# ketanfatania/QMRI-PnP-Recon-POC

Hardware: AMD Instinct MI355X
Metric: ADMM iters/sec (224x224x10 TSMI, spiral mask) (higher is better)
Workload: dtype f32; 1 GPU; cut3 224x224x10 single slice per GPU, spiral mask S=771 T=200, PnP-ADMM + 10-channel UNetRes (DRUNet) denoiser; solver=lsqr, admm_iters=20, dc_dtype=f64, parallelism=slice-parallel x1 (no collective)

## Files before the change

### include/qmri.h

```cpp
#ifndef QMRI_H
#define QMRI_H

#include <stddef.h>
#include <stdint.h>

#ifdef __cplusplus
extern "C" {
#endif

#define QMRI_ABI_VERSION 1

typedef enum {
    QMRI_OK = 0,
    QMRI_ERR_INVALID_ARG = -1,
    QMRI_ERR_STATE = -2,
    QMRI_ERR_HIP = -3,
    QMRI_ERR_UNSUPPORTED = -4,
    QMRI_ERR_NOMEM = -5
} qmri_status;

typedef struct qmri_ctx qmri_ctx;

int qmri_abi_version(void);
int qmri_create(int device, qmri_ctx** out);
// ... 192 lines not shown
int qmri_coil_maps(qmri_ctx* ctx, int nslices, int ncoil, int N, int M, const void* calib, const qmri_csm_params* p, void* maps_out, void* img_out,
                   double* lambda_out, qmri_csm_info* info);
int qmri_coil_maps_dev(qmri_ctx* ctx, int nslices, int ncoil, int N, int M, const void* d_calib, const qmri_csm_params* p, void* d_maps_out,
                       void* d_img_out, double* d_lambda_out, qmri_csm_info* info);

typedef struct {
    int32_t s;
    int32_t s_max;
    double  energy;
    double  tol;
    int32_t maxit;
} qmri_dsvd_params;
typedef struct {
    int32_t s;
    int32_t iters;
    int32_t converged;
    int32_t energy_reached;
    double  max_resid;
    double  energy_kept;
} qmri_dsvd_info;
int qmri_dict_compress(qmri_ctx* ctx, int K, int T, const void* F, int f_is_f64, const qmri_dsvd_params* p, int* s_out, double* V_out, float* D_out,
                       float* normD_out, double* eig_out, qmri_dsvd_info* info);
int qmri_dict_compress_dev(qmri_ctx* ctx, int K, int T, const void* d_F, int f_is_f64, const qmri_dsvd_params* p, int* s_out, double* d_V_out,
                           float* d_D_out, float* d_normD_out, double* eig_out, qmri_dsvd_info* info);

typedef struct {
    int32_t nstates;
    int32_t inversion;
    double  ti;
    double  inv_eff;
    int32_t out_is_f64;
} qmri_epg_params;
int qmri_dict_simulate(qmri_ctx* ctx, int K, int T, const double* alpha, const double* tr, const double* te, const double* t1, const double* t2,
                       const double* b1, const qmri_epg_params* p, void* F_out);
int qmri_dict_simulate_dev(qmri_ctx* ctx, int K, int T, const double* alpha, const double* tr, const double* te, const double* d_t1, const double* d_t2,
                           const double* d_b1, const qmri_epg_params* p, void* d_F_out);

typedef struct {
    int32_t iters;
    double  beta;
    int32_t phase_sign;
    int32_t reserved[4];
} qmri_fieldmap_params;
typedef struct {
    double  cost0, cost;
    double  f_min, f_max;
    int32_t iters;
    int32_t reserved;
    double  unwrap_limit_hz;
} qmri_fieldmap_info;
int qmri_field_map_estimate(qmri_ctx* ctx, int nslices, int nechoes, int ncoil, int N, int M, const void* Y, const double* t_s, const double* f_init,
                            const qmri_fieldmap_params* p, double* f_out, double* trust_out, qmri_fieldmap_info* info);
int qmri_field_map_estimate_dev(qmri_ctx* ctx, int nslices, int nechoes, int ncoil, int N, int M, const void* d_Y, const double* t_s,
                                const double* d_f_init, const qmri_fieldmap_params* p, double* d_f_out, double* d_trust_out, qmri_fieldmap_info* info);

typedef struct {
    double  tau;
    int32_t block;
    int32_t shift;
    int32_t reserved[5];
} qmri_llr_params;
int qmri_llr_prox(qmri_ctx* ctx, int N, int M, int s, int nslices, const void* x, int x_is_complex, const qmri_llr_params* p, int o1, int o2,
                  void* out, double* sigma_max_out);
int qmri_llr_prox_dev(qmri_ctx* ctx, int N, int M, int s, int nslices, const void* d_x, int x_is_complex, const qmri_llr_params* p, int o1, int o2,
                      void* d_out, double* sigma_max_out);
int qmri_set_llr(qmri_ctx* ctx, const qmri_llr_params* p);

typedef struct {
    double ms_xupdate, ms_denoiser, ms_elementwise, ms_diag, ms_match;
    double ms_conv3x3;
    int64_t n_conv3x3;
    int64_t lsqr_iters;
    int64_t admm_iters;
    double ms_tv_iter;
    int64_t n_tv_iter;
    double flop_conv3x3;
    double ms_conv2x2;
    int64_t n_conv2x2;
    double flop_conv2x2;
    double ms_lsqr_kernels;
    int64_t n_lsqr_launches;
    double ms_net_forward;
    int64_t n_net_forward;
} qmri_profile;
int qmri_profile_enable(qmri_ctx* ctx, int level);
int qmri_profile_get(qmri_ctx* ctx, qmri_profile* out, int reset);

typedef struct {
    int denoiser_scheme;
    int denoiser_fallbacks;
    int resident_armed;
    int resident_timeouts;
    int lsqr_one_launch;
    int lsqr_timeouts;
    int repeated_calls;
    int reserved;
    double last_call_wall_ms;
    double last_call_stage_ms[4];
    double set_denoiser_ms[3];
} qmri_health;
int qmri_get_health(const qmri_ctx* ctx, qmri_health* out);

int qmri_debug_lsqr_stamps(qmri_ctx* ctx, unsigned long long* out);
int qmri_debug_conv_stamps(qmri_ctx* ctx, unsigned long long* out, int reserved);
int qmri_debug_lsqr_persist(qmri_ctx* ctx, int on);
int qmri_debug_dict_filter(qmri_ctx* ctx, int on, float margin_scale);
int qmri_debug_conv_resident(qmri_ctx* ctx, int on, int* timeouts_out);
int qmri_debug_dsvd_gram(qmri_ctx* ctx, int K, int T, const void* F, int f_is_f64, int on_device, double* G_out);
int qmri_debug_epg_shift(qmri_ctx* ctx, int S, int nshift, const double* in, double* out);
int qmri_debug_knob(const char* name, int value);

#ifdef __cplusplus
}
#endif
#endif
```

### qmri_pnp_recon_poc_amd/_lib.py

```python
from __future__ import annotations

import ctypes as C
import os
import subprocess

_PKG = os.path.dirname(os.path.abspath(__file__))
LIB_PATH = os.path.join(_PKG, "libqmri.so")
CSRC = os.path.join(_PKG, "csrc")

SYMBOLS = [
    "qmri_abi_version", "qmri_create", "qmri_destroy", "qmri_last_error", "qmri_set_stream", "qmri_synchronize",
    "qmri_build_spiral", "qmri_build_epi", "qmri_build_spiral_traj", "qmri_set_operator", "qmri_set_operator_nufft", "qmri_nufft_prepare_normal", "qmri_normal", "qmri_normal_dev",
    "qmri_nufft_dcf", "qmri_set_sample_weights", "qmri_adjoint_w", "qmri_adjoint_w_dev", "qmri_adjoint_w_mc", "qmri_set_field_map", "qmri_nufft_prepare_normal_fm", "qmri_operator_m", "qmri_forward", "qmri_adjoint",
    "qmri_forward_f32", "qmri_adjoint_f32", "qmri_forward_dev", "qmri_adjoint_dev", "qmri_set_coils", "qmri_forward_mc", "qmri_adjoint_mc", "qmri_xupdate_mc", "qmri_pnp_admm_mc", "qmri_xupdate_mc_batch", "qmri_pnp_admm_mc_batch", "qmri_pnp_admm_mc_dev", "qmri_xupdate", "qmri_net_nparams", "qmri_set_denoiser", "qmri_denoise",
    "qmri_net_forward_dev", "qmri_denoiser_scheme", "qmri_pnp_admm", "qmri_pnp_admm_dev", "qmri_pnp_admm_batch", "qmri_set_dictionary", "qmri_dict_match",
    "qmri_dict_match_dev", "qmri_dict_match_xfit", "qmri_dict_match_xfit_dev", "qmri_set_dictionary_groups", "qmri_dict_group_assign", "qmri_dict_match_grouped",
    "qmri_dict_match_grouped_dev", "qmri_recon_batch", "qmri_recon_batch_mc",
    "qmri_coil_compress", "qmri_coil_compress_dev", "qmri_coil_eig", "qmri_recon_batch_mc_cc", "qmri_coil_maps", "qmri_coil_maps_dev", "qmri_dict_compress", "qmri_dict_compress_dev", "qmri_dict_simulate", "qmri_dict_simulate_dev", "qmri_field_map_estimate", "qmri_field_map_estimate_dev", "qmri_llr_prox", "qmri_llr_prox_dev", "qmri_set_llr", "qmri_profile_enable", "qmri_profile_get", "qmri_get_health",
    "qmri_debug_lsqr_stamps", "qmri_debug_conv_stamps", "qmri_debug_lsqr_persist", "qmri_debug_dict_filter", "qmri_debug_conv_resident", "qmri_debug_dsvd_gram", "qmri_debug_epg_shift", "qmri_debug_knob",
    "qmri_onnx_read_unetres",
    "qmri_lrtv", "qmri_prox_tv", "qmri_norm_tv", "qmri_synthesize_tsmi", "qmri_synthesize_tsmi_complex",
]


# ... 19 lines not shown
    _fields_ = [("nv", C.c_int32), ("energy", C.c_double), ("shared", C.c_int32)]


class CsmParams(C.Structure):
    _fields_ = [("kind", C.c_int), ("cN", C.c_int), ("cM", C.c_int), ("patch", C.c_int), ("window", C.c_int), ("phase_ref", C.c_int), ("thresh", C.c_double)]


class CsmInfo(C.Structure):
    _fields_ = [("max_iters", C.c_int32), ("not_converged", C.c_int32)]


class DsvdParams(C.Structure):
    _fields_ = [("s", C.c_int32), ("s_max", C.c_int32), ("energy", C.c_double), ("tol", C.c_double), ("maxit", C.c_int32)]


class DsvdInfo(C.Structure):
    _fields_ = [("s", C.c_int32), ("iters", C.c_int32), ("converged", C.c_int32), ("energy_reached", C.c_int32),
                ("max_resid", C.c_double), ("energy_kept", C.c_double)]


class EpgParams(C.Structure):
    _fields_ = [("nstates", C.c_int32), ("inversion", C.c_int32), ("ti", C.c_double), ("inv_eff", C.c_double), ("out_is_f64", C.c_int32)]


class NufftParams(C.Structure):
    _fields_ = [("width", C.c_int32), ("reserved", C.c_int32 * 7)]


class DcfParams(C.Structure):
    _fields_ = [("niter", C.c_int32), ("tol", C.c_double), ("reserved", C.c_int32 * 6)]


class DcfInfo(C.Structure):
    _fields_ = [("iters", C.c_int32), ("dev", C.c_double), ("clamped", C.c_int32), ("split_tiles", C.c_int32), ("reserved", C.c_int32 * 4)]


class OffresParams(C.Structure):
    _fields_ = [("nseg", C.c_int32), ("nbins", C.c_int32), ("tol", C.c_double), ("reserved", C.c_int32 * 4)]


class OffresInfo(C.Structure):
    _fields_ = [("nseg", C.c_int32), ("tol_reached", C.c_int32), ("fit_max", C.c_double), ("fit_rms", C.c_double), ("f_min", C.c_double),
                ("f_max", C.c_double), ("t_min", C.c_double), ("t_max", C.c_double), ("reserved", C.c_int32 * 4)]


class OffresNormalParams(C.Structure):
    _fields_ = [("nseg", C.c_int32), ("tol", C.c_double), ("reserved", C.c_int32 * 4)]


class OffresNormalInfo(C.Structure):
    _fields_ = [("nseg", C.c_int32), ("tol_reached", C.c_int32), ("fit_max", C.c_double), ("fit_rms", C.c_double), ("khat_bytes", C.c_uint64),
                ("reserved", C.c_int32 * 4)]


class FieldmapParams(C.Structure):
    _fields_ = [("iters", C.c_int32), ("beta", C.c_double), ("phase_sign", C.c_int32), ("reserved", C.c_int32 * 4)]


class FieldmapInfo(C.Structure):
    _fields_ = [("cost0", C.c_double), ("cost", C.c_double), ("f_min", C.c_double), ("f_max", C.c_double), ("iters", C.c_int32), ("reserved", C.c_int32),
                ("unwrap_limit_hz", C.c_double)]


class LlrParams(C.Structure):
    _fields_ = [("tau", C.c_double), ("block", C.c_int32), ("shift", C.c_int32), ("reserved", C.c_int32 * 5)]


class LrtvParams(C.Structure):
    _fields_ = [("K", C.c_double), ("iters", C.c_int32), ("step", C.c_double), ("tol", C.c_double), ("backtrack", C.c_int32),
                ("prox_tol", C.c_double), ("prox_maxit", C.c_int32)]


class LrtvInfo(C.Structure):
    _fields_ = [("iters", C.c_int32), ("halvings", C.c_int32), ("step", C.c_double), ("obj", C.c_double),
                ("prox_calls", C.c_int32), ("prox_iters_total", C.c_int32)]


class Profile(C.Structure):
    _fields_ = [("ms_xupdate", C.c_double), ("ms_denoiser", C.c_double), ("ms_elementwise", C.c_double),
                ("ms_diag", C.c_double), ("ms_match", C.c_double), ("ms_conv3x3", C.c_double),
                ("n_conv3x3", C.c_int64), ("lsqr_iters", C.c_int64), ("admm_iters", C.c_int64),
                ("ms_tv_iter", C.c_double), ("n_tv_iter", C.c_int64),
                ("flop_conv3x3", C.c_double), ("ms_conv2x2", C.c_double), ("n_conv2x2", C.c_int64), ("flop_conv2x2", C.c_double),
                ("ms_lsqr_kernels", C.c_double), ("n_lsqr_launches", C.c_int64), ("ms_net_forward", C.c_double), ("n_net_forward", C.c_int64)]


class Health(C.Structure):
    _fields_ = [("denoiser_scheme", C.c_int32), ("denoiser_fallbacks", C.c_int32), ("resident_armed", C.c_int32), ("resident_timeouts", C.c_int32),
                ("lsqr_one_launch", C.c_int32), ("lsqr_timeouts", C.c_int32), ("repeated_calls", C.c_int32), ("reserved", C.c_int32),
                ("last_call_wall_ms", C.c_double), ("last_call_stage_ms", C.c_double * 4), ("set_denoiser_ms", C.c_double * 3)]


def build(force: bool = False) -> str:
    srcs = [os.path.join(CSRC, f) for f in os.listdir(CSRC) if f.endswith((".hip", ".cpp", ".h")) or f == "Makefile"]
    srcs.append(os.path.join(os.path.dirname(_PKG), "include", "qmri.h"))
    stale = force or not os.path.exists(LIB_PATH)
    if not stale:
        t = os.path.getmtime(LIB_PATH)
        stale = any(os.path.getmtime(s) > t for s in srcs)
    if stale:
        subprocess.run(["make", "-C", CSRC, "-s", "-j4"], check=True)
    return LIB_PATH


_lib = None


def lib() -> C.CDLL:
    global _lib
    if _lib is not None:
        return _lib
    path = os.environ.get("QMRI_LIBQMRI") or LIB_PATH
    if path == LIB_PATH and not os.path.exists(LIB_PATH):
        build()
    L = C.CDLL(path)
    missing = [s for s in SYMBOLS if not hasattr(L, s)]
    if missing:
        raise ImportError(f"libqmri.so lacks symbols declared in include/qmri.h: {missing}")
    vp, ip, dp, fp, i = C.c_void_p, C.POINTER(C.c_int32), C.POINTER(C.c_double), C.POINTER(C.c_float), C.c_int
    L.qmri_abi_version.restype = i
    L.qmri_create.argtypes = [i, C.POINTER(vp)]
    L.qmri_destroy.argtypes = [vp]
    L.qmri_last_error.restype = C.c_char_p
    L.qmri_last_error.argtypes = [vp]
    L.qmri_set_stream.argtypes = [vp, vp]
    L.qmri_synchronize.argtypes = [vp]
    L.qmri_build_spiral.argtypes = [vp, i, i, i, ip, ip, i, C.POINTER(i)]
    L.qmri_build_epi.argtypes = [vp, i, i, C.c_double, i, ip, ip, i, C.POINTER(i)]
    L.qmri_set_operator.argtypes = [vp, i, i, i, i, dp, ip, ip, i]
    L.qmri_build_spiral_traj.argtypes = [vp, i, i, i, ip, dp, i, C.POINTER(i)]
    L.qmri_set_operator_nufft.argtypes = [vp, i, i, i, i, dp, ip, dp, i, C.POINTER(NufftParams)]
    L.qmri_nufft_prepare_normal.argtypes = [vp]
    L.qmri_normal.argtypes = [vp, vp, i, vp]
    L.qmri_normal_dev.argtypes = [vp, vp, vp, i]
    L.qmri_nufft_dcf.argtypes = [vp, C.POINTER(DcfParams), dp, C.POINTER(DcfInfo)]
    L.qmri_set_sample_weights.argtypes = [vp, dp]
    L.qmri_adjoint_w.argtypes = [vp, vp, vp]
    L.qmri_adjoint_w_dev.argtypes = [vp, vp, vp, i]
    L.qmri_adjoint_w_mc.argtypes = [vp, vp, vp]
    L.qmri_set_field_map.argtypes = [vp, dp, dp, C.POINTER(OffresParams), C.POINTER(OffresInfo)]
    L.qmri_nufft_prepare_normal_fm.argtypes = [vp, C.POINTER(OffresNormalParams), C.POINTER(OffresNormalInfo)]
    L.qmri_operator_m.argtypes = [vp, C.POINTER(i)]
    L.qmri_forward.argtypes = [vp, vp, i, vp]
    L.qmri_adjoint.argtypes = [vp, vp, vp]
    L.qmri_forward_f32.argtypes = [vp, fp, i, fp]
    L.qmri_adjoint_f32.argtypes = [vp, fp, fp]
    L.qmri_forward_dev.argtypes = [vp, vp, vp, i]
    L.qmri_adjoint_dev.argtypes = [vp, vp, vp, i]
    L.qmri_set_coils.argtypes = [vp, i, vp]
    L.qmri_forward_mc.argtypes = [vp, vp, i, vp]
    L.qmri_adjoint_mc.argtypes = [vp, vp, vp]
    L.qmri_xupdate_mc.argtypes = [vp, vp, vp, C.c_double, C.c_double, i, vp, vp, ip, ip]
    L.qmri_pnp_admm_mc.argtypes = [vp, vp, C.POINTER(AdmmParams), vp, vp, ip]
    L.qmri_xupdate_mc_batch.argtypes = [vp, i, i, vp, vp, vp, C.c_double, C.c_double, i, vp, vp, ip, ip]
    L.qmri_pnp_admm_mc_batch.argtypes = [vp, i, i, i, vp, vp, C.POINTER(AdmmParams), vp, vp, ip]
    L.qmri_pnp_admm_mc_dev.argtypes = [vp, i, i, vp, vp, C.POINTER(AdmmParams), vp, vp, ip]
    L.qmri_xupdate.argtypes = [vp, vp, vp, C.c_double, C.c_double, i, i, vp, ip, ip]
    L.qmri_net_nparams.restype = C.c_size_t
    L.qmri_net_nparams.argtypes = [C.POINTER(NetDesc)]
    L.qmri_set_denoiser.argtypes = [vp, C.POINTER(NetDesc), fp, C.c_size_t, i, i, i]
    L.qmri_denoise.argtypes = [vp, dp, i, i, i, i, dp]
    L.qmri_onnx_read_unetres.argtypes = [C.c_char_p, C.POINTER(NetDesc), fp, C.c_size_t, C.POINTER(C.c_size_t)]
    L.qmri_net_forward_dev.argtypes = [vp, vp, i, vp]
    L.qmri_denoiser_scheme.argtypes = [vp, C.POINTER(i), C.POINTER(i)]
    L.qmri_get_health.argtypes = [vp, C.POINTER(Health)]
    L.qmri_pnp_admm.argtypes = [vp, vp, C.POINTER(AdmmParams), vp, vp, vp, dp, ip]
    L.qmri_pnp_admm_dev.argtypes = [vp, i, vp, C.POINTER(AdmmParams), vp, vp, vp, dp, ip]
# ... 42 lines not shown
```

### qmri_pnp_recon_poc_amd/csrc/api_admm.cpp

```cpp
#include "qmri_internal.h"

#include <algorithm>
#include <chrono>
#include <cstdio>

struct StageTimer {
    qmri_ctx* ctx;
    bool on, marks;
    int cur = -1;
    explicit StageTimer(qmri_ctx* c) : ctx(c), on(c->prof_level == 1 || c->prof_level == 2), marks(c->prof_level == 3) {
        c->marks_n = 0;
        for (double& v : c->last_call_ms) v = 0.0;
    }
    void start() {
        if (on) (void)hipEventRecord(ctx->ev[0], ctx->stream);
        if (marks) {
            if (ctx->marks_n + 2 > ctx->marks.size()) {
                hipEvent_t a = nullptr, b = nullptr;
                if (hipEventCreate(&a) != hipSuccess || hipEventCreate(&b) != hipSuccess) { marks = false; return; }
                ctx->marks.push_back(a); ctx->marks.push_back(b); ctx->mark_kind.push_back(0);
            }
            cur = (int)ctx->marks_n;
            (void)hipEventRecord(ctx->marks[cur], ctx->stream);
        }
    }
    void stop(double& acc) {
        if (on) {
            (void)hipEventRecord(ctx->ev[1], ctx->stream);
            (void)hipEventSynchronize(ctx->ev[1]);
            float ms = 0.f;
            (void)hipEventElapsedTime(&ms, ctx->ev[0], ctx->ev[1]);
            acc += ms;
            ctx->last_call_ms[kind_of(acc)] += ms;
        }
        if (marks && cur >= 0) {
            (void)hipEventRecord(ctx->marks[cur + 1], ctx->stream);
            ctx->mark_kind[cur / 2] = kind_of(acc);
            ctx->marks_n = (size_t)cur + 2;
            cur = -1;
        }
    }
    int kind_of(const double& acc) const {
        const qmri_profile& p = ctx->prof;
        return (&acc == &p.ms_xupdate) ? 0 : (&acc == &p.ms_denoiser) ? 1 : (&acc == &p.ms_elementwise) ? 2 : 3;
    }
    void resolve() {
        if (!marks) return;
        for (size_t i = 0; i + 1 < ctx->marks_n; i += 2) {
            float ms = 0.f;
            if (hipEventElapsedTime(&ms, ctx->marks[i], ctx->marks[i + 1]) != hipSuccess) continue;
            const int k = ctx->mark_kind[i / 2];
            ctx->last_call_ms[k] += ms;
            (k == 0 ? ctx->prof.ms_xupdate : k == 1 ? ctx->prof.ms_denoiser : k == 2 ? ctx->prof.ms_elementwise : ctx->prof.ms_diag) += ms;
        }
        ctx->marks_n = 0;
    }
};

static int admm_net_fits(qmri_ctx* ctx, const qmri_admm_params* prm, int* multi_out, bool* cpx_out) {
    const OpHost& o = ctx->op;
    const NetPlan& net = ctx->net;
    QMRI_CHECK_ARG(ctx, prm->denoiser_type >= 0 && prm->denoiser_type <= (QMRI_DENOISER_COMPLEX | QMRI_DENOISER_MULTI_LEVEL),
                   "denoiser_type must be 0 .. 3 (QMRI_DENOISER_MULTI_LEVEL | QMRI_DENOISER_COMPLEX)");
    const int multi = (prm->denoiser_type & QMRI_DENOISER_MULTI_LEVEL) ? 1 : 0;
    const bool cpx = (prm->denoiser_type & QMRI_DENOISER_COMPLEX) != 0;
    const int planes = cpx ? 2 * o.s : o.s, other = cpx ? o.s : 2 * o.s;
    if (net.H != o.N || net.W != o.M || net.desc.in_nc != planes + multi || net.desc.out_nc != planes) {
        const bool other_domain = net.desc.in_nc == other + multi && net.desc.out_nc == other;
        qmri_set_error(ctx, "denoiser (%d x %d, %d -> %d channels) does not fit the operator (%d x %d x %d, %s, %s TSMIs: %d -> %d channels needed)",
                       net.H, net.W, net.desc.in_nc, net.desc.out_nc, o.N, o.M, o.s, multi ? "multi_level" : "single_level",
                       cpx ? "complex" : "real", planes + multi, planes);
        return (cpx || other_domain) ? QMRI_ERR_STATE : QMRI_ERR_INVALID_ARG;
    }
    *multi_out = multi;
    *cpx_out = cpx;
    return QMRI_OK;
}

static int admm_step_fits(qmri_ctx* ctx, const qmri_admm_params* prm, int* multi_out, bool* cpx_out) {
    if (!ctx->llr.on) return admm_net_fits(ctx, prm, multi_out, cpx_out);
    const OpHost& o = ctx->op;
    QMRI_CHECK_ARG(ctx, prm->denoiser_type >= 0 && prm->denoiser_type <= (QMRI_DENOISER_COMPLEX | QMRI_DENOISER_MULTI_LEVEL),
                   "denoiser_type must be 0 .. 3 (QMRI_DENOISER_MULTI_LEVEL | QMRI_DENOISER_COMPLEX)");
    if (o.N % ctx->llr.block || o.M % ctx->llr.block || o.s > 16) {
        qmri_set_error(ctx, "invalid argument: the LLR regulariser (block side %d, at most 16 channels) does not fit the operator (%d x %d x %d): the "
                            "block side must divide both sides", ctx->llr.block, o.N, o.M, o.s);
        return QMRI_ERR_INVALID_ARG;
    }
    *multi_out = 0;
    *cpx_out = (prm->denoiser_type & QMRI_DENOISER_COMPLEX) != 0;
    return QMRI_OK;
}

static int admm_start(qmri_ctx* ctx, int B, const double2* d_x, bool z_now) {
    OpHost& o = ctx->op;
    const size_t nb = (size_t)B * o.N * o.M * o.s * sizeof(double2);
    QMRI_HIP(ctx, hipMemcpyAsync(o.d_vv, d_x, nb, hipMemcpyDeviceToDevice, ctx->stream));
    QMRI_HIP(ctx, hipMemsetAsync(o.d_u, 0, nb, ctx->stream));
    if (z_now) QMRI_TRY(dc_launch_prepare_z(ctx, qmri_opdev(ctx), o.ls, B, o.d_vv, o.d_u, o.d_z));
    return QMRI_OK;
}

struct DenoiserStep { int B; const qmri_admm_params* prm; int multi; bool cpx; const double2* d_x; StageTimer* tm; };

static int admm_to_net(qmri_ctx* ctx, const DenoiserStep& d, int mm_nblk, bool mm_ready, bool copy_range_flag) {
    OpHost& o = ctx->op;
    NetPlan& net = ctx->net;
    const size_t plane = (size_t)o.N * o.M;
    if (d.tm) d.tm->start();
    QMRI_TRY(ew_launch_minmax_normalise(ctx, d.B, plane * o.s, (int)plane, o.N, o.s, d.multi, d.prm->noise_std, d.d_x, o.d_u, o.d_mm, o.d_norm, mm_nblk, net.in32,
                                        mm_ready, d.cpx));
    if (d.tm) { d.tm->stop(ctx->prof.ms_elementwise); d.tm->start(); }
    QMRI_TRY(net_forward(ctx, d.B));
    if (copy_range_flag && net.sp6 == 2 && (int)net.layers.size() + 1 > net.h_range_words)
        QMRI_HIP(ctx, hipMemcpyAsync(net.h_range_flag, net.d_range_flag, sizeof(unsigned), hipMemcpyDeviceToHost, ctx->stream));
    if (d.tm) d.tm->stop(ctx->prof.ms_denoiser);
    return QMRI_OK;
}

static int admm_denoiser_step(qmri_ctx* ctx, const DenoiserStep& d, bool copy_range_flag, int it) {
    OpHost& o = ctx->op;
    NetPlan& net = ctx->net;
    const size_t plane = (size_t)o.N * o.M;
    if (ctx->llr.on) {
        LlrPlan pl = {o.N, o.M, o.s, ctx->llr.block, 0, 0, d.cpx ? 0 : 1, ctx->llr.tau};
        llr_offsets(it, pl.block, ctx->llr.shift, &pl.o1, &pl.o2);
        if (d.tm) d.tm->start();
        QMRI_TRY(llr_prox_dev(ctx, pl, d.B, d.d_x, o.d_u, o.d_vv, nullptr, nullptr));
        if (d.tm) { d.tm->stop(ctx->prof.ms_denoiser); d.tm->start(); }
        QMRI_TRY(llr_dual_dev(ctx, d.B, plane * o.s, d.d_x, o.d_vv, o.d_u, o.d_z, o.ls.pz, o.ls.nblk_z));
        if (d.tm) d.tm->stop(ctx->prof.ms_elementwise);
        return QMRI_OK;
    }
    QMRI_TRY(admm_to_net(ctx, d, o.ls.nblk_z, false, copy_range_flag));
    if (d.tm) d.tm->start();
    QMRI_TRY(ew_launch_unnormalise_dual(ctx, d.B, plane * o.s, (int)plane, o.N, net.out32, net.in32, net.desc.residual_noise, o.d_norm, d.d_x, o.d_u,
                                        nullptr , o.d_z, o.ls.pz, o.ls.nblk_z, o.s, d.cpx));
    if (d.tm) d.tm->stop(ctx->prof.ms_elementwise);
    return QMRI_OK;
}

static int mc_require(qmri_ctx* ctx, int nslices, int ncoil, const void* maps, const void* y) {
    const OpHost& o = ctx->op;
    if (!o.ready) { qmri_set_error(ctx, "operator not set: call qmri_set_operator first"); return QMRI_ERR_STATE; }
    QMRI_CHECK_ARG(ctx, nslices >= 1 && ncoil >= 1 && ncoil <= 1024, "nslices >= 1 and 1 <= ncoil <= 1024");
    QMRI_CHECK_ARG(ctx, maps && y, "maps / y_mc must not be NULL");
    return QMRI_OK;
}
static int mc_admm_check(qmri_ctx* ctx, const qmri_admm_params* prm) {
    const NetPlan& net = ctx->net;
    if (!net.ready && !ctx->llr.on) { qmri_set_error(ctx, "denoiser not set: call qmri_set_denoiser first"); return QMRI_ERR_STATE; }
    QMRI_CHECK_ARG(ctx, prm, "params must not be NULL");
    QMRI_TRY(toep_check_solver(ctx, prm->solver));
    QMRI_CHECK_ARG(ctx, prm->iters >= 0 && prm->gamma > 0 && prm->cg_maxit >= 0 && (prm->solver == QMRI_SOLVER_LSQR || prm->solver == QMRI_SOLVER_TOEPLITZ),
                   "iters >= 0, gamma > 0, cg_maxit >= 0, LSQR solver required");
    int multi = 0;
    bool cpx = false;
    return admm_step_fits(ctx, prm, &multi, &cpx);
}

static int mc_admm_group(qmri_ctx* ctx, int B, int ncoil, const double2* d_maps, const double2* d_y, const qmri_admm_params* prm, const double2* d_x0,
                         double2* d_x, int32_t* li_out, int li_stride) {
    OpHost& o = ctx->op;
    const bool llr = ctx->llr.on;
    const int multi = (!llr && (prm->denoiser_type & QMRI_DENOISER_MULTI_LEVEL)) ? 1 : 0;
    const bool cpx = (prm->denoiser_type & QMRI_DENOISER_COMPLEX) != 0;
    const size_t n = (size_t)o.N * o.M * o.s;
    std::vector<int32_t> li((size_t)B);
    for (int attempt = 0;; ++attempt) {
        if (d_x0) QMRI_HIP(ctx, hipMemcpyAsync(d_x, d_x0, (size_t)B * n * sizeof(double2), hipMemcpyDeviceToDevice, ctx->stream));
        else QMRI_TRY(mc_adjoint_batch_dev(ctx, B, ncoil, d_maps, d_y, d_x));
        QMRI_TRY(admm_start(ctx, B, d_x, true));
        bool again = false;
        for (int it = 0; it < prm->iters; ++it) {
            QMRI_TRY(mc_xupdate_dev(ctx, prm->solver, B, ncoil, d_maps, d_y, o.d_z, prm->gamma, prm->cg_tol, prm->cg_maxit, d_x, li.data(), nullptr));
            if (li_out) for (int b = 0; b < B; ++b) li_out[(size_t)b * li_stride + it] = li[b];
            QMRI_TRY(admm_denoiser_step(ctx, {B, prm, multi, cpx, d_x, nullptr}, false, it));
            if (llr) continue;
            QMRI_HIP(ctx, hipStreamSynchronize(ctx->stream));
            QMRI_TRY(net_range_tripped(ctx, again));
            if (again) break;
        }
        if (!again) break;
        ctx->admm_repeats += 1;
        if (attempt >= 2) { qmri_set_error(ctx, "the denoiser's range guard tripped three times in a row in the multi-coil PnP-ADMM loop"); return QMRI_ERR_HIP; }
    }
    o.xhat_valid = false;
    return QMRI_OK;
}

struct McStaged {
    const void* maps;
    const void* y;
    const void* to_sz;
    const void* to_sx; bool zero_sx;
    void* x_out;
// ... 12 lines not shown
    else if (sg.zero_sx) QMRI_HIP(ctx, hipMemsetAsync(w.sx, 0, nx, ctx->stream));
    QMRI_TRY(run(w));
    QMRI_HIP(ctx, hipMemcpyAsync(sg.x_out, w.sx, nx, out, ctx->stream));
    if (sync) QMRI_HIP(ctx, hipStreamSynchronize(ctx->stream));
    return QMRI_OK;
}

static int pnp_admm_nufft(qmri_ctx* ctx, int nslices, const void* d_y, const qmri_admm_params* prm, const void* d_x0, void* d_x_out,
                          double* diag_out, int32_t* lsqr_iters_out) {
    if (nslices != 1) {
        qmri_set_error(ctx, "PnP-ADMM of %d slices in one call is not available on a trajectory operator (qmri_set_operator_nufft): reconstruct them "
                            "one at a time, or as a stack with qmri_pnp_admm_mc_batch and one unit coil per slice", nslices);
        return QMRI_ERR_UNSUPPORTED;
    }
    if (prm && prm->solver != QMRI_SOLVER_LSQR && prm->solver != QMRI_SOLVER_TOEPLITZ) {
        qmri_set_error(ctx, "the DIRECT solver is not available on a trajectory operator (qmri_set_operator_nufft): its closed form needs a gridded "
                            "mask; use QMRI_SOLVER_LSQR");
        return QMRI_ERR_UNSUPPORTED;
    }
    if (prm && prm->want_diag && diag_out) {
        qmri_set_error(ctx, "the per-iteration diagnostics are not available on a trajectory operator (qmri_set_operator_nufft): set want_diag = 0 "
                            "and evaluate the result with qmri_forward");
        return QMRI_ERR_UNSUPPORTED;
    }
    QMRI_TRY(mc_admm_check(ctx, prm));
    QMRI_CHECK_ARG(ctx, d_y && d_x_out && d_x_out != d_x0, "y / x_out must not be NULL, x_out must not alias x0");
    return mc_staged(ctx, 1, 1, {nullptr, d_y, d_x0, nullptr, false, d_x_out, true}, true, [&](McWork& w) {
        return mc_admm_group(ctx, 1, 1, ctx->op.nu.d_ones, w.sy, prm, d_x0 ? w.sz : nullptr, w.sx, lsqr_iters_out, prm->iters);
    });
}

static int pnp_admm_dev_impl(qmri_ctx* ctx, int nslices, const void* d_y, const qmri_admm_params* prm, const void* d_x0,
                             const void* d_gt, void* d_x_out, double* diag_out, int32_t* lsqr_iters_out, bool* repeat) {
    QMRI_HIP(ctx, hipSetDevice(ctx->device));
    if (ctx->op.ready && ctx->op.kind == OP_NUFFT) return pnp_admm_nufft(ctx, nslices, d_y, prm, d_x0, d_x_out, diag_out, lsqr_iters_out);
    OpHost& o = ctx->op;
    NetPlan& net = ctx->net;
    if (!o.ready) { qmri_set_error(ctx, "operator not set: call qmri_set_operator first"); return QMRI_ERR_STATE; }
    const bool llr = ctx->llr.on;
    if (!net.ready && !llr) { qmri_set_error(ctx, "denoiser not set: call qmri_set_denoiser first"); return QMRI_ERR_STATE; }
    QMRI_CHECK_ARG(ctx, d_y && prm && d_x_out, "y / params / x_out must not be NULL");
    const int B = nslices;
    QMRI_CHECK_ARG(ctx, B >= 1 && B <= o.maxB && (llr || B <= net.maxB), "nslices exceeds max_batch of the operator or the denoiser");
    QMRI_CHECK_ARG(ctx, prm->iters >= 0 && prm->gamma > 0 && prm->cg_maxit >= 0, "iters >= 0, gamma > 0, cg_maxit >= 0 required");
    int multi = 0;
    bool cpx = false;
    QMRI_TRY(admm_step_fits(ctx, prm, &multi, &cpx));
    const OpDev op = qmri_opdev(ctx);
    const size_t plane = (size_t)o.N * o.M, n = plane * o.s, nb = (size_t)B * n * sizeof(double2);
    const double2* y = (const double2*)d_y;
    StageTimer tm(ctx);

    QMRI_TRY(dc_launch_sort_y(ctx, op, o.ls, B, y));
    if (d_x0) QMRI_HIP(ctx, hipMemcpyAsync(o.d_x, d_x0, nb, hipMemcpyDeviceToDevice, ctx->stream));
    else QMRI_TRY(dc_launch_adj(ctx, op, B, y, o.d_tmp, o.d_x));
    QMRI_TRY(admm_start(ctx, B, o.d_x, false));
    if (prm->solver == QMRI_SOLVER_DIRECT) {
        QMRI_TRY(qmri_prepare_direct(ctx, prm->gamma));
        const double2* aty = o.d_x;
        if (d_x0) { QMRI_TRY(dc_launch_adj(ctx, op, B, y, o.d_tmp, o.d_xa)); aty = o.d_xa; }
        QMRI_TRY(dc_launch_fwd(ctx, op, o.ls, DC_SPECTRUM, B, aty, o.d_tmp, o.d_chat, nullptr));
    } else if (prm->solver != QMRI_SOLVER_LSQR) {
        QMRI_TRY(toep_check_solver(ctx, prm->solver));
        qmri_set_error(ctx, "unknown solver %d", prm->solver);
        return QMRI_ERR_INVALID_ARG;
    }
    if (prm->want_diag && diag_out) {
        if (o.d_diag) { (void)hipFree(o.d_diag); o.d_diag = nullptr; }
        QMRI_HIP(ctx, hipMalloc((void**)&o.d_diag, (size_t)B * std::max(prm->iters, 1) * 2 * sizeof(double)));
    }
    std::vector<int32_t> it_b(B);
    o.xhat_valid = false;
    const bool diag = prm->want_diag && diag_out;
    bool range_trip = false;
    std::vector<char> deferred_it((size_t)std::max(prm->iters, 1), 0);
    if (prm->solver == QMRI_SOLVER_LSQR && (size_t)prm->iters * B > o.h_ring_cap) {
        if (o.h_ring) { QMRI_HIP(ctx, hipStreamSynchronize(ctx->stream)); (void)hipHostFree(o.h_ring); o.h_ring = nullptr; o.h_ring_cap = 0; }
        const size_t cap = std::max<size_t>((size_t)prm->iters * B, 128);
        QMRI_HIP(ctx, hipHostMalloc((void**)&o.h_ring, cap * sizeof(LsqrState), hipHostMallocDefault));
        o.h_ring_cap = cap;
    }
    const bool fused = qmri_knob(K_FUSE_EW) != 0 && prm->solver == QMRI_SOLVER_LSQR && !llr;
    const int hb = dc_hpass_blocks(op);
    bool z_in_tmp = false;
    struct DeferGuard { NetPlan& n; ~DeferGuard() { n.act_defer = false; n.act_pending_valid = false; } } defer_guard{net};
    net.act_defer = fused;
    const DenoiserStep step = {B, prm, multi, cpx, o.d_x, &tm};
    for (int it = 0; it < prm->iters; ++it) {
        tm.start();
        if (it == 0) QMRI_TRY(dc_launch_prepare_z(ctx, op, o.ls, B, o.d_vv, o.d_u, o.d_z));
        if (prm->solver == QMRI_SOLVER_LSQR) {
            bool deferred = false;
            LsqrFuse lf;
            if (fused) { lf.z_hpass_nblk = z_in_tmp ? hb : 0; lf.mm_u = o.d_u; lf.mm = o.d_mm; lf.mm_cpx = cpx; }
            QMRI_TRY(qmri_lsqr_run(ctx, B, o.d_z, prm->gamma, prm->cg_tol, prm->cg_maxit, o.d_x, it_b.data(), nullptr,
                                   diag ? o.d_pd : nullptr,
                                   o.h_ring + (size_t)it * B, &deferred, &lf));
            deferred_it[it] = deferred ? 1 : 0;
            if (!deferred && lsqr_iters_out) for (int b = 0; b < B; ++b) lsqr_iters_out[(size_t)b * prm->iters + it] = it_b[b];
            if (it > 0 && !llr && net.sp6 == 2 && host_range_tripped(net)) { range_trip = true; tm.stop(ctx->prof.ms_xupdate); break; }
        } else {
            QMRI_TRY(dc_launch_direct(ctx, op, B, o.d_z, o.d_chat, prm->gamma, o.d_tmp, o.d_x));
            if (lsqr_iters_out) for (int b = 0; b < B; ++b) lsqr_iters_out[(size_t)b * prm->iters + it] = 0;
        }
        tm.stop(ctx->prof.ms_xupdate);
        if (prm->want_diag && diag_out) {
            tm.start();
            if (prm->solver != QMRI_SOLVER_LSQR) QMRI_TRY(dc_launch_fwd(ctx, op, o.ls, DC_DIAG, B, o.d_x, o.d_tmp, nullptr, o.d_pd));
            QMRI_TRY(ew_launch_diag(ctx, op, o.ls, B, o.d_x, (const double2*)d_gt, o.d_pd, o.d_diag, prm->iters, it));
            tm.stop(ctx->prof.ms_diag);
        }
        if (!fused) QMRI_TRY(admm_denoiser_step(ctx, step, !llr, it));
        else {
            QMRI_TRY(admm_to_net(ctx, step, hb, true, true));
            tm.start();
            const DualArgs da = {net.out32.base1(), net.in32.base1(), net.out32.hp, (int)net.out32.plane(), net.out32.batch_stride(), net.in32.batch_stride(),
                                 net.desc.residual_noise, o.d_norm, o.d_x, o.d_u, o.ls.pz, cpx ? 1 : 0};
            ActCheckArgs ac{};
            if (net.act_pending_valid) { ac = net.act_pending; net.act_pending_valid = false; }
            QMRI_TRY(dc_launch_dual_fwd_h(ctx, op, B, da, ac, o.d_tmp));
            z_in_tmp = true;
            tm.stop(ctx->prof.ms_elementwise);
        }
        ctx->prof.admm_iters += 1;
    }
    if (!range_trip) {
        QMRI_HIP(ctx, hipMemcpyAsync(d_x_out, o.d_x, nb, hipMemcpyDeviceToDevice, ctx->stream));
    }
    if (prm->want_diag && diag_out && prm->iters > 0 && !range_trip)
        QMRI_HIP(ctx, hipMemcpyAsync(diag_out, o.d_diag, (size_t)B * prm->iters * 2 * sizeof(double), hipMemcpyDeviceToHost, ctx->stream));
    QMRI_HIP(ctx, hipStreamSynchronize(ctx->stream));
    tm.resolve();
    QMRI_TRY(qmri_prof_chain_finish(ctx));
    if (prm->solver == QMRI_SOLVER_LSQR && !range_trip) {
        bool timed_out = false;
        for (int it = 0; it < prm->iters; ++it) {
            if (!deferred_it[it]) continue;
            for (int b = 0; b < B; ++b) {
                const LsqrState& h = o.h_ring[(size_t)it * B + b];
                if (h.flag == 77) timed_out = true;
                const int n_it = h.done ? h.iter : prm->cg_maxit;
                if (lsqr_iters_out) lsqr_iters_out[(size_t)b * prm->iters + it] = n_it;
                ctx->prof.lsqr_iters += n_it;
            }
        }
        if (timed_out) {
            fprintf(stderr, "libqmri: the one-launch LSQR timed out waiting for a partial sum; repeating the reconstruction with the two-launch iteration\n");
            ctx->ks_persist = 0;
            ctx->ks_timeouts += 1;
            *repeat = true;
            return QMRI_OK;
        }
    }
    if (prm->iters > 0 && !llr) QMRI_TRY(net_range_tripped(ctx, *repeat));
    return QMRI_OK;
}

extern "C" int qmri_pnp_admm_dev(qmri_ctx* ctx, int nslices, const void* d_y, const qmri_admm_params* prm, const void* d_x0,
                                 const void* d_gt, void* d_x_out, double* diag_out, int32_t* lsqr_iters_out) {
    if (!ctx) return QMRI_ERR_INVALID_ARG;
    const auto t0 = std::chrono::steady_clock::now();
    const auto prof_at_entry = ctx->prof;
    int st = QMRI_OK;
    for (bool repeat = true; st == QMRI_OK && repeat;) {
        repeat = false;
        st = pnp_admm_dev_impl(ctx, nslices, d_y, prm, d_x0, d_gt, d_x_out, diag_out, lsqr_iters_out, &repeat);
        if (st == QMRI_OK && repeat) { ctx->prof = prof_at_entry; ctx->admm_repeats += 1; }
    }
    ctx->last_call_wall_ms = std::chrono::duration<double, std::milli>(std::chrono::steady_clock::now() - t0).count();
    return st;
}

extern "C" int qmri_xupdate_mc_batch(qmri_ctx* ctx, int nslices, int ncoil, const void* maps, const void* y_mc, const void* z, double r, double tol, int maxit,
                                     const void* x0, void* x_out, int32_t* iters_out, int32_t* flags_out) {
    if (!ctx) return QMRI_ERR_INVALID_ARG;
    QMRI_HIP(ctx, hipSetDevice(ctx->device));
    QMRI_TRY(mc_require(ctx, nslices, ncoil, maps, y_mc));
    QMRI_CHECK_ARG(ctx, z && x_out && r > 0 && maxit >= 0, "z / x_out must not be NULL, r > 0, maxit >= 0");
    return mc_staged(ctx, nslices, ncoil, {maps, y_mc, z, x0, true, x_out}, true, [&](McWork& w) {
        return qmri_lsqr_mc_batch_dev(ctx, nslices, ncoil, w.sm, w.sy, w.sz, r, tol, maxit, w.sx, iters_out, flags_out);
    });
}

extern "C" int qmri_pnp_admm_mc_dev(qmri_ctx* ctx, int nslices, int ncoil, const void* d_maps, const void* d_y, const qmri_admm_params* prm,
                                    const void* d_x0, void* d_x_out, int32_t* lsqr_iters_out) {
    if (!ctx) return QMRI_ERR_INVALID_ARG;
    QMRI_HIP(ctx, hipSetDevice(ctx->device));
    QMRI_TRY(mc_require(ctx, nslices, ncoil, d_maps, d_y));
    QMRI_TRY(mc_admm_check(ctx, prm));
    QMRI_CHECK_ARG(ctx, d_x_out && d_x_out != d_x0, "x_out must not be NULL and must not alias x0");
    QMRI_CHECK_ARG(ctx, nslices <= ctx->op.maxB && (ctx->llr.on || nslices <= ctx->net.maxB), "nslices exceeds max_batch of the operator or the denoiser");
    QMRI_TRY(mc_admm_group(ctx, nslices, ncoil, (const double2*)d_maps, (const double2*)d_y, prm, (const double2*)d_x0, (double2*)d_x_out,
                           lsqr_iters_out, prm->iters));
    QMRI_HIP(ctx, hipStreamSynchronize(ctx->stream));
    return QMRI_OK;
}

// ... 112 lines not shown
```

### qmri_pnp_recon_poc_amd/csrc/api_core.cpp

```cpp
#include "qmri_internal.h"
#include "fft_codelets.h"

#include <algorithm>
#include <atomic>
#include <cmath>
#include <cstdarg>
#include <cstdlib>
#include <cstring>
#include <mutex>

static thread_local std::string g_create_err;

namespace {
struct KnobDef { const char* name; int dflt; };
const KnobDef g_knob_defs[K_COUNT] = {
    {"conv_scheme", 2}, {"conv_f32", 0}, {"conv_wt", 1}, {"conv_xcd", 1}, {"conv_persist", 1}, {"conv_splitk", 1},
    {"conv_midcfg", 3}, {"conv_deepcfg", 3}, {"conv_deepks", 4},
    {"conv_resident", 1}, {"res_head", 1}, {"res_tail", 1}, {"res_down", 1}, {"res_delay", 24}, {"res_rearm", 64},
    {"res_stamps", 0}, {"conv_stamps", 0}, {"conv_stamp_launch", -1}, {"lsqr_stamps", 0},
    {"conv_mt2", 1024}, {"conv_occ", 2},
    {"fuse_ew", 1}, {"lsqr_persist", 1}, {"lsqr_fold", 1}, {"dictw_lsp", 2}, {"verbose", 0},
    {"pack_gpu", 1}, {"nufft_seg", NU_SEG},
    {"fmap_fuse", 0}, {"fmap_start", 0},
};
std::atomic<int> g_knob_val[K_COUNT];
std::once_flag g_knob_once;

int knob_index(const char* name, size_t len) {
    for (int k = 0; k < K_COUNT; ++k)
        if (strlen(g_knob_defs[k].name) == len && strncmp(g_knob_defs[k].name, name, len) == 0) return k;
    return -1;
}
void knob_init() {
    for (int k = 0; k < K_COUNT; ++k) g_knob_val[k].store(g_knob_defs[k].dflt, std::memory_order_relaxed);
    const char* e = getenv("QMRI_DEBUG");
    while (e && *e) {
        const char* end = strchr(e, ',');
        const size_t len = end ? (size_t)(end - e) : strlen(e);
        const char* eq = (const char*)memchr(e, '=', len);
        const int k = eq ? knob_index(e, (size_t)(eq - e)) : -1;
        if (k >= 0) g_knob_val[k].store(atoi(eq + 1), std::memory_order_relaxed);
        else if (len) fprintf(stderr, "libqmri: QMRI_DEBUG: unknown or malformed entry '%.*s' ignored\n", (int)len, e);
        e = end ? end + 1 : nullptr;
    }
}
}

int qmri_knob(QmriKnob k) {
    std::call_once(g_knob_once, knob_init);
    return g_knob_val[k].load(std::memory_order_relaxed);
}

extern "C" int qmri_debug_knob(const char* name, int value) {
    std::call_once(g_knob_once, knob_init);
    const int k = name ? knob_index(name, strlen(name)) : -1;
    if (k < 0) { qmri_set_error(nullptr, "qmri_debug_knob: unknown knob '%s'", name ? name : "(null)"); return QMRI_ERR_INVALID_ARG; }
    g_knob_val[k].store(value, std::memory_order_relaxed);
    return QMRI_OK;
}

void qmri_set_error(qmri_ctx* ctx, const char* fmt, ...) {
    char buf[1024];
    va_list ap;
    va_start(ap, fmt);
    vsnprintf(buf, sizeof buf, fmt, ap);
    va_end(ap);
    if (ctx) ctx->err = buf; else g_create_err = buf;
}

extern "C" int qmri_abi_version(void) { return QMRI_ABI_VERSION; }

extern "C" const char* qmri_last_error(const qmri_ctx* ctx) { return ctx ? ctx->err.c_str() : g_create_err.c_str(); }

extern "C" int qmri_create(int device, qmri_ctx** out) {
    if (!out) { qmri_set_error(nullptr, "qmri_create: out is NULL"); return QMRI_ERR_INVALID_ARG; }
    *out = nullptr;
    int ndev = 0;
    hipError_t e = hipGetDeviceCount(&ndev);
    if (e != hipSuccess || ndev <= 0) {
        qmri_set_error(nullptr, "no HIP device available (%s); libqmri has no CPU fallback",
                       e != hipSuccess ? hipGetErrorString(e) : "device count 0");
        return QMRI_ERR_HIP;
    }
    if (device < 0 || device >= ndev) {
        qmri_set_error(nullptr, "device %d out of range (0..%d)", device, ndev - 1);
        return QMRI_ERR_INVALID_ARG;
    }
    hipDeviceProp_t prop;
    if ((e = hipGetDeviceProperties(&prop, device)) != hipSuccess) {
        qmri_set_error(nullptr, "hipGetDeviceProperties failed: %s", hipGetErrorString(e));
        return QMRI_ERR_HIP;
    }
    if (strncmp(prop.gcnArchName, "gfx950", 6) != 0) {
        qmri_set_error(nullptr, "device %d is %s; libqmri is built for gfx950 (MI355X) only", device, prop.gcnArchName);
        return QMRI_ERR_UNSUPPORTED;
    }
    if ((e = hipSetDevice(device)) != hipSuccess) {
        qmri_set_error(nullptr, "hipSetDevice failed: %s", hipGetErrorString(e));
        return QMRI_ERR_HIP;
    }
    qmri_ctx* ctx = new (std::nothrow) qmri_ctx();
    if (!ctx) { qmri_set_error(nullptr, "out of host memory"); return QMRI_ERR_NOMEM; }
    ctx->device = device;
    if ((e = hipStreamCreateWithFlags(&ctx->own_stream, hipStreamNonBlocking)) != hipSuccess) {
        qmri_set_error(nullptr, "hipStreamCreate failed: %s", hipGetErrorString(e));
        delete ctx;
        return QMRI_ERR_HIP;
    }
    ctx->stream = ctx->own_stream;
    for (auto& ev : ctx->ev) {
        if ((e = hipEventCreate(&ev)) != hipSuccess) {
            qmri_set_error(nullptr, "hipEventCreate failed: %s", hipGetErrorString(e));
            for (auto& x : ctx->ev) if (x) (void)hipEventDestroy(x);
            (void)hipStreamDestroy(ctx->own_stream);
            delete ctx;
            return QMRI_ERR_HIP;
        }
    }
    *out = ctx;
    return QMRI_OK;
}

static void free_dev(void* p) { if (p) (void)hipFree(p); }

void qmri_free_operator(qmri_ctx* ctx) {
    OpHost& o = ctx->op;
    void* ptrs[] = { o.d_Vt, o.d_ent, o.d_perm, o.d_kptr, o.d_tw, o.d_kslot, o.d_ginv, o.d_tmp, o.d_xa, o.d_xb, o.d_ya,
                     o.ls.st, o.ls.pz, o.ls.yk, o.ls.py,
                     (void*)o.ks.unit, (void*)o.ks.es, (void*)o.ks.grp, (void*)o.ks.sgrp,
                     o.ks.pu[0], o.ks.pu[1], o.ks.pv[0], o.ks.pv[1], o.ks.pinit, o.ks.pR, o.ks.cx, o.ks.cv, o.ks.cd, o.ks.cub,
                     o.ks.ut, o.ks.xhat, o.ks.zhat, o.ks.xhat_out, o.ks.stamps,
                     o.d_x, o.d_u, o.d_vv, o.d_z, o.d_chat, o.d_mm, o.d_norm, o.d_diag, o.d_pd, o.d_coils };
    for (void* p : ptrs) free_dev(p);
    if (o.h_state) (void)hipHostFree(o.h_state);
    if (o.h_ring) (void)hipHostFree(o.h_ring);
    free_dev(ctx->d_ks_gran); ctx->d_ks_gran = nullptr; ctx->ks_persist_cap = -1;
    mc_free_work(o.mc);
    nufft_free(o.nu);
    o = OpHost();
}

extern "C" int qmri_destroy(qmri_ctx* ctx) {
    if (!ctx) return QMRI_OK;
    (void)hipSetDevice(ctx->device);
    (void)hipStreamSynchronize(ctx->stream);
    qmri_free_operator(ctx);
    qmri_free_net(ctx);
    qmri_free_dict(ctx);
    cc_free_work(ctx->cc);
    for (auto& ev : ctx->ev) if (ev) (void)hipEventDestroy(ev);
    if (ctx->ev_state) (void)hipEventDestroy(ctx->ev_state);
    for (hipEvent_t e : ctx->chain) if (e) (void)hipEventDestroy(e);
    for (hipEvent_t e : ctx->marks) if (e) (void)hipEventDestroy(e);
    if (ctx->own_stream) (void)hipStreamDestroy(ctx->own_stream);
    delete ctx;
    return QMRI_OK;
}

extern "C" int qmri_set_stream(qmri_ctx* ctx, void* hip_stream) {
    if (!ctx) return QMRI_ERR_INVALID_ARG;
    ctx->stream = hip_stream ? (hipStream_t)hip_stream : ctx->own_stream;
    return QMRI_OK;
}

extern "C" int qmri_synchronize(qmri_ctx* ctx) {
    if (!ctx) return QMRI_ERR_INVALID_ARG;
    QMRI_HIP(ctx, hipSetDevice(ctx->device));
    QMRI_HIP(ctx, hipStreamSynchronize(ctx->stream));
    return QMRI_OK;
}

void spiral_points(int S, std::vector<double>& theta, std::vector<double>& rad) {
    const double pi = 3.14159265358979323846;
    theta.assign(S, 0.0); rad.assign(S, 0.0);
    double lo = HUGE_VAL, hi = -HUGE_VAL;
    for (int j = 0; j < S; ++j) {
        const double t = (j == S - 1) ? 2.0 * pi : (double)j * (2.0 * pi) / (double)(S - 1);
        theta[j] = 8.0 * t;
        rad[j] = std::pow(1.05, theta[j]);
        lo = std::min(lo, rad[j]);
        hi = std::max(hi, rad[j]);
    }
    for (double& r : rad) r = (r - lo) / (hi - lo);
}

extern "C" int qmri_build_spiral(qmri_ctx* ctx, int N, int S, int T, int32_t* frame_ptr, int32_t* kidx, int cap, int* m_out) {
    QMRI_CHECK_ARG(ctx, N > 0 && S > 1 && T > 0 && frame_ptr && (kidx || cap == 0) && m_out, "qmri_build_spiral arguments");
    const double delta = SPIRAL_DELTA;
    std::vector<double> theta, rad;
    spiral_points(S, theta, rad);
    std::vector<uint8_t> grid((size_t)N * N);
    const int half = N / 2;
    long m = 0;
    for (int f = 0; f < T; ++f) {
        frame_ptr[f] = (int32_t)m;
        std::fill(grid.begin(), grid.end(), 0);
        const double rot = (double)f * delta;
        for (int j = 0; j < S; ++j) {
            double gx = std::round(rad[j] * std::cos(theta[j] + rot) * N / 2.0) + N / 2.0 + 1.0;
            double gy = std::round(rad[j] * std::sin(theta[j] + rot) * N / 2.0) + N / 2.0 + 1.0;
            gx = std::min(gx, (double)N);
            gy = std::min(gy, (double)N);
            const int r = ((int)gx - 1 + half) % N, c = ((int)gy - 1 + half) % N;
            grid[(size_t)c * N + r] = 1;
        }
        for (int k = 0; k < N * N; ++k)
            if (grid[k]) {
                if (m < cap) kidx[m] = k;
                ++m;
            }
    }
    frame_ptr[T] = (int32_t)m;
    *m_out = (int)m;
    if (m > cap) { qmri_set_error(ctx, "kidx capacity %d too small, need %ld", cap, m); return QMRI_ERR_INVALID_ARG; }
    return QMRI_OK;
// ... 153 lines not shown
        ks.caps = base;
        int nunits = cut(KS_CAPS[base]);
        if (sparse && nunits < 0) { base = 0; ks.caps = 0; nunits = cut(KS_CAPS[0]); }
        const bool one_launch = ctx->ks_persist != 0 && (ctx->ks_persist > 0 || qmri_knob(K_LSQR_PERSIST));
        if ((max_batch == 1 || one_launch) && s == 10 && (nunits > 320 || nunits < 0)) {
            int ncu = 0;
            QMRI_HIP(ctx, hipDeviceGetAttribute(&ncu, hipDeviceAttributeMultiprocessorCount, ctx->device));
            const int order[2] = {sparse ? 1 : 2, sparse ? 2 : 1};
            for (int c : order) {
                bool fits = false;
                QMRI_TRY(ks_lds_fits(ctx, N, s, M, ks.vcap, c, &fits));
                if (!fits) continue;
                const int nu = cut(KS_CAPS[c]);
                if (nu > 0 && nu <= ncu) { ks.caps = c; nunits = nu; break; }
            }
            if (ks.caps == base) nunits = cut(KS_CAPS[base]);
        }
        if (nunits < 0) {
            int tried = std::max(KS_CAPS[base].ecap, KS_CAPS[0].ecap);
            if ((max_batch == 1 || one_launch) && s == 10) tried = std::max(tried, std::max(KS_CAPS[1].ecap, KS_CAPS[2].ecap));
            qmri_set_error(ctx, "a k location is sampled %d times; at most %d are supported%s", -nunits, tried,
                           tried < KS_CAPS[2].ecap ? " with several slices per launch and the two-launch LSQR iteration (one slice per launch: 2560)" : "");
            return QMRI_ERR_UNSUPPORTED;
        }
        bslot.push_back(ns);
        gptr.push_back((int32_t)grp.size());
        sgrp[ns] = (int32_t)grp.size();
        ks.ns = ns; ks.G = (int)bslot.size() - 1; ks.b0 = 0;
        bool v_fits = false;
        QMRI_TRY(ks_lds_fits(ctx, N, s, M, ks.vcap, ks.caps, &v_fits));
        if (!v_fits) {
            qmri_set_error(ctx, "V (T=%d x s=%d) does not fit the on-chip budget of the LSQR kernels", T, s);
            return QMRI_ERR_UNSUPPORTED;
        }
        std::vector<KsUnit> units(ks.G);
        for (int g = 0; g < ks.G; ++g) units[g] = KsUnit{bslot[g], bslot[g + 1], sptr[bslot[g]], sptr[bslot[g + 1]], gptr[g], gptr[g + 1], 0, 0};
        int32_t* p32; KSample* pes; KsGroup* pg; KsUnit* pu_;
#define KS_UPLOAD(ptr, field, vec, T_)                                                                 \
        QMRI_TRY(dev_alloc(ctx, &ptr, (vec).size()));                                                  \
        QMRI_HIP(ctx, hipMemcpy(ptr, (vec).data(), (vec).size() * sizeof(T_), hipMemcpyHostToDevice)); \
        ks.field = ptr;
        KS_UPLOAD(p32, sgrp, sgrp, int32_t)
        KS_UPLOAD(pes, es, es, KSample)
        KS_UPLOAD(pg, grp, grp, KsGroup)
        KS_UPLOAD(pu_, unit, units, KsUnit)
#undef KS_UPLOAD
        ctx->ks_lds_attr[0] = ctx->ks_lds_attr[1] = false;
    }
    ls.nblk_z = 256;
    OpDev dims{};
    dims.N = N; dims.M = M; dims.s = s;
    const size_t npart = (size_t)std::max(ls.nblk_z, dc_hpass_blocks(dims));
    QMRI_TRY(dev_alloc(ctx, &o.d_tmp, B * n));
    QMRI_TRY(dev_alloc(ctx, &o.d_xa, B * n));
    QMRI_TRY(dev_alloc(ctx, &o.d_xb, B * n));
    QMRI_TRY(dev_alloc(ctx, &o.d_ya, B * (size_t)m));
    QMRI_TRY(dev_alloc(ctx, &ls.st, B));
    QMRI_TRY(dev_alloc(ctx, &ls.pz, B * npart));
    QMRI_TRY(dev_alloc(ctx, &ls.py, B * (size_t)DC_SORT_BLOCKS));
    for (int par = 0; par < 2; ++par) {
        QMRI_TRY(dev_alloc(ctx, &ks.pu[par], B * 2 * ks.G));
        QMRI_TRY(dev_alloc(ctx, &ks.pv[par], B * ks.G));
    }
    QMRI_TRY(dev_alloc(ctx, &ks.pinit, B * 2 * N));
    QMRI_TRY(dev_alloc(ctx, &ks.pR, B * N));
    QMRI_TRY(dev_alloc(ctx, &ks.cx, B * ks.ns * s));
    QMRI_TRY(dev_alloc(ctx, &ks.cv, B * ks.ns * s));
    QMRI_TRY(dev_alloc(ctx, &ks.cd, B * ks.ns * s));
    QMRI_TRY(dev_alloc(ctx, &ks.cub, B * ks.ns * s));
    QMRI_TRY(dev_alloc(ctx, &ks.ut, B * (size_t)m));
    QMRI_TRY(dev_alloc(ctx, &ks.xhat, B * n));
    QMRI_TRY(dev_alloc(ctx, &ks.zhat, B * n));
    QMRI_TRY(dev_alloc(ctx, &ks.xhat_out, B * n));
    ks.stamps = nullptr;
    if (qmri_knob(K_LSQR_STAMPS) > 0) { QMRI_TRY(dev_alloc(ctx, &ks.stamps, (size_t)2 * 512 * 16)); QMRI_HIP(ctx, hipMemset(ks.stamps, 0, 2 * 512 * 16 * 8)); }
    QMRI_TRY(dev_alloc(ctx, &ls.yk, B * (size_t)m));
    QMRI_TRY(dev_alloc(ctx, &o.d_x, B * n));
    QMRI_TRY(dev_alloc(ctx, &o.d_u, B * n));
    QMRI_TRY(dev_alloc(ctx, &o.d_vv, B * n));
    QMRI_TRY(dev_alloc(ctx, &o.d_z, B * n));
    QMRI_TRY(dev_alloc(ctx, &o.d_chat, B * n));
    QMRI_TRY(dev_alloc(ctx, &o.d_mm, B * npart * 2));
    QMRI_TRY(dev_alloc(ctx, &o.d_norm, B * 2));
    QMRI_TRY(dev_alloc(ctx, &o.d_pd, B * ((size_t)N + 2 * ls.nblk_z)));
    QMRI_HIP(ctx, hipMemset(ls.st, 0, B * sizeof(LsqrState)));
    QMRI_HIP(ctx, hipHostMalloc((void**)&o.h_state, B * sizeof(LsqrState), hipHostMallocDefault));
    ks.hst = nullptr; ks.st = ls.st; ks.pz = ls.pz; ks.nblk_z = ls.nblk_z; ks.yk = ls.yk; ks.pdiag = nullptr;
    o.xhat_valid = false;
    o.ginv_r = -1.0;
    QMRI_HIP(ctx, hipDeviceSynchronize());
    o.ready = true;
    return QMRI_OK;
}

extern "C" int qmri_operator_m(const qmri_ctx* ctx, int* m_out) {
    if (!ctx || !m_out) return QMRI_ERR_INVALID_ARG;
    if (!ctx->op.ready) return QMRI_ERR_STATE;
    *m_out = ctx->op.m;
    return QMRI_OK;
}

#define REQUIRE_OP(ctx)                                                                   \
    do {                                                                                  \
        if (!(ctx)) return QMRI_ERR_INVALID_ARG;                                          \
        QMRI_HIP((ctx), hipSetDevice((ctx)->device));                                     \
        if (!(ctx)->op.ready) { qmri_set_error((ctx), "operator not set: call qmri_set_operator first"); return QMRI_ERR_STATE; } \
    } while (0)

extern "C" int qmri_forward_dev(qmri_ctx* ctx, const void* d_x, void* d_y, int batch) {
    REQUIRE_OP(ctx);
    QMRI_CHECK_ARG(ctx, d_x && d_y && batch >= 1 && batch <= ctx->op.maxB, "qmri_forward_dev arguments / batch > max_batch");
    if (ctx->op.kind == OP_NUFFT) return nufft_launch_fwd(ctx, batch, (const double2*)d_x, (double2*)d_y);
    return dc_launch_fwd(ctx, qmri_opdev(ctx), ctx->op.ls, DC_PLAIN, batch, (const double2*)d_x, ctx->op.d_tmp,
                         (double2*)d_y, nullptr);
}

extern "C" int qmri_adjoint_dev(qmri_ctx* ctx, const void* d_y, void* d_x, int batch) {
    REQUIRE_OP(ctx);
    QMRI_CHECK_ARG(ctx, d_x && d_y && batch >= 1 && batch <= ctx->op.maxB, "qmri_adjoint_dev arguments / batch > max_batch");
    if (ctx->op.kind == OP_NUFFT) return nufft_launch_adj(ctx, batch, (const double2*)d_y, (double2*)d_x);
    return dc_launch_adj(ctx, qmri_opdev(ctx), batch, (const double2*)d_y, ctx->op.d_tmp, (double2*)d_x);
}

extern "C" int qmri_forward(qmri_ctx* ctx, const void* x, int x_is_complex, void* y) {
    REQUIRE_OP(ctx);
    QMRI_CHECK_ARG(ctx, x && y, "x / y must not be NULL");
    OpHost& o = ctx->op;
    const size_t n = (size_t)o.N * o.M * o.s;
    if (x_is_complex) {
        QMRI_HIP(ctx, hipMemcpyAsync(o.d_xa, x, n * sizeof(double2), hipMemcpyHostToDevice, ctx->stream));
    } else {
        QMRI_HIP(ctx, hipMemcpyAsync(o.d_xb, x, n * sizeof(double), hipMemcpyHostToDevice, ctx->stream));
        QMRI_TRY(ew_launch_real_to_complex(ctx, n, (const double*)o.d_xb, o.d_xa));
    }
    QMRI_TRY(qmri_forward_dev(ctx, o.d_xa, o.d_ya, 1));
    QMRI_HIP(ctx, hipMemcpyAsync(y, o.d_ya, (size_t)o.m * sizeof(double2), hipMemcpyDeviceToHost, ctx->stream));
    QMRI_HIP(ctx, hipStreamSynchronize(ctx->stream));
    return QMRI_OK;
}

extern "C" int qmri_adjoint(qmri_ctx* ctx, const void* y, void* x) {
    REQUIRE_OP(ctx);
    QMRI_CHECK_ARG(ctx, x && y, "x / y must not be NULL");
    OpHost& o = ctx->op;
    const size_t n = (size_t)o.N * o.M * o.s;
    QMRI_HIP(ctx, hipMemcpyAsync(o.d_ya, y, (size_t)o.m * sizeof(double2), hipMemcpyHostToDevice, ctx->stream));
    QMRI_TRY(qmri_adjoint_dev(ctx, o.d_ya, o.d_xa, 1));
    QMRI_HIP(ctx, hipMemcpyAsync(x, o.d_xa, n * sizeof(double2), hipMemcpyDeviceToHost, ctx->stream));
    QMRI_HIP(ctx, hipStreamSynchronize(ctx->stream));
    return QMRI_OK;
}

extern "C" int qmri_set_coils(qmri_ctx* ctx, int ncoil, const void* maps) {
    REQUIRE_OP(ctx);
    OpHost& o = ctx->op;
    QMRI_CHECK_ARG(ctx, ncoil >= 0 && ncoil <= 1024 && (ncoil == 0 || maps), "0 <= ncoil <= 1024, maps must not be NULL");
    QMRI_HIP(ctx, hipStreamSynchronize(ctx->stream));
    if (o.d_coils) { (void)hipFree(o.d_coils); o.d_coils = nullptr; }
    o.ncoil = 0;
    if (ncoil == 0) return QMRI_OK;
    const size_t count = (size_t)ncoil * o.N * o.M;
    QMRI_HIP(ctx, hipMalloc((void**)&o.d_coils, count * sizeof(double2)));
    QMRI_HIP(ctx, hipMemcpy(o.d_coils, maps, count * sizeof(double2), hipMemcpyHostToDevice));
    QMRI_HIP(ctx, hipDeviceSynchronize());
    o.ncoil = ncoil;
    return QMRI_OK;
// ... 47 lines not shown
    const size_t n = (size_t)o.N * o.M * o.s * (x_is_complex ? 2 : 1);
    std::vector<double> xd(x, x + n), yd((size_t)2 * o.m);
    QMRI_TRY(qmri_forward(ctx, xd.data(), x_is_complex, yd.data()));
    for (size_t i = 0; i < yd.size(); ++i) y[i] = (float)yd[i];
    return QMRI_OK;
}

extern "C" int qmri_adjoint_f32(qmri_ctx* ctx, const float* y, float* x) {
    REQUIRE_OP(ctx);
    QMRI_CHECK_ARG(ctx, x && y, "x / y must not be NULL");
    const OpHost& o = ctx->op;
    const size_t n2 = (size_t)2 * o.N * o.M * o.s;
    std::vector<double> yd(y, y + (size_t)2 * o.m), xd(n2);
    QMRI_TRY(qmri_adjoint(ctx, yd.data(), xd.data()));
    for (size_t i = 0; i < n2; ++i) x[i] = (float)xd[i];
    return QMRI_OK;
}

int qmri_prepare_direct(qmri_ctx* ctx, double r) {
    OpHost& o = ctx->op;
    if (o.ginv_r == r) return QMRI_OK;
    const int s = o.s, NM = o.N * o.M, T = o.T;
    std::vector<double> ginv((size_t)o.nsampled * s * s);
    std::vector<double> G(s * s), Li(s * s);
    int slot = 0;
    for (int kp = 0; kp < NM; ++kp) {
        const int e0 = o.kptr_h[kp], e1 = o.kptr_h[kp + 1];
        if (e1 == e0) continue;
        std::fill(G.begin(), G.end(), 0.0);
        for (int e = e0; e < e1; ++e) {
            const int t = o.ent_h[e].t;
            for (int a = 0; a < s; ++a)
                for (int b = 0; b < s; ++b) G[a * s + b] += o.V[t + (size_t)T * a] * o.V[t + (size_t)T * b];
        }
        for (int a = 0; a < s; ++a) G[a * s + a] += r;
        for (int j = 0; j < s; ++j) {
            double d = G[j * s + j];
            for (int k = 0; k < j; ++k) d -= G[j * s + k] * G[j * s + k];
            const double ljj = std::sqrt(d);
            G[j * s + j] = ljj;
            for (int i = j + 1; i < s; ++i) {
                double v = G[i * s + j];
                for (int k = 0; k < j; ++k) v -= G[i * s + k] * G[j * s + k];
                G[i * s + j] = v / ljj;
            }
        }
        std::fill(Li.begin(), Li.end(), 0.0);
        for (int c = 0; c < s; ++c) {
            for (int i = c; i < s; ++i) {
                double v = (i == c) ? 1.0 : 0.0;
                for (int k = c; k < i; ++k) v -= G[i * s + k] * Li[k * s + c];
                Li[i * s + c] = v / G[i * s + i];
            }
        }
        double* out = ginv.data() + (size_t)slot * s * s;
        for (int a = 0; a < s; ++a)
            for (int b = 0; b < s; ++b) {
                double v = 0.0;
                for (int k = std::max(a, b); k < s; ++k) v += Li[k * s + a] * Li[k * s + b];
                out[a * s + b] = v;
            }
        ++slot;
    }
    QMRI_HIP(ctx, hipMemcpyAsync(o.d_ginv, ginv.data(), ginv.size() * sizeof(double), hipMemcpyHostToDevice, ctx->stream));
    QMRI_HIP(ctx, hipStreamSynchronize(ctx->stream));
    o.ginv_r = r;
    return QMRI_OK;
}

int qmri_lsqr_run(qmri_ctx* ctx, int B, const double2* d_z, double r, double tol, int maxit, double2* d_x,
                  int32_t* iters_out, int32_t* flag_out, double* pdiag, LsqrState* hslot, bool* deferred, const LsqrFuse* fuse) {
    OpHost& o = ctx->op;
    QMRI_TRY(nufft_check_gridded(ctx, "the k-space LSQR", "the image-domain LSQR of the qmri_*_mc calls applies (internal)"));
    const OpDev op = qmri_opdev(ctx);
    KsDev ks = o.ks;
    ks.sr = std::sqrt(r); ks.tol = tol; ks.maxit = maxit; ks.ii = 0; ks.pdiag = pdiag;
    LsqrState* const hs = hslot ? hslot : o.h_state;
    ks.hst = hs;
    if (deferred) *deferred = false;
    const bool z_fused = fuse && fuse->z_hpass_nblk > 0;
    const double2* const mm_u = fuse ? fuse->mm_u : nullptr;
    double* const mm = fuse ? fuse->mm : nullptr;
    const bool mm_cpx = fuse && fuse->mm_cpx;
    if (z_fused && !o.xhat_valid) { qmri_set_error(ctx, "qmri_lsqr_run: a transformed z needs the spectrum of x (internal)"); return QMRI_ERR_STATE; }
    if (!o.xhat_valid) QMRI_TRY(dc_launch_fwd(ctx, op, o.ls, DC_SPECTRUM, B, d_x, o.d_tmp, ks.xhat, nullptr));
    if (z_fused) ks.nblk_z = fuse->z_hpass_nblk;
    else QMRI_TRY(dc_launch_fwd(ctx, op, o.ls, DC_FWD_H_ONLY, B, d_z, o.d_tmp, nullptr, nullptr));
    if (ctx->ks_persist < 0) ctx->ks_persist = qmri_knob(K_LSQR_PERSIST) ? 1 : 0;
    int per_launch = 0;
    if (ctx->ks_persist > 0 && maxit >= 1) QMRI_TRY(ks_persist_plan(ctx, op, ks, B, &per_launch));
    const bool fold = per_launch > 0 && qmri_knob(K_LSQR_FOLD) != 0;
    QMRI_TRY(ks_launch_init(ctx, op, ks, B, o.d_tmp, !fold));
    if (!ctx->ev_state) QMRI_HIP(ctx, hipEventCreateWithFlags(&ctx->ev_state, hipEventDisableTiming));
    bool persisted = false;
    if (per_launch > 0) {
        if (!ctx->d_ks_gran) {
            const size_t nb = ks_gran_bytes(ks.G, o.maxB);
            QMRI_HIP(ctx, hipMalloc(&ctx->d_ks_gran, nb));
            QMRI_HIP(ctx, hipMemsetAsync(ctx->d_ks_gran, 0, nb, ctx->stream));
        }
        const unsigned tag0 = ctx->ks_tag;
        QMRI_TRY(ks_launch_persist(ctx, op, ks, B, ctx->d_ks_gran, tag0, fold, &persisted));
        if (persisted) {
            ctx->ks_tag += 2u * (unsigned)(maxit + 2);
            QMRI_TRY(ks_launch_final(ctx, op, ks, B, o.d_tmp));
            QMRI_TRY(dc_launch_adj_h(ctx, op, B, o.d_tmp, d_x, mm_u, mm, mm_cpx));
            if (deferred) {
                *deferred = true;
                std::swap(o.ks.xhat, o.ks.xhat_out);
                o.xhat_valid = true;
                return QMRI_OK;
            }
            QMRI_HIP(ctx, hipStreamSynchronize(ctx->stream));
            for (int b = 0; b < B; ++b)
                if ((unsigned)__atomic_load_n(&hs[b].pad, __ATOMIC_ACQUIRE) != tag0) {
                    qmri_set_error(ctx, "the one-launch LSQR kernel ended without reporting its state");
                    return QMRI_ERR_HIP;
                }
            bool timed_out = false;
            for (int b = 0; b < B; ++b) timed_out = timed_out || hs[b].flag == 77;
            if (timed_out) {
                fprintf(stderr, "libqmri: the one-launch LSQR timed out waiting for a partial sum; using the two-launch iteration from now on\n");
                ctx->ks_persist = 0;
                ctx->ks_timeouts += 1;
                persisted = false;
                QMRI_TRY(ks_launch_init(ctx, op, ks, B));
            }
        }
    }
    if (fold && !persisted && !(ctx->ks_persist == 0)) QMRI_TRY(ks_launch_init(ctx, op, ks, B));
    int launched = 0;
    int chunk = std::min(std::max(ctx->lsqr_pred, 1), std::max(maxit, 1));
    bool all_done = persisted;
    if (!persisted) do {
        const int nthis = std::min(chunk, maxit - launched);
        for (int k = 0; k < nthis; ++k) {
            ks.ii = launched + k + 1;
            QMRI_TRY(ks_launch_iter(ctx, op, ks, B));
        }
        launched += std::max(nthis, 0);
        QMRI_HIP(ctx, hipEventRecord(ctx->ev_state, ctx->stream));
        QMRI_TRY(ks_launch_final(ctx, op, ks, B, o.d_tmp));
        QMRI_TRY(dc_launch_adj_h(ctx, op, B, o.d_tmp, d_x, mm_u, mm, mm_cpx));
        QMRI_HIP(ctx, hipEventSynchronize(ctx->ev_state));
        all_done = true;
        for (int b = 0; b < B; ++b) all_done = all_done && hs[b].done;
        chunk = 2;
    } while (launched < maxit && !all_done);
    std::swap(o.ks.xhat, o.ks.xhat_out);
    o.xhat_valid = true;
    int worst = 0;
    for (int b = 0; b < B; ++b) {
        const int it = hs[b].done ? hs[b].iter : maxit;
        if (iters_out) iters_out[b] = it;
        if (flag_out) flag_out[b] = hs[b].done ? hs[b].flag : 1;
        worst = std::max(worst, it);
        ctx->prof.lsqr_iters += it;
    }
    ctx->lsqr_pred = worst + 1;
    return QMRI_OK;
}

extern "C" int qmri_xupdate(qmri_ctx* ctx, const void* y, const void* z, double r, double tol, int maxit, int solver,
                            void* x, int32_t* iters_out, int32_t* flag_out) {
    if (solver == QMRI_SOLVER_TOEPLITZ) QMRI_TRY(offres_refuse_toeplitz(ctx, "QMRI_SOLVER_TOEPLITZ"));
    REQUIRE_OP(ctx);
    QMRI_CHECK_ARG(ctx, y && z && x && r > 0 && maxit >= 0, "qmri_xupdate arguments");
    OpHost& o = ctx->op;
    if (o.kind == OP_NUFFT) {
        if (solver != QMRI_SOLVER_LSQR && solver != QMRI_SOLVER_TOEPLITZ) {
            qmri_set_error(ctx, "the DIRECT solver is not available on a trajectory operator (qmri_set_operator_nufft): its closed form needs a gridded "
                                "mask; use QMRI_SOLVER_LSQR");
            return QMRI_ERR_UNSUPPORTED;
        }
        const size_t n = (size_t)o.N * o.M * o.s;
        QMRI_TRY(mc_ensure_staging(ctx, 1, 1));
        McWork& w = o.mc;
        QMRI_HIP(ctx, hipMemcpyAsync(w.sy, y, (size_t)o.m * sizeof(double2), hipMemcpyHostToDevice, ctx->stream));
        QMRI_HIP(ctx, hipMemcpyAsync(w.sz, z, n * sizeof(double2), hipMemcpyHostToDevice, ctx->stream));
        QMRI_HIP(ctx, hipMemcpyAsync(w.sx, x, n * sizeof(double2), hipMemcpyHostToDevice, ctx->stream));
        QMRI_TRY(mc_xupdate_dev(ctx, solver, 1, 1, o.nu.d_ones, w.sy, w.sz, r, tol, maxit, w.sx, iters_out, flag_out));
        QMRI_HIP(ctx, hipMemcpyAsync(x, w.sx, n * sizeof(double2), hipMemcpyDeviceToHost, ctx->stream));
        QMRI_HIP(ctx, hipStreamSynchronize(ctx->stream));
        return QMRI_OK;
    }
    const OpDev op = qmri_opdev(ctx);
    const size_t n = (size_t)o.N * o.M * o.s;
    QMRI_HIP(ctx, hipMemcpyAsync(o.d_ya, y, (size_t)o.m * sizeof(double2), hipMemcpyHostToDevice, ctx->stream));
    QMRI_HIP(ctx, hipMemcpyAsync(o.d_z, z, n * sizeof(double2), hipMemcpyHostToDevice, ctx->stream));
    QMRI_HIP(ctx, hipMemcpyAsync(o.d_x, x, n * sizeof(double2), hipMemcpyHostToDevice, ctx->stream));
    if (solver == QMRI_SOLVER_LSQR) {
        QMRI_TRY(dc_launch_sort_y(ctx, op, o.ls, 1, o.d_ya));
        QMRI_HIP(ctx, hipMemsetAsync(o.d_u, 0, n * sizeof(double2), ctx->stream));
        QMRI_TRY(dc_launch_prepare_z(ctx, op, o.ls, 1, o.d_z, o.d_u, o.d_vv));
        o.xhat_valid = false;
        QMRI_TRY(qmri_lsqr_run(ctx, 1, o.d_vv, r, tol, maxit, o.d_x, iters_out, flag_out, nullptr, nullptr, nullptr, nullptr));
    } else if (solver == QMRI_SOLVER_DIRECT) {
        QMRI_TRY(qmri_prepare_direct(ctx, r));
        QMRI_TRY(dc_launch_adj(ctx, op, 1, o.d_ya, o.d_tmp, o.d_xa));
        QMRI_TRY(dc_launch_fwd(ctx, op, o.ls, DC_SPECTRUM, 1, o.d_xa, o.d_tmp, o.d_chat, nullptr));
        QMRI_TRY(dc_launch_direct(ctx, qmri_opdev(ctx), 1, o.d_z, o.d_chat, r, o.d_tmp, o.d_x));
        if (iters_out) *iters_out = 0;
        if (flag_out) *flag_out = 0;
    } else {
        QMRI_TRY(toep_check_solver(ctx, solver));
        qmri_set_error(ctx, "unknown solver %d", solver);
        return QMRI_ERR_INVALID_ARG;
    }
    QMRI_HIP(ctx, hipMemcpyAsync(x, o.d_x, n * sizeof(double2), hipMemcpyDeviceToHost, ctx->stream));
    QMRI_HIP(ctx, hipStreamSynchronize(ctx->stream));
    return qmri_prof_chain_finish(ctx);
}

extern "C" int qmri_debug_lsqr_persist(qmri_ctx* ctx, int on) {
    if (!ctx) return QMRI_ERR_INVALID_ARG;
    ctx->ks_persist = (on == 2) ? 2 : (on ? 1 : 0);
    if (ctx->d_ks_gran && ctx->op.ready) {
        QMRI_HIP(ctx, hipSetDevice(ctx->device));
        QMRI_HIP(ctx, hipMemsetAsync((char*)ctx->d_ks_gran + ks_gran_bytes(ctx->op.ks.G, ctx->op.maxB) - 64, 0, 64, ctx->stream));
    }
    return QMRI_OK;
}

extern "C" int qmri_debug_lsqr_stamps(qmri_ctx* ctx, unsigned long long* out) {
    if (!ctx || !ctx->op.ks.stamps) return QMRI_ERR_STATE;
    QMRI_HIP(ctx, hipStreamSynchronize(ctx->stream));
// ... 56 lines not shown
```

### qmri_pnp_recon_poc_amd/csrc/api_net.cpp

```cpp
#include "qmri_internal.h"

#include <algorithm>
#include <chrono>
#include <cmath>
#include <cstdio>
#include <cstring>

extern "C" size_t qmri_net_nparams(const qmri_net_desc* d) {
    if (!d) return 0;
    size_t n = 0;
    if (d->arch == QMRI_ARCH_UNETRES) {
        const int32_t* nc = d->nc;
        n += (size_t)nc[0] * d->in_nc * 9;
        for (int l = 0; l < 3; ++l) n += (size_t)2 * d->nb * nc[l] * nc[l] * 9 + (size_t)nc[l + 1] * nc[l] * 4;
        n += (size_t)2 * d->nb * nc[3] * nc[3] * 9;
        for (int l = 3; l > 0; --l) n += (size_t)nc[l] * nc[l - 1] * 4 + (size_t)2 * d->nb * nc[l - 1] * nc[l - 1] * 9;
        n += (size_t)d->out_nc * nc[0] * 9;
    } else if (d->arch == QMRI_ARCH_SEQ_CONV) {
        if (d->nb == 1) return (size_t)d->out_nc * d->in_nc * 9;
        n = (size_t)d->nc[0] * d->in_nc * 9 + (size_t)(d->nb - 2) * d->nc[0] * d->nc[0] * 9 + (size_t)d->out_nc * d->nc[0] * 9;
    }
    return n;
}

// ... 289 lines not shown
        QMRI_HIP(ctx, hipStreamSynchronize(ctx->stream));
        ms_pack += std::chrono::duration<double, std::milli>(Clk::now() - t0).count();
    }
    p.w_begin = nullptr;
    QMRI_TRY(alloc_tensor(ctx, p.in32, desc->in_nc, conv_cin_pad(CONV_3X3, desc->in_nc), H, W, B));
    QMRI_TRY(alloc_tensor(ctx, p.out32, desc->out_nc, desc->out_nc, H, W, B));
    p.blk_ok = conv6_enabled();
    for (const ConvLayer& L : p.layers) if (!L.wp6) p.blk_ok = false;
    if (desc->arch == QMRI_ARCH_UNETRES) { for (int l = 0; l < 4; ++l) if (desc->nc[l] % 8) p.blk_ok = false; }
    else if (nb > 1 && desc->nc[0] % 8) p.blk_ok = false;
    for (int l = 0; l < 4; ++l) if ((p.x[l].p && p.x[l].Cal % 8) || (p.a[l].p && p.a[l].Cal % 8) || (p.t[l].p && p.t[l].Cal % 8)) p.blk_ok = false;
    p.interior_fmt = -1;
    QMRI_TRY(dev_alloc(ctx, &p.d_counter, (size_t)1));
    QMRI_HIP(ctx, hipMemset(p.d_counter, 0, sizeof(unsigned)));
    if (qmri_knob(K_CONV_STAMPS)) { QMRI_HIP(ctx, hipMalloc(&p.d_stamps, 4096 * 11 * sizeof(unsigned long long))); }
    p.counter_base = 0;
    p.ready = true;
    QMRI_HIP(ctx, hipDeviceSynchronize());
    const auto t_cal = Clk::now();
    if (p.sp6 == 2) QMRI_TRY(net_calibrate_scheme(ctx));
    const auto t_end = Clk::now();
    p.setup_ms[0] = ms_pack;
    p.setup_ms[2] = std::chrono::duration<double, std::milli>(t_end - t_cal).count();
    p.setup_ms[1] = std::chrono::duration<double, std::milli>(t_cal - t_upload).count() - ms_pack;
    return QMRI_OK;
}

static int run_resblocks(qmri_ctx* ctx, size_t& li, int nb, int B, const PTensor& src, const PTensor& cur, const PTensor& tmp,
                         const PTensor* skip) {
    NetPlan& p = ctx->net;
    if (p.d_res_xbuf && src.H == p.H && src.W == p.W && !p.force_f32) {
        bool done = false;
        Conv6rRun r;
        r.res = &p.layers[li]; r.nres = 2 * nb; r.src = &src; r.cur = &cur; r.skip = skip;
        QMRI_TRY(conv6r_try(ctx, r, B, &done));
        if (done) { li += (size_t)(2 * nb); return QMRI_OK; }
    }
    const PTensor* in = &src;
    for (int b = 0; b < nb; ++b) {
        QMRI_TRY(conv_launch(ctx, p.layers[li++], B, *in, tmp, nullptr, nullptr, 1));
        QMRI_TRY(conv_launch(ctx, p.layers[li++], B, tmp, cur, in, (b == nb - 1) ? skip : nullptr, 0));
        in = &cur;
    }
    return QMRI_OK;
}

static int net_forward_layers(qmri_ctx* ctx, int B);

static int net_forward_padded(qmri_ctx* ctx, int B) {
    {
        NetPlan& p = ctx->net;
        const bool blk = p.blk_ok && !p.force_f32 && conv6_enabled();
        if (p.interior_fmt != -1 && p.interior_fmt != (blk ? 1 : 0)) {
            PTensor* ts[12];
            int nt = 0;
            for (int l = 0; l < 4; ++l) { ts[nt++] = &p.x[l]; ts[nt++] = &p.a[l]; ts[nt++] = &p.t[l]; }
            for (int i = 0; i < nt; ++i)
                if (ts[i]->p) QMRI_HIP(ctx, hipMemsetAsync(ts[i]->p, 0, ((size_t)p.maxB * ts[i]->batch_stride() + 8192) * sizeof(float), ctx->stream));
        }
        p.interior_fmt = blk ? 1 : 0;
        for (int l = 0; l < 4; ++l) { p.x[l].blk = blk; p.a[l].blk = blk; p.t[l].blk = blk; }
    }
    const bool report = !ctx->net.force_f32;
    const bool timed = ctx->prof_level >= 2;
    if (timed) QMRI_HIP(ctx, hipEventRecord(ctx->ev[2], ctx->stream));
    if (report) QMRI_TRY(conv6_act_begin(ctx, (int)ctx->net.layers.size()));
    QMRI_TRY(net_forward_layers(ctx, B));
    if (report) QMRI_TRY(conv6_act_end(ctx));
    if (timed) QMRI_HIP(ctx, hipEventRecord(ctx->ev[3], ctx->stream));
    QMRI_TRY(qmri_prof_chain_finish(ctx));
    if (timed) {
        float ms = 0.f;
        QMRI_HIP(ctx, hipEventSynchronize(ctx->ev[3]));
        QMRI_HIP(ctx, hipEventElapsedTime(&ms, ctx->ev[2], ctx->ev[3]));
        ctx->prof.ms_net_forward += ms; ctx->prof.n_net_forward += 1;
    }
    return QMRI_OK;
}

static int net_forward_layers(qmri_ctx* ctx, int B) {
    NetPlan& p = ctx->net;
    const int nb = p.desc.nb;
    size_t li = 0;
    if (p.desc.arch == QMRI_ARCH_SEQ_CONV) {
        const size_t nl = p.layers.size();
        const PTensor* in = &p.in32;
        const PTensor* bufs[2] = { &p.a[0], &p.t[0] };
        for (size_t l = 0; l < nl; ++l) {
            const PTensor* out = (l == nl - 1) ? &p.out32 : bufs[l & 1];
            QMRI_TRY(conv_launch(ctx, p.layers[l], B, *in, *out, nullptr, nullptr, l != nl - 1));
            in = out;
        }
        return QMRI_OK;
    }
    const bool res_head = qmri_knob(K_RES_HEAD) != 0, res_tail = qmri_knob(K_RES_TAIL) != 0, res_down = qmri_knob(K_RES_DOWN) != 0;
    bool head_done = false, down_done = false;
    if (res_head && p.d_res_xbuf && !p.force_f32 && p.layers.size() >= (size_t)(2 + 2 * nb)) {
        Conv6rRun r;
        r.head = &p.layers[0]; r.head_in = &p.in32; r.res = &p.layers[1]; r.nres = 2 * nb; r.src = &p.x[0]; r.cur = &p.a[0];
        if (res_down) {
            r.down = &p.layers[1 + 2 * nb]; r.down_out = &p.x[1];
            QMRI_TRY(conv6r_try(ctx, r, B, &down_done));
            if (down_done) { head_done = true; li = (size_t)(2 + 2 * nb); }
            r.down = nullptr; r.down_out = nullptr;
        }
        if (!down_done) {
            QMRI_TRY(conv6r_try(ctx, r, B, &head_done));
            if (head_done) li = (size_t)(1 + 2 * nb);
        }
    }
    if (!head_done) QMRI_TRY(conv_launch(ctx, p.layers[li++], B, p.in32, p.x[0], nullptr, nullptr, 0));
    for (int l = 0; l < 3; ++l) {
        if (!(l == 0 && head_done)) QMRI_TRY(run_resblocks(ctx, li, nb, B, p.x[l], p.a[l], p.t[l], nullptr));
        if (!(l == 0 && down_done)) QMRI_TRY(conv_launch(ctx, p.layers[li++], B, p.a[l], p.x[l + 1], nullptr, nullptr, 0));
    }
    QMRI_TRY(run_resblocks(ctx, li, nb, B, p.x[3], p.a[3], p.t[3], &p.x[3]));
    for (int l = 3; l > 0; --l) {
        QMRI_TRY(conv_launch(ctx, p.layers[li++], B, p.a[l], p.a[l - 1], nullptr, nullptr, 0));
        if (l == 1 && res_tail && p.d_res_xbuf && !p.force_f32 && li + (size_t)(2 * nb) < p.layers.size()) {
            bool done = false;
            Conv6rRun r;
            r.res = &p.layers[li]; r.nres = 2 * nb; r.src = &p.a[0]; r.cur = &p.a[0]; r.skip = &p.x[0]; r.tail = &p.layers[li + 2 * nb]; r.tail_out = &p.out32;
            QMRI_TRY(conv6r_try(ctx, r, B, &done));
            if (done) { li += (size_t)(2 * nb + 1); return QMRI_OK; }
        }
        QMRI_TRY(run_resblocks(ctx, li, nb, B, p.a[l - 1], p.a[l - 1], p.t[l - 1], &p.x[l - 1]));
    }
    QMRI_TRY(conv_launch(ctx, p.layers[li++], B, p.a[0], p.out32, nullptr, nullptr, 0));
    return QMRI_OK;
}

int net_forward(qmri_ctx* ctx, int B) {
    NetPlan& p = ctx->net;
    const int st = net_forward_padded(ctx, B);
    if (st == QMRI_OK && p.res_off && p.res_timeouts > 0 && p.res_timeouts < 3 && !p.res_forced_off && ++p.res_clean >= std::max(1, qmri_knob(K_RES_REARM))) {
        p.res_off = false;
        p.res_clean = 0;
    }
    return st;
}

extern "C" int qmri_net_forward_dev(qmri_ctx* ctx, const float* d_in, int B, float* d_out) {
    if (!ctx) return QMRI_ERR_INVALID_ARG;
    QMRI_HIP(ctx, hipSetDevice(ctx->device));
    NetPlan& p = ctx->net;
    if (!p.ready) { qmri_set_error(ctx, "denoiser not set: call qmri_set_denoiser first"); return QMRI_ERR_STATE; }
    QMRI_CHECK_ARG(ctx, d_in && d_out && B >= 1 && B <= p.maxB, "qmri_net_forward_dev arguments / batch > max_batch");
    {
        const size_t hw = (size_t)p.H * p.W * B * sizeof(float);
        const char *a = (const char*)d_in, *b = (const char*)d_out;
        QMRI_CHECK_ARG(ctx, a + hw * p.desc.in_nc <= b || b + hw * p.desc.out_nc <= a, "qmri_net_forward_dev: d_in and d_out must not overlap");
    }
    bool again = false;
    for (int attempt = 0; attempt < 3; ++attempt) {
        QMRI_TRY(ew_launch_pack(ctx, B, p.desc.in_nc, p.H, p.W, d_in, 0, p.in32));
        QMRI_TRY(net_forward(ctx, B));
        QMRI_TRY(ew_launch_unpack(ctx, B, p.desc.out_nc, p.H, p.W, p.out32, p.in32, 0, d_out, 0));
        again = false;
        if (p.sp6 != 2) break;
        QMRI_HIP(ctx, hipStreamSynchronize(ctx->stream));
        QMRI_TRY(net_range_tripped(ctx, again));
        if (!again) break;
    }
    if (again) { qmri_set_error(ctx, "the network's guards asked for a fourth pass (resident-tile hand-off / f16 range): giving up"); return QMRI_ERR_HIP; }
    return QMRI_OK;
}

extern "C" int qmri_debug_conv_resident(qmri_ctx* ctx, int on, int* timeouts_out) {
    if (!ctx) return QMRI_ERR_INVALID_ARG;
    NetPlan& p = ctx->net;
    if (timeouts_out) *timeouts_out = p.res_timeouts;
    if (!p.ready) return QMRI_OK;
    p.res_off = (on == 0);
    p.res_forced_off = (on == 0);
    if (on) { p.res_timeouts = std::min(p.res_timeouts, 2); p.res_clean = 0; }
    p.res_drop = (on == 2) ? 1 : 0;
    return QMRI_OK;
}

extern "C" int qmri_denoiser_scheme(const qmri_ctx* ctx, int* scheme_out, int* fallbacks_out) {
    if (!ctx) return QMRI_ERR_INVALID_ARG;
    if (!ctx->net.ready) return QMRI_ERR_STATE;
    if (scheme_out) *scheme_out = ctx->net.sp6;
    if (fallbacks_out) *fallbacks_out = ctx->net.fallbacks;
    return QMRI_OK;
}

extern "C" int qmri_get_health(const qmri_ctx* ctx, qmri_health* out) {
    if (!ctx || !out) return QMRI_ERR_INVALID_ARG;
    const NetPlan& p = ctx->net;
    std::memset(out, 0, sizeof *out);
    out->denoiser_scheme = p.ready ? p.sp6 : 0;
    out->denoiser_fallbacks = p.ready ? p.fallbacks : 0;
// ... 78 lines not shown
```

### qmri_pnp_recon_poc_amd/csrc/conv6r_kernels.hip

```cpp
#include "conv6_device.h"

namespace {

constexpr int R_MAXL = 10;
constexpr int R_RELU = 1;
constexpr int R_ADD = 2;
constexpr int R_SKIP = 4;
constexpr int R_STORE = 8;
constexpr int R_STORE_WT = 16;
constexpr int R_KEEP = 32;
constexpr int R_DOWN = 128;
constexpr unsigned R_DOWN_STEPB = 2 * 2 * 2 * 64 * 16;
constexpr int R_LOCAL = 256;
constexpr int R_TAIL = 64;
constexpr int R_IH = 18, R_IW = 18, R_IHP = 24;
constexpr int R_NPX = R_IHP * (R_IW - 1) + R_IH;
constexpr int R_CHUNK = 2 * 2 * R_NPX;
constexpr int R_AST = ast6(2);
constexpr int R_SPIN_MAX = 1 << 16;
constexpr int R_SEGT = 86, R_CORT = 6;
constexpr int R_NTRI = 4 * R_SEGT + 4 * R_CORT;
constexpr size_t conv6r_lds() { return (size_t)(NABUF * R_AST + 4 * R_CHUNK) * 16; }

struct Conv6rArgs {
    const float* src; const float* skip;
    const float* radd[R_MAXL]; float* sdst[R_MAXL];
    float* dn_out; int dn_hp, dn_plane;
    float* out; int out_hp, out_plane, out_c;
    int in_planar, in_plane;
    int nch[R_MAXL], kind[R_MAXL];
    unsigned char* xbuf; size_t xbuf_half;
    const uint4* wp[R_MAXL];
    float dh[R_MAXL], dl[R_MAXL];
    int am_layer[R_MAXL];
    int nlayers, hp, plane, tiles_h, tiles_w, xcd;
    int drop;
    int delay;
    unsigned epoch;
    unsigned* range_flag; float* am_slots; int* am_count;
    unsigned long long* stamps;
};

template <int N> __device__ __forceinline__ void gwait_a(u32x4 (&a)[3]) { asm volatile("s_waitcnt vmcnt(%3)" : "+v"(a[0]), "+v"(a[1]), "+v"(a[2]) : "n"(N) : "memory"); }
template <int IMM> __device__ __forceinline__ void gload4r_sc1(f32x4& dst, unsigned off, const void* base) { asm volatile("global_load_dwordx4 %0, %1, %2 offset:%3 sc1" : "=v"(dst) : "v"(off), "s"(base), "n"(IMM) : "memory"); }
template <int IMM> __device__ __forceinline__ void gstore4r(unsigned off, f32x4 x, void* base) { asm volatile("global_store_dwordx4 %0, %1, %2 offset:%3\n\ts_nop 1" ::"v"(off), "v"(x), "s"(base), "n"(IMM) : "memory"); }
template <int IMM> __device__ __forceinline__ void gstore4r_sc1(unsigned off, f32x4 x, void* base) { asm volatile("global_store_dwordx4 %0, %1, %2 offset:%3 sc1\n\ts_nop 1" ::"v"(off), "v"(x), "s"(base), "n"(IMM) : "memory"); }

__device__ __forceinline__ void r_tri_decode(int t, int& seg, int& j) {
    if (t < 4 * R_SEGT) { seg = t / R_SEGT; j = t - seg * R_SEGT; } else { seg = 4 + (t - 4 * R_SEGT) / R_CORT; j = (t - 4 * R_SEGT) - (seg - 4) * R_CORT; }
}
__device__ __forceinline__ int r_seg_base(int seg) { return seg < 4 ? seg * R_SEGT : 4 * R_SEGT + (seg - 4) * R_CORT; }
__device__ __forceinline__ unsigned r_ent_lds(int k, int dw, int dh) {
    const int cb = k >> 1, sp = k & 1;
    return (unsigned)(((cb >> 1) * R_CHUNK + sp * 2 * R_NPX + (cb & 1) * R_NPX + dw * R_IHP + dh) * 16);
}

#define R_STAMP(role, k)                                                                                         \
    do {                                                                                                         \
        if constexpr (STAMP) {                                                                                   \
            if (A.stamps && (threadIdx.x & 255) == 0 && blockIdx.x % 50 == 0 && blockIdx.x / 50 < 4)             \
                A.stamps[(((blockIdx.x / 50) * 2 + (role)) * R_MAXL + l) * 8 + (k)] = wall_clock64();            \
        }                                                                                                        \
    } while (0)
template <bool STAMP>
__global__ __launch_bounds__(NT6) void k_conv6r(const Conv6rArgs A) {
    constexpr int SP = 2, AST = R_AST, IHP = R_IHP, NPX = R_NPX, NAQ = 3;
    static_assert(AST == NAQ * NLD6, "one weight step = three 16-byte entries per loader thread");
    extern __shared__ __align__(16) unsigned char smem[];
    uint4* Abuf = (uint4*)smem;
    uint4* Bt = Abuf + NABUF * AST;
    const int tid = threadIdx.x;
    const int bid = A.xcd ? xcd_remap(blockIdx.x, gridDim.x) : blockIdx.x;
    const int th = bid % A.tiles_h, tw = bid / A.tiles_h;
    const int oh0 = th * 16, ow0 = tw * 16;
    const int nl = A.nlayers;
    const unsigned plane32 = (unsigned)A.plane * 32u;
    const unsigned tile0 = (unsigned)((ow0 * A.hp + oh0) * 32);

    if (tid >= NT6 - NLD6) {
        const int lt = tid - (NT6 - NLD6);
        __builtin_amdgcn_s_setprio(2);
        constexpr unsigned ASTB = AST * 16;
        unsigned aoff[NAQ];
#pragma unroll
        for (int q = 0; q < NAQ; ++q) aoff[q] = (unsigned)((lt + NLD6 * q) * 16);
        int rq_l = 0, rq_s = 0, rq_n = 3 * A.nch[0];
        unsigned rq_stride = ASTB;
        u32x4 srdW = make_srd(A.wp[0]);
#define R_REQ(ra_)                                                                                               \
        {                                                                                                        \
            const unsigned so_ = (unsigned)rq_s * rq_stride;                                                     \
            _Pragma("unroll") for (int q = 0; q < NAQ; ++q) bload4(ra_[q], (q == 2 && rq_stride != ASTB) ? aoff[0] : aoff[q], srdW, so_); \
            if (++rq_s == rq_n) {                                                                                \
                if (rq_l + 1 < nl) { ++rq_l; rq_s = 0; rq_n = 3 * A.nch[rq_l]; srdW = make_srd(A.wp[rq_l]); rq_stride = (A.kind[rq_l] & R_DOWN) ? R_DOWN_STEPB : ASTB; } \
                else rq_s = rq_n - 1;                 \
            }                                                                                                    \
        }
#define R_STORE_A(buf_, ra_)                                                                                     \
        {                                                                                                        \
            uint4* ad = Abuf + (buf_) * AST;                                                                     \
            _Pragma("unroll") for (int q = 0; q < NAQ; ++q) *(uint4*)((unsigned char*)ad + aoff[q]) = __builtin_bit_cast(uint4, ra_[q]); \
        }
        u32x4 ra0[NAQ], ra1[NAQ], ra2[NAQ];
        {
            u32x4 pa1[NAQ];
            R_REQ(ra0) R_REQ(pa1) R_REQ(ra1) R_REQ(ra2)
            if (!A.in_planar) {
                constexpr int NHALF = 8 * R_IH * R_IW * 2, NPRO = (NHALF + NLD6 - 1) / NLD6;
                f32x4 v[NPRO];
                unsigned lo[NPRO];
#pragma unroll
                for (int k = 0; k < NPRO; ++k) {
                    const int idx = lt + NLD6 * k;
                    const bool valid = idx < NHALF;
                    const int idc = valid ? idx : 0, half = idc & 1, item = idc >> 1;
                    const int cb = item / (R_IH * R_IW), px = item - cb * (R_IH * R_IW), dw = px / R_IH, dh = px - dw * R_IH;
                    gload4r(v[k], (unsigned)cb * plane32 + (unsigned)((dw * A.hp + dh) * 32 + 16 * half) + tile0, A.src);
                    lo[k] = valid ? (unsigned)(((cb >> 1) * R_CHUNK + (cb & 1) * NPX + dw * IHP + dh) * 16 + 8 * half) : ~0u;
                }
                static_assert(NPRO == 21, "the wait below names 21 registers");
                asm volatile("s_waitcnt vmcnt(0)"
                             : "+v"(v[0]), "+v"(v[1]), "+v"(v[2]), "+v"(v[3]), "+v"(v[4]), "+v"(v[5]), "+v"(v[6]), "+v"(v[7]), "+v"(v[8]), "+v"(v[9]), "+v"(v[10]),
                               "+v"(v[11]), "+v"(v[12]), "+v"(v[13]), "+v"(v[14]), "+v"(v[15]), "+v"(v[16]), "+v"(v[17]), "+v"(v[18]), "+v"(v[19]), "+v"(v[20])::"memory");
#pragma unroll
                for (int k = 0; k < NPRO; ++k) {
                    uint2 s0, s1;
                    split_pair_h(v[k][0], v[k][1], s0.x, s1.x);
                    split_pair_h(v[k][2], v[k][3], s0.y, s1.y);
                    if (lo[k] != ~0u) {
                        *(uint2*)((unsigned char*)Bt + lo[k]) = s0;
                        *(uint2*)((unsigned char*)Bt + lo[k] + 2 * NPX * 16) = s1;
                    }
                }
            } else {
                constexpr int NIT = 2 * R_IH * R_IW, NQ = (NIT + NLD6 - 1) / NLD6;
                static_assert(NQ == 3, "the wait below names 24 registers");
                const int nin = A.nch[0];
                const unsigned pl4 = (unsigned)A.in_plane * 4u, t0 = (unsigned)((ow0 * A.hp + oh0) * 4);
#pragma unroll 1
                for (int ck = 0; ck < nin; ++ck) {
                    float v[NQ][8];
                    unsigned lo[NQ];
#pragma unroll
                    for (int k = 0; k < NQ; ++k) {
                        const int idx = lt + NLD6 * k;
                        const bool valid = idx < NIT;
                        const int idc = valid ? idx : 0, kh = idc / (R_IH * R_IW), px = idc - kh * (R_IH * R_IW), dw = px / R_IH, dh = px - dw * R_IH;
#pragma unroll
                        for (int j = 0; j < 8; ++j) gload1(v[k][j], (unsigned)(16 * ck + 8 * kh + j) * pl4 + (unsigned)((dw * A.hp + dh) * 4) + t0, A.src);
                        lo[k] = valid ? (unsigned)((ck * R_CHUNK + kh * NPX + dw * IHP + dh) * 16) : ~0u;
                    }
                    if (ck == 0) {
                        const uint4 z = make_uint4(0u, 0u, 0u, 0u);
                        for (int i = lt; i < (4 - nin) * R_CHUNK; i += NLD6) Bt[nin * R_CHUNK + i] = z;
                    }
                    asm volatile("s_waitcnt vmcnt(0)"
                                 : "+v"(v[0][0]), "+v"(v[0][1]), "+v"(v[0][2]), "+v"(v[0][3]), "+v"(v[0][4]), "+v"(v[0][5]), "+v"(v[0][6]), "+v"(v[0][7]), "+v"(v[1][0]),
                                   "+v"(v[1][1]), "+v"(v[1][2]), "+v"(v[1][3]), "+v"(v[1][4]), "+v"(v[1][5]), "+v"(v[1][6]), "+v"(v[1][7]), "+v"(v[2][0]), "+v"(v[2][1]),
                                   "+v"(v[2][2]), "+v"(v[2][3]), "+v"(v[2][4]), "+v"(v[2][5]), "+v"(v[2][6]), "+v"(v[2][7])::"memory");
#pragma unroll
                    for (int k = 0; k < NQ; ++k) {
                        uint4 s0, s1;
                        split_pair_h(v[k][0], v[k][1], s0.x, s1.x);
                        split_pair_h(v[k][2], v[k][3], s0.y, s1.y);
                        split_pair_h(v[k][4], v[k][5], s0.z, s1.z);
                        split_pair_h(v[k][6], v[k][7], s0.w, s1.w);
                        if (lo[k] != ~0u) {
                            *(uint4*)((unsigned char*)Bt + lo[k]) = s0;
                            *(uint4*)((unsigned char*)Bt + lo[k] + 2 * NPX * 16) = s1;
                        }
                    }
                }
            }
            gwait_a<0>(ra0); gwait_a<0>(pa1);
            R_STORE_A(0, ra0) R_STORE_A(1, pa1)
        }
        unsigned p_lds[2][3], p_x[2];
#pragma unroll
        for (int q = 0; q < 2; ++q) {
            const int t = lt + NLD6 * q;
            const bool valid = t < R_NTRI;
            int seg, j;
            r_tri_decode(valid ? t : 0, seg, j);
            const int npx = seg < 4 ? 16 : 1;
#pragma unroll
            for (int i = 0; i < 3; ++i) {
                const int E = 3 * j + i, Ec = (E < npx * 16) ? E : 0, pp = Ec >> 4, k = Ec & 15;
                const int w = (seg == 0) ? 0 : (seg == 1) ? 15 : (seg == 2 || seg == 3) ? pp : (seg < 6 ? 0 : 15);
                const int h = (seg == 0 || seg == 1) ? pp : (seg == 2) ? 0 : (seg == 3) ? 15 : ((seg & 1) ? 15 : 0);
                p_lds[q][i] = r_ent_lds(k, w + 1, h + 1);
            }
            p_x[q] = valid ? (unsigned)((tw * A.tiles_h + th) * (R_NTRI * 64) + t * 16) : ~0u;
        }
        lds_barrier6();
#define R_ITER(k_, rs_, rq_)               \
        {                                                                                                        \
            __builtin_amdgcn_s_setprio(2);                                                                       \
            R_REQ(rq_)                                                                                           \
            __builtin_amdgcn_s_setprio(0);                                                                       \
            gwait_a<2 * NAQ>(rs_);                                                                               \
            R_STORE_A(((k_) + 2) % NABUF, rs_)                                                                   \
            lds_barrier6();                                                                                      \
        }
#pragma unroll 1
        for (int l = 0; l < nl; ++l) {
#pragma unroll 1
            for (int g = 0; g < 3 * A.nch[l]; g += 3) {
                R_ITER(0, ra1, ra0)
                R_ITER(1, ra2, ra1)
                R_ITER(2, ra0, ra2)
            }
            R_STAMP(1, 0);
            if (A.kind[l] & R_TAIL) {
                lds_barrier6();
// ... 300 lines not shown
                bool pend[2] = {c_x[0] != ~0u && !dead, c_x[1] != ~0u && !dead};
                bool ok = false;
                for (int spin = 0; spin < R_SPIN_MAX; ++spin) {
                    u32x4 g[2][4];
#pragma unroll
                    for (int q = 0; q < 2; ++q)
                        if (pend[q]) {
#pragma unroll
                            for (int i = 0; i < 4; ++i) asm volatile("global_load_dwordx4 %0, %1, %2 sc1" : "=v"(g[q][i]) : "v"(c_x[q] + (unsigned)(i * (R_NTRI * 16))), "s"(xb) : "memory");
                        }
                    asm volatile("s_waitcnt vmcnt(0)" : "+v"(g[0][0]), "+v"(g[0][1]), "+v"(g[0][2]), "+v"(g[0][3]), "+v"(g[1][0]), "+v"(g[1][1]), "+v"(g[1][2]), "+v"(g[1][3])::"memory");
#pragma unroll
                    for (int q = 0; q < 2; ++q)
                        if (pend[q]) {
                            unsigned bad = 0;
#pragma unroll
                            for (int i = 0; i < 4; ++i) bad |= (g[q][i][1] ^ thi) | (g[q][i][3] ^ thi);
                            if ((bad >> 16) == 0) {
                                unsigned d[12];
#pragma unroll
                                for (int i = 0; i < 4; ++i) {
                                    d[3 * i] = g[q][i][0];
                                    d[3 * i + 1] = (g[q][i][1] & 0xFFFFu) | (g[q][i][2] << 16);
                                    d[3 * i + 2] = (g[q][i][2] >> 16) | (g[q][i][3] << 16);
                                }
#pragma unroll
                                for (int i = 0; i < 3; ++i)
                                    if (c_lds[q][i] != ~0u) *(uint4*)((unsigned char*)Bt + c_lds[q][i]) = make_uint4(d[4 * i], d[4 * i + 1], d[4 * i + 2], d[4 * i + 3]);
                                pend[q] = false;
                            }
                        }
                    if (!__any(pend[0] || pend[1])) { ok = true; break; }
                    __builtin_amdgcn_s_sleep(1);
                }
                if (!ok && !dead) { dead = true; if (lane == 0 && A.range_flag) atomicOr(A.range_flag, 4u); }
            }
        }
        R_STAMP(0, 5);
        lds_barrier6();
        R_STAMP(0, 6);
    }
}

}

int conv6r_try(qmri_ctx* ctx, const Conv6rRun& run, int B, bool* done) {
    *done = false;
    NetPlan& net = ctx->net;
    hipStreamCaptureStatus cap = hipStreamCaptureStatusNone;
    const bool capturing = hipStreamIsCapturing(ctx->stream, &cap) == hipSuccess && cap != hipStreamCaptureStatusNone;
    const int nres = run.nres, nl = nres + (run.head ? 1 : 0) + (run.tail ? 1 : 0) + (run.down ? 1 : 0);
    if (!qmri_knob(K_CONV_RESIDENT) || capturing || net.res_off || !net.d_res_xbuf || B != 1 || nres < 2 || nl > R_MAXL || (nres & 1) || net.d_stamps) return QMRI_OK;
    if (!run.res || !run.src || !run.cur || (run.head && (!run.head_in || run.skip)) || (run.tail && !run.tail_out) || (run.down && (!run.down_out || run.tail || run.skip))) return QMRI_OK;
    auto is3 = [](const ConvLayer& L) { return (L.kind == CONV_3X3 || L.kind == CONV_3X3N) && L.sp6 == 2 && L.wp6 && L.n_ct6 == 1; };
    for (int l = 0; l < nres; ++l) {
        const ConvLayer& L = run.res[l];
        if (!is3(L) || L.Cin != 64 || L.Cout != 64 || L.nchunk6 != 4) return QMRI_OK;
    }
    const PTensor &src = *run.src, &cur = *run.cur;
    const PTensor* ts[3] = {&src, &cur, run.skip};
    for (const PTensor* t : ts) {
        if (!t) continue;
        if (!t->p || !t->blk || t->Cal < 64 || t->H != src.H || t->W != src.W || t->hp != src.hp || t->h0 != src.h0) return QMRI_OK;
    }
    if (run.head) {
        const ConvLayer& L = *run.head;
        const PTensor& in = *run.head_in;
        if (!is3(L) || L.Cout != 64 || L.nchunk6 < 1 || L.nchunk6 > 2 || L.Cin > 16 * L.nchunk6 || !in.p || in.blk || in.Cal < 16 * L.nchunk6 || in.H != src.H || in.W != src.W || in.hp != src.hp ||
            in.h0 != src.h0 || src.p == cur.p) return QMRI_OK;
    }
    if (run.tail) {
        const ConvLayer& L = *run.tail;
        const PTensor& out = *run.tail_out;
        if (!is3(L) || L.Cin != 64 || L.nchunk6 != 4 || L.Cout > 32 || !out.p || out.blk || out.H != src.H || out.W != src.W ||
            (size_t)out.Cal * out.plane() * 4 >= ((size_t)1 << 31)) return QMRI_OK;
    }
    if (run.down) {
        const ConvLayer& L = *run.down;
        const PTensor& out = *run.down_out;
        if (L.kind != CONV_DOWN || L.sp6 != 2 || !L.wp6 || L.Cin != 64 || L.Cout != 128 || L.nchunk6 != 9 || L.n_ct6 != 2 || !out.p || !out.blk || out.Cal < 128 ||
            out.H * 2 != src.H || out.W * 2 != src.W || (size_t)out.Cal * out.plane() * 4 >= ((size_t)1 << 31)) return QMRI_OK;
    }
    if (src.H % 16 || src.W % 16) return QMRI_OK;
    if ((size_t)src.Cal * src.plane() * 4 >= ((size_t)1 << 31)) return QMRI_OK;
    if (!ctx->conv_ncu) {
        hipDeviceProp_t prop;
        QMRI_HIP(ctx, hipGetDeviceProperties(&prop, ctx->device));
        ctx->conv_ncu = prop.multiProcessorCount;
    }
    const int tiles_h = src.H / 16, tiles_w = src.W / 16, tiles = tiles_h * tiles_w;
    if (tiles > ctx->conv_ncu || tiles != net.res_tiles) return QMRI_OK;
    Conv6rArgs A{};
    A.src = run.head ? run.head_in->fbase() : src.fbase();
    A.in_planar = run.head ? 1 : 0; A.in_plane = run.head ? (int)run.head_in->plane() : 0;
    A.skip = run.skip ? run.skip->fbase() : nullptr;
    if (run.down) { A.dn_out = run.down_out->fbase(); A.dn_hp = run.down_out->hp; A.dn_plane = (int)run.down_out->plane(); }
    if (run.tail) { A.out = run.tail_out->fbase(); A.out_hp = run.tail_out->hp; A.out_plane = (int)run.tail_out->plane(); A.out_c = run.tail->Cout; }
    int l = 0;
    auto put = [&](const ConvLayer& L, int kind, const float* radd, float* sdst) {
        A.wp[l] = reinterpret_cast<const uint4*>(L.wp6);
        A.dh[l] = L.w6_descale; A.dl[l] = L.w6_descale * (1.f / LO_SCALE);
        A.am_layer[l] = conv6_act_slot(ctx, true, L).layer;
        A.nch[l] = L.nchunk6; A.kind[l] = kind; A.radd[l] = radd; A.sdst[l] = sdst;
        ++l;
    };
    if (run.head) put(*run.head, R_STORE | R_KEEP, nullptr, src.fbase());
    for (int r = 0; r < nres; ++r) {
        const bool last = r == nres - 1;
        if (!(r & 1)) put(run.res[r], R_RELU | R_KEEP, nullptr, nullptr);
        else if (!last) put(run.res[r], R_ADD | R_STORE | R_KEEP, (r == 1) ? src.fbase() : cur.fbase(), cur.fbase());
        else if (run.tail) put(run.res[r], R_ADD | (run.skip ? R_SKIP : 0) | R_KEEP, (r == 1) ? src.fbase() : cur.fbase(), nullptr);
        else if (run.down) put(run.res[r], R_ADD | R_KEEP | R_LOCAL, (r == 1) ? src.fbase() : cur.fbase(), nullptr);
        else put(run.res[r], R_ADD | (run.skip ? R_SKIP : 0) | R_STORE_WT, (r == 1) ? src.fbase() : cur.fbase(), cur.fbase());
    }
    if (run.tail) put(*run.tail, R_TAIL, nullptr, nullptr);
    if (run.down) { put(*run.down, R_DOWN, nullptr, nullptr); A.nch[l - 1] = 6; }
    for (int k = l; k < R_MAXL; ++k) { A.wp[k] = A.wp[l - 1]; A.nch[k] = A.nch[l - 1]; A.am_layer[k] = -1; }
    int pub[2] = {0, 0};
    for (int k = 0; k < l; ++k) if ((A.kind[k] & R_KEEP) && !(A.kind[k] & R_LOCAL)) pub[k & 1] += 1;
    if (!pub[0] || !pub[1]) return QMRI_OK;
    A.nlayers = nl; A.hp = src.hp; A.plane = (int)src.plane(); A.tiles_h = tiles_h; A.tiles_w = tiles_w;
    A.xbuf = net.d_res_xbuf; A.xbuf_half = (size_t)tiles * R_NTRI * 64;
    A.xcd = qmri_knob(K_CONV_XCD);
    const int delay = std::max(0, std::min(4096, qmri_knob(K_RES_DELAY)));
    A.epoch = net.res_epoch; A.drop = net.res_drop; A.delay = delay;
    A.range_flag = net.d_range_flag; A.am_slots = net.d_act_slots; A.am_count = net.d_act_count;
    if (!ctx->conv6r_attr) {
        QMRI_HIP(ctx, hipFuncSetAttribute((const void*)k_conv6r<false>, hipFuncAttributeMaxDynamicSharedMemorySize, (int)conv6r_lds()));
        QMRI_HIP(ctx, hipFuncSetAttribute((const void*)k_conv6r<true>, hipFuncAttributeMaxDynamicSharedMemorySize, (int)conv6r_lds()));
        ctx->conv6r_attr = true;
    }
    g_conv6_launch_counter.fetch_add(nl, std::memory_order_relaxed);
    const int stamp_which = qmri_knob(K_RES_STAMPS);
    A.stamps = (stamp_which == 2) == (run.head != nullptr) ? (unsigned long long*)net.d_res_stamps : nullptr;
    hipEvent_t e0 = nullptr, e1 = nullptr;
    double flop = 0.0;
    for (int r = 0; r < nres; ++r) flop += conv_layer_flop(run.res[r], 1, src.H, src.W);
    if (run.head) flop += conv_layer_flop(*run.head, 1, src.H, src.W);
    if (run.tail) flop += conv_layer_flop(*run.tail, 1, src.H, src.W);
    if (run.down) flop += conv_layer_flop(*run.down, 1, src.H, src.W);
    QMRI_TRY(qmri_prof_pair(ctx, &e0, &e1, PROF_CONV3, flop));
    if (A.stamps) k_conv6r<true><<<dim3(tiles), dim3(NT6), conv6r_lds(), ctx->stream>>>(A);
    else if (e0) hipExtLaunchKernelGGL((k_conv6r<false>), dim3(tiles), dim3(NT6), (std::uint32_t)conv6r_lds(), ctx->stream, e0, e1, 0, A);
    else k_conv6r<false><<<dim3(tiles), dim3(NT6), conv6r_lds(), ctx->stream>>>(A);
    QMRI_HIP(ctx, hipGetLastError());
    net.res_epoch += (unsigned)(nl - 1);
    *done = true;
    return QMRI_OK;
}

size_t conv6r_xbuf_bytes(int tiles) { return (size_t)2 * tiles * R_NTRI * 64; }
```

### qmri_pnp_recon_poc_amd/csrc/dc_kernels.hip

```cpp
#include "dc_device.h"
#include "conv6_act.h"

using namespace dcdev;

namespace {

template <int R1, int R2>
__global__ __launch_bounds__(NT) void k_fwd_h(OpDev op, const double2* __restrict__ src, double2* __restrict__ tmp) {
    typedef Plan<R1, R2> P;
    constexpr int N = P::N, L = Cfg<R1, R2>::L;
    __shared__ cd lds[L * P::LINE];
    const int tid = threadIdx.x, b = blockIdx.y;
    const size_t n = (size_t)op.s * N * op.M;
    const size_t base = (size_t)b * n + (size_t)blockIdx.x * L * N;
    for (int i = tid; i < L * N; i += NT) {
        const int line = i / N, nn = i - line * N;
        lds[line * P::LINE + nn] = src[base + i];
    }
    cd out[R2];
    int line2, k1;
    if (fft_lds<R1, R2, true>(lds, L, op.tw_h, out, line2, k1)) {
        const int l = blockIdx.x * L + line2;
        const int c = l / op.M, w = l - c * op.M;
        double2* dst = tmp + (size_t)b * n + (size_t)c * N * op.M + w;
// ... 164 lines not shown

template <int R1, int R2>
__global__ __launch_bounds__(NT) void k_adj_w(OpDev op, const double2* __restrict__ y_in,
                                               double2* __restrict__ tmp) {
    typedef Plan<R1, R2> P;
    constexpr int M = P::N;
    __shared__ cd lds[DC_MAXS * P::LINE];
    __shared__ double vlds[DC_VCAP];
    __shared__ double2 ulds[DC_CH];
    __shared__ unsigned short tlds[DC_CH];
    const int tid = threadIdx.x, b = blockIdx.y, kh = blockIdx.x, s = op.s, N = op.N;
    const size_t n = (size_t)s * N * M;
    const bool v_in_lds = op.T * s <= DC_VCAP;
    if (v_in_lds) for (int i = tid; i < op.T * s; i += NT) vlds[i] = op.Vt[i];
    const size_t mb = (size_t)b * op.m;
    constexpr int NQ = (M * DC_MAXS + NT - 1) / NT;
    double ar[NQ], ai[NQ];
    int e0[NQ], e1[NQ];
#pragma unroll
    for (int q = 0; q < NQ; ++q) {
        const int item = tid + NT * q;
        ar[q] = 0.0; ai[q] = 0.0;
        if (item < M * s) {
            const int kw = item / s;
            e0[q] = op.kptr[kh * M + kw]; e1[q] = op.kptr[kh * M + kw + 1];
        } else { e0[q] = 0; e1[q] = 0; }
    }
    const int r0 = op.kptr[kh * M], r1 = op.kptr[(kh + 1) * M];
    for (int lo = r0; lo < r1; lo += DC_CH) {
        const int hi = (lo + DC_CH < r1) ? lo + DC_CH : r1;
        __syncthreads();
        for (int i = tid; i < hi - lo; i += NT) {
            const int e = lo + i;
            ulds[i] = y_in[mb + op.perm[e]];
            tlds[i] = op.ent[e].t;
        }
        __syncthreads();
#pragma unroll
        for (int q = 0; q < NQ; ++q) {
            const int c = (tid + NT * q) % s;
            const int a0 = (e0[q] > lo) ? e0[q] : lo, a1 = (e1[q] < hi) ? e1[q] : hi;
            double xr = ar[q], xi = ai[q];
            int e = a0;
            for (; e + 4 <= a1; e += 4) {
                double2 u0 = ulds[e - lo], u1 = ulds[e - lo + 1], u2 = ulds[e - lo + 2], u3 = ulds[e - lo + 3];
                const int t0 = tlds[e - lo], t1 = tlds[e - lo + 1], t2 = tlds[e - lo + 2], t3 = tlds[e - lo + 3];
                const double v0 = v_in_lds ? vlds[t0 * s + c] : op.Vt[(size_t)t0 * s + c];
                const double v1 = v_in_lds ? vlds[t1 * s + c] : op.Vt[(size_t)t1 * s + c];
                const double v2 = v_in_lds ? vlds[t2 * s + c] : op.Vt[(size_t)t2 * s + c];
                const double v3 = v_in_lds ? vlds[t3 * s + c] : op.Vt[(size_t)t3 * s + c];
                xr += v0 * u0.x; xi += v0 * u0.y;
                xr += v1 * u1.x; xi += v1 * u1.y;
                xr += v2 * u2.x; xi += v2 * u2.y;
                xr += v3 * u3.x; xi += v3 * u3.y;
            }
            for (; e < a1; ++e) {
                const double2 u0 = ulds[e - lo];
                const int t0 = tlds[e - lo];
                const double v0 = v_in_lds ? vlds[t0 * s + c] : op.Vt[(size_t)t0 * s + c];
                xr += v0 * u0.x; xi += v0 * u0.y;
            }
            ar[q] = xr; ai[q] = xi;
        }
    }
#pragma unroll
    for (int q = 0; q < NQ; ++q) {
        const int item = tid + NT * q;
        if (item < M * s) {
            const int kw = item / s, c = item - kw * s;
            lds[c * P::LINE + kw] = mk(ar[q], -ai[q]);
        }
    }
    cd out[R2];
    int line2, k1;
    if (fft_lds<R1, R2, false>(lds, s, op.tw_w, out, line2, k1)) {
        double2* dst = tmp + (size_t)b * n + ((size_t)line2 * N + kh) * M;
#pragma unroll
        for (int k2 = 0; k2 < R2; ++k2) st_wt(dst + k1 + R1 * k2, out[k2]);
    }
}

template <int R1, int R2, bool CPX>
__global__ __launch_bounds__(NT) void k_adj_h(OpDev op, const double2* __restrict__ tmp, double2* __restrict__ dst,
                                               const double2* __restrict__ u, double* __restrict__ mm) {
    typedef Plan<R1, R2> P;
    constexpr int N = P::N, L = Cfg<R1, R2>::L;
    __shared__ cd lds[L * P::LINE];
    __shared__ double shm[2 * NT / 64];
    const int tid = threadIdx.x, b = blockIdx.y, M = op.M;
    const size_t n = (size_t)op.s * N * M;
    const int l0 = blockIdx.x * L;
    const int c = l0 / M, w0 = l0 - c * M;
    const double2* srcp = tmp + (size_t)b * n + (size_t)c * N * M + w0;
    for (int i = tid; i < L * N; i += NT) {
        const int kh = i / L, line = i - kh * L;
        lds[line * P::LINE + kh] = srcp[(size_t)kh * M + line];
    }
    cd out[R2];
    int line2, k1;
    double lo = INFINITY, hi = -INFINITY;
    if (fft_lds<R1, R2, false>(lds, L, op.tw_h, out, line2, k1)) {
        const double sc = 1.0 / sqrt((double)N * (double)M);
        const size_t g0 = (size_t)b * n + (size_t)(l0 + line2) * N;
        constexpr int RI = CPX ? R2 : 1;
        double ur[R2], ui[RI];
        if (u) {
#pragma unroll
            for (int k2 = 0; k2 < R2; ++k2) {
                ur[k2] = u[g0 + k1 + R1 * k2].x;
                if (CPX) ui[k2 % RI] = u[g0 + k1 + R1 * k2].y;
            }
        }
#pragma unroll
        for (int k2 = 0; k2 < R2; ++k2) {
            const double2 xv = make_double2(out[k2].x * sc, -out[k2].y * sc);
            st_wt(dst + g0 + k1 + R1 * k2, xv);
            if (u) {
                const double v = xv.x + ur[k2]; lo = fmin(lo, v); hi = fmax(hi, v);
                if (CPX) { const double vi = xv.y + ui[k2 % RI]; lo = fmin(lo, vi); hi = fmax(hi, vi); }
            }
        }
    }
    if (u) {
#pragma unroll
        for (int off = 32; off > 0; off >>= 1) { lo = fmin(lo, __shfl_down(lo, off, 64)); hi = fmax(hi, __shfl_down(hi, off, 64)); }
        const int wid = tid >> 6, lane = tid & 63;
        if (lane == 0) { shm[2 * wid] = lo; shm[2 * wid + 1] = hi; }
        __syncthreads();
        if (tid == 0) {
#pragma unroll
            for (int i = 1; i < NT / 64; ++i) { lo = fmin(lo, shm[2 * i]); hi = fmax(hi, shm[2 * i + 1]); }
            mm[((size_t)b * gridDim.x + blockIdx.x) * 2] = lo;
            mm[((size_t)b * gridDim.x + blockIdx.x) * 2 + 1] = hi;
        }
    }
}

__global__ __launch_bounds__(NT) void k_sort_y(OpDev op, LsqrDev ls, const double2* __restrict__ y) {
    __shared__ double red[NT / 64];
    const int b = blockIdx.y;
    const size_t mb = (size_t)b * op.m;
    const int chunk = (op.m + DC_SORT_BLOCKS - 1) / DC_SORT_BLOCKS;
    const int e0 = blockIdx.x * chunk, e1 = min(op.m, e0 + chunk);
    double acc = 0.0;
    for (int e = e0 + threadIdx.x; e < e1; e += NT) {
        const double2 v = y[mb + op.perm[e]];
        ls.yk[mb + e] = v;
        acc += v.x * v.x + v.y * v.y;
    }
    const double tot = block_sum(acc, red);
    if (threadIdx.x == 0) ls.py[(size_t)b * DC_SORT_BLOCKS + blockIdx.x] = tot;
}
__global__ __launch_bounds__(64) void k_sort_y_sum(LsqrDev ls) {
    const int b = blockIdx.x;
    if (threadIdx.x == 0) {
        double tot = 0.0;
        for (int k = 0; k < DC_SORT_BLOCKS; ++k) tot += ls.py[(size_t)b * DC_SORT_BLOCKS + k];
        ls.st[b].ny2 = tot;
    }
}

__global__ __launch_bounds__(NT) void k_prepare_z(LsqrDev ls, size_t n, const double2* __restrict__ v,
                                                   const double2* __restrict__ u, double2* __restrict__ z) {
    __shared__ double red[NT / 64];
    const int b = blockIdx.y;
    const size_t chunk = (n + gridDim.x - 1) / gridDim.x;
    const size_t i0 = (size_t)blockIdx.x * chunk, i1 = (i0 + chunk < n) ? i0 + chunk : n;
    double acc = 0.0;
    for (size_t i = i0 + threadIdx.x; i < i1; i += NT) {
        const double2 a = v[(size_t)b * n + i], c = u[(size_t)b * n + i];
        const double2 zz = make_double2(a.x - c.x, a.y - c.y);
        st_wt(z + (size_t)b * n + i, zz);
        acc += zz.x * zz.x + zz.y * zz.y;
    }
    const double tot = block_sum(acc, red);
    if (threadIdx.x == 0) ls.pz[(size_t)b * ls.nblk_z + blockIdx.x] = tot;
}

template <int R1, int R2>
int launch_fwd_h_t(qmri_ctx* ctx, const OpDev& op, int B, const double2* src, double2* tmp) {
    int gx = 0;
    QMRI_TRY((hpass_grid<R1, R2>(ctx, op, &gx)));
    k_fwd_h<R1, R2><<<dim3(gx, B), dim3(NT), 0, ctx->stream>>>(op, src, tmp);
    QMRI_HIP(ctx, hipGetLastError());
    return QMRI_OK;
}

template <int R1, int R2>
int launch_fwd_w_t(qmri_ctx* ctx, const OpDev& op, const LsqrDev& ls, int mode, int B, const double2* tmp, double2* y_out, double* pdiag,
                   const double2* chat, double rr) {
    dim3 gw(op.N, B), blk(NT);
    hipStream_t st = ctx->stream;
    switch (mode) {
        case DC_FWD_H_ONLY: break;
        case DC_DIAG: k_fwd_w<R1, R2, DC_DIAG><<<gw, blk, 0, st>>>(op, ls, tmp, nullptr, pdiag, nullptr, 0.0); break;
        case DC_SPECTRUM: k_fwd_w<R1, R2, DC_SPECTRUM><<<gw, blk, 0, st>>>(op, ls, tmp, y_out, nullptr, nullptr, 0.0); break;
        case DC_DIRECT: k_fwd_w<R1, R2, DC_DIRECT><<<gw, blk, 0, st>>>(op, ls, tmp, y_out, nullptr, chat, rr); break;
        default: k_fwd_w<R1, R2, DC_PLAIN><<<gw, blk, 0, st>>>(op, ls, tmp, y_out, nullptr, nullptr, 0.0); break;
    }
    QMRI_HIP(ctx, hipGetLastError());
    return QMRI_OK;
}

template <int R1, int R2>
int launch_adj_w_t(qmri_ctx* ctx, const OpDev& op, int B, const double2* y_in, double2* tmp) {
    k_adj_w<R1, R2><<<dim3(op.N, B), dim3(NT), 0, ctx->stream>>>(op, y_in, tmp);
    QMRI_HIP(ctx, hipGetLastError());
    return QMRI_OK;
}

template <int R1, int R2>
int launch_adj_h_t(qmri_ctx* ctx, const OpDev& op, int B, const double2* tmp, double2* dst, const double2* u, double* mm, bool mm_cpx) {
    int gx = 0;
    QMRI_TRY((hpass_grid<R1, R2>(ctx, op, &gx)));
    if (u && mm_cpx) k_adj_h<R1, R2, true><<<dim3(gx, B), dim3(NT), 0, ctx->stream>>>(op, tmp, dst, u, mm);
    else k_adj_h<R1, R2, false><<<dim3(gx, B), dim3(NT), 0, ctx->stream>>>(op, tmp, dst, u, mm);
    QMRI_HIP(ctx, hipGetLastError());
    return QMRI_OK;
}

int launch_fwd(qmri_ctx* ctx, const OpDev& op, const LsqrDev& ls, int mode, int B, const double2* src, double2* tmp, double2* y_out,
               double* pdiag, const double2* chat, double rr) {
    QMRI_TRY(with_plan(ctx, op.N, [&](auto p) { return launch_fwd_h_t<decltype(p)::R1, decltype(p)::R2>(ctx, op, B, src, tmp); }));
    if (mode == DC_FWD_H_ONLY) return QMRI_OK;
    return with_plan(ctx, op.M, [&](auto p) {
        return launch_fwd_w_t<decltype(p)::R1, decltype(p)::R2>(ctx, op, ls, mode, B, tmp, y_out, pdiag, chat, rr);
    });
}

int launch_adj(qmri_ctx* ctx, const OpDev& op, int B, const double2* y_in, double2* tmp, double2* dst, bool skip_w,
               const double2* u = nullptr, double* mm = nullptr, bool mm_cpx = false) {
    if (!skip_w) QMRI_TRY(with_plan(ctx, op.M, [&](auto p) { return launch_adj_w_t<decltype(p)::R1, decltype(p)::R2>(ctx, op, B, y_in, tmp); }));
    return with_plan(ctx, op.N, [&](auto p) { return launch_adj_h_t<decltype(p)::R1, decltype(p)::R2>(ctx, op, B, tmp, dst, u, mm, mm_cpx); });
}

}

bool dc_size_supported(int n) { return qfft::side_supported(n); }

int dc_launch_fwd(qmri_ctx* ctx, const OpDev& op, const LsqrDev& ls, int mode, int B, const double2* src, double2* tmp,
                  double2* y_out, double* pdiag) {
    if (mode != DC_SPECTRUM && mode != DC_FWD_H_ONLY && !op.kptr) {
        qmri_set_error(ctx, "dc_launch_fwd: the operator has no gridded mask (a trajectory operator reached a gridded path; internal)");
        return QMRI_ERR_UNSUPPORTED;
    }
    return launch_fwd(ctx, op, ls, mode, B, src, tmp, y_out, pdiag, nullptr, 0.0);
}

int dc_launch_adj(qmri_ctx* ctx, const OpDev& op, int B, const double2* y_in, double2* tmp, double2* dst) {
    if (!op.kptr) { qmri_set_error(ctx, "dc_launch_adj: the operator has no gridded mask (a trajectory operator reached a gridded path; internal)"); return QMRI_ERR_UNSUPPORTED; }
    return launch_adj(ctx, op, B, y_in, tmp, dst, false);
}

int dc_launch_adj_h(qmri_ctx* ctx, const OpDev& op, int B, const double2* tmp, double2* dst, const double2* u, double* mm, bool mm_cpx) {
    return launch_adj(ctx, op, B, nullptr, const_cast<double2*>(tmp), dst, true, u, mm, mm_cpx);
}

int dc_hpass_blocks(const OpDev& op) {
    switch (op.N) {
#define DC_HPASS_CASE_(n_, a_, b_) case n_: return op.s * op.M / Cfg<a_, b_>::L;
        QFFT_PLANS(DC_HPASS_CASE_)
#undef DC_HPASS_CASE_
        default: return 0;
    }
}

template <int R1, int R2>
static int launch_dual_t(qmri_ctx* ctx, const OpDev& op, int B, const DualArgs& d, const ActCheckArgs& ac, double2* tmp) {
    int gx = 0;
    QMRI_TRY((hpass_grid<R1, R2>(ctx, op, &gx)));
    if (d.complex_tsmi) k_dual_fwd_h<R1, R2, true><<<dim3(gx, B), dim3(NT), 0, ctx->stream>>>(op, d, ac, tmp);
    else k_dual_fwd_h<R1, R2, false><<<dim3(gx, B), dim3(NT), 0, ctx->stream>>>(op, d, ac, tmp);
    QMRI_HIP(ctx, hipGetLastError());
    return QMRI_OK;
}

int dc_launch_dual_fwd_h(qmri_ctx* ctx, const OpDev& op, int B, const DualArgs& d, const ActCheckArgs& ac, double2* tmp) {
    return with_plan(ctx, op.N, [&](auto p) { return launch_dual_t<decltype(p)::R1, decltype(p)::R2>(ctx, op, B, d, ac, tmp); });
}

int dc_launch_direct(qmri_ctx* ctx, const OpDev& op, int B, const double2* z, const double2* chat, double r,
                     double2* tmp, double2* x_out) {
    if (!op.kslot) { qmri_set_error(ctx, "dc_launch_direct: the operator has no gridded mask (a trajectory operator reached a gridded path; internal)"); return QMRI_ERR_UNSUPPORTED; }
    LsqrDev ls{};
    QMRI_TRY(launch_fwd(ctx, op, ls, DC_DIRECT, B, z, tmp, tmp, nullptr, chat, r));
    return launch_adj(ctx, op, B, nullptr, tmp, x_out, true);
}

int dc_launch_sort_y(qmri_ctx* ctx, const OpDev& op, const LsqrDev& ls, int B, const double2* y) {
    if (!op.perm) { qmri_set_error(ctx, "dc_launch_sort_y: the operator has no gridded mask (a trajectory operator reached a gridded path; internal)"); return QMRI_ERR_UNSUPPORTED; }
    k_sort_y<<<dim3(DC_SORT_BLOCKS, B), dim3(NT), 0, ctx->stream>>>(op, ls, y);
    k_sort_y_sum<<<dim3(B), dim3(64), 0, ctx->stream>>>(ls);
    QMRI_HIP(ctx, hipGetLastError());
    return QMRI_OK;
}

int dc_launch_prepare_z(qmri_ctx* ctx, const OpDev& op, const LsqrDev& ls, int B, const double2* v, const double2* u,
                        double2* z) {
    const size_t n = (size_t)op.s * op.N * op.M;
    k_prepare_z<<<dim3(ls.nblk_z, B), dim3(NT), 0, ctx->stream>>>(ls, n, v, u, z);
    QMRI_HIP(ctx, hipGetLastError());
    return QMRI_OK;
}
```

### qmri_pnp_recon_poc_amd/csrc/ew_kernels.hip

```cpp
#include "qmri_internal.h"

namespace {
__device__ __forceinline__ void st_wt(double2* p, double2 v) {
    typedef double d2v_ __attribute__((ext_vector_type(2)));
    const d2v_ t = {v.x, v.y};
    asm volatile("global_store_dwordx4 %0, %1, off sc1\n\ts_nop 1" ::"v"(p), "v"(t) : "memory");
}
}

namespace {

constexpr int NT = 256;

__device__ __forceinline__ double block_sum(double v, double* sh) {
#pragma unroll
    for (int off = 32; off > 0; off >>= 1) v += __shfl_down(v, off, 64);
    const int wid = threadIdx.x >> 6, lane = threadIdx.x & 63;
    __syncthreads();
    if (lane == 0) sh[wid] = v;
    __syncthreads();
    double r = 0.0;
#pragma unroll
    for (int i = 0; i < NT / 64; ++i) r += sh[i];
    return r;
// ... 6 lines not shown
        hi = fmax(hi, __shfl_down(hi, off, 64));
    }
    const int wid = threadIdx.x >> 6, lane = threadIdx.x & 63;
    __syncthreads();
    if (lane == 0) { sh[2 * wid] = lo; sh[2 * wid + 1] = hi; }
    __syncthreads();
    lo = sh[0]; hi = sh[1];
#pragma unroll
    for (int i = 1; i < NT / 64; ++i) { lo = fmin(lo, sh[2 * i]); hi = fmax(hi, sh[2 * i + 1]); }
}

template <bool CPX>
__global__ __launch_bounds__(NT) void k_minmax(size_t n, const double2* __restrict__ x, const double2* __restrict__ u,
                                                double* __restrict__ mm) {
    __shared__ double sh[2 * NT / 64];
    const int b = blockIdx.y;
    const size_t chunk = (n + gridDim.x - 1) / gridDim.x;
    const size_t i0 = (size_t)blockIdx.x * chunk, i1 = (i0 + chunk < n) ? i0 + chunk : n;
    double lo = INFINITY, hi = -INFINITY;
    for (size_t i = i0 + threadIdx.x; i < i1; i += NT) {
        const double v = x[(size_t)b * n + i].x + u[(size_t)b * n + i].x;
        lo = fmin(lo, v); hi = fmax(hi, v);
        if (CPX) {
            const double vi = x[(size_t)b * n + i].y + u[(size_t)b * n + i].y;
            lo = fmin(lo, vi); hi = fmax(hi, vi);
        }
    }
    block_minmax(lo, hi, sh);
    if (threadIdx.x == 0) {
        mm[((size_t)b * gridDim.x + blockIdx.x) * 2] = lo;
        mm[((size_t)b * gridDim.x + blockIdx.x) * 2 + 1] = hi;
    }
}

constexpr int NRQ = 16;
template <bool CPX>
__global__ __launch_bounds__(NT) void k_normalise(size_t n, int plane, int H, int s, int multi_level, double noise_std,
                                                   const double2* __restrict__ x, const double2* __restrict__ u,
                                                   const double* __restrict__ mm, int nblk, double* __restrict__ norm,
                                                   float* __restrict__ in32, int php, int pplane, size_t pbs) {
    __shared__ double sh[2 * NT / 64];
    const int b = blockIdx.y;
    const size_t chunk = (n + gridDim.x - 1) / gridDim.x;
    const size_t i0 = (size_t)blockIdx.x * chunk, i1 = (i0 + chunk < n) ? i0 + chunk : n;
    constexpr int NRI = CPX ? NRQ : 1;
    double xr[NRQ], ur[NRQ], xi[NRI], ui[NRI];
#pragma unroll
    for (int q = 0; q < NRQ; ++q) {
        const size_t i = i0 + threadIdx.x + (size_t)NT * q;
        const size_t ic = (i < i1) ? i : i0;
        xr[q] = x[(size_t)b * n + ic].x; ur[q] = u[(size_t)b * n + ic].x;
        if (CPX) { xi[q % NRI] = x[(size_t)b * n + ic].y; ui[q % NRI] = u[(size_t)b * n + ic].y; }
    }
    double lo = INFINITY, hi = -INFINITY;
    for (int i = threadIdx.x; i < nblk; i += NT) {
        lo = fmin(lo, mm[((size_t)b * nblk + i) * 2]);
        hi = fmax(hi, mm[((size_t)b * nblk + i) * 2 + 1]);
    }
    block_minmax(lo, hi, sh);
    const double range = hi - lo;
    if (blockIdx.x == 0 && threadIdx.x == 0) { norm[2 * b] = lo; norm[2 * b + 1] = range; }
    float* dst = in32 + (size_t)b * pbs;
    auto put = [&](size_t i, double v, double vi) __attribute__((always_inline)) {
        const int c = (int)(i / plane), rem = (int)(i - (size_t)c * plane);
        const int w = rem / H, h = rem - w * H;
        const size_t pi = (size_t)c * pplane + (size_t)(w + 1) * php + h + 1;
        dst[pi] = (float)((v - lo) / range);
        if (CPX) dst[pi + (size_t)s * pplane] = (float)((vi - lo) / range);
    };
#pragma unroll
    for (int q = 0; q < NRQ; ++q) {
        const size_t i = i0 + threadIdx.x + (size_t)NT * q;
        if (i < i1) put(i, xr[q] + ur[q], CPX ? xi[q % NRI] + ui[q % NRI] : 0.0);
    }
    for (size_t i = i0 + threadIdx.x + (size_t)NT * NRQ; i < i1; i += NT)
        put(i, x[(size_t)b * n + i].x + u[(size_t)b * n + i].x, CPX ? x[(size_t)b * n + i].y + u[(size_t)b * n + i].y : 0.0);
    if (multi_level) {
        const int noise_c = CPX ? 2 * s : s;
        const int per = (plane + gridDim.x - 1) / gridDim.x;
        const int c0 = blockIdx.x * per, c1 = (c0 + per < plane) ? c0 + per : plane;
        for (int i = c0 + threadIdx.x; i < c1; i += NT) {
            const int w = i / H, h = i - w * H;
            dst[(size_t)noise_c * pplane + (size_t)(w + 1) * php + h + 1] = (float)noise_std;
        }
    }
}

template <bool CPX>
__global__ __launch_bounds__(NT) void k_unnormalise_dual(size_t n, int plane, int H, int s, int php, int pplane, size_t out_bs,
                                                          size_t in_bs, const float* __restrict__ out32,
                                                          const float* __restrict__ in32, int residual_noise,
                                                          const double* __restrict__ norm, const double2* __restrict__ x,
                                                          double2* __restrict__ u, double2* __restrict__ v,
                                                          double2* __restrict__ z, double* __restrict__ pz) {
    __shared__ double red[NT / 64];
    const int b = blockIdx.y;
    const double lo = norm[2 * b], range = norm[2 * b + 1];
    const size_t chunk = (n + gridDim.x - 1) / gridDim.x;
    const size_t i0 = (size_t)blockIdx.x * chunk, i1 = (i0 + chunk < n) ? i0 + chunk : n;
    const size_t simag = (size_t)s * pplane;
    double acc = 0.0;
    for (size_t i = i0 + threadIdx.x; i < i1; i += NT) {
        const int c = (int)(i / plane), rem = (int)(i - (size_t)c * plane);
        const int w = rem / H, h = rem - w * H;
        const size_t pi = (size_t)c * pplane + (size_t)(w + 1) * php + h + 1;
        float I = out32[(size_t)b * out_bs + pi];
        if (residual_noise) I = in32[(size_t)b * in_bs + pi] - I;
        const double vv = (double)I * range + lo;
        double vi = 0.0;
        if (CPX) {
            float Ii = out32[(size_t)b * out_bs + pi + simag];
            if (residual_noise) Ii = in32[(size_t)b * in_bs + pi + simag] - Ii;
            vi = (double)Ii * range + lo;
        }
        const double2 xv = x[(size_t)b * n + i];
        double2 uv = u[(size_t)b * n + i];
        uv.x = uv.x + xv.x - vv;
        uv.y = uv.y + xv.y - vi;
        st_wt(u + (size_t)b * n + i, uv);
        if (v) v[(size_t)b * n + i] = make_double2(vv, vi);
        const double2 zz = make_double2(vv - uv.x, vi - uv.y);
        st_wt(z + (size_t)b * n + i, zz);
        acc += zz.x * zz.x + zz.y * zz.y;
    }
#pragma unroll
    for (int off = 32; off > 0; off >>= 1) acc += __shfl_down(acc, off, 64);
    const int wid = threadIdx.x >> 6, lane = threadIdx.x & 63;
    if (lane == 0) red[wid] = acc;
    __syncthreads();
    if (threadIdx.x == 0) {
        double r = 0.0;
#pragma unroll
        for (int i = 0; i < NT / 64; ++i) r += red[i];
        pz[(size_t)b * gridDim.x + blockIdx.x] = r;
    }
}

__global__ __launch_bounds__(NT) void k_diffnorm(size_t n, const double2* __restrict__ a, const double2* __restrict__ c,
                                                  double* __restrict__ part) {
    __shared__ double sh[NT / 64];
    const int b = blockIdx.y;
    const size_t chunk = (n + gridDim.x - 1) / gridDim.x;
    const size_t i0 = (size_t)blockIdx.x * chunk, i1 = (i0 + chunk < n) ? i0 + chunk : n;
    double acc = 0.0, ref = 0.0;
    for (size_t i = i0 + threadIdx.x; i < i1; i += NT) {
        const double2 p = a[(size_t)b * n + i], q = c[(size_t)b * n + i];
        const double dx = p.x - q.x, dy = p.y - q.y;
        acc += dx * dx + dy * dy;
        ref += p.x * p.x + p.y * p.y;
    }
    const double t0 = block_sum(acc, sh);
    const double t1 = block_sum(ref, sh);
    if (threadIdx.x == 0) {
        part[((size_t)b * gridDim.x + blockIdx.x) * 2] = t0;
        part[((size_t)b * gridDim.x + blockIdx.x) * 2 + 1] = t1;
    }
}

__global__ __launch_bounds__(NT) void k_diag_final(const LsqrState* __restrict__ st, const double* __restrict__ py, int npy,
                                                    const double* __restrict__ pg, int npg, int have_gt,
                                                    double* __restrict__ diag, int iters_total, int it) {
    __shared__ double sh[NT / 64];
    const int b = blockIdx.x;
    double a = 0.0;
    for (int i = threadIdx.x; i < npy; i += NT) a += py[(size_t)b * npy + i];
    const double ry = block_sum(a, sh);
    double g = 0.0, r = 0.0;
    for (int i = threadIdx.x; i < npg; i += NT) { g += pg[((size_t)b * npg + i) * 2]; r += pg[((size_t)b * npg + i) * 2 + 1]; }
    const double dg = block_sum(g, sh);
    const double rg = block_sum(r, sh);
    if (threadIdx.x == 0) {
        diag[((size_t)b * iters_total + it) * 2] = sqrt(ry) / sqrt(st[b].ny2);
        diag[((size_t)b * iters_total + it) * 2 + 1] = have_gt ? sqrt(dg) / sqrt(rg) : NAN;
    }
}

template <typename T>
__global__ __launch_bounds__(NT) void k_pack(size_t count, int C, int plane, int H, int php, int pplane, size_t pbs,
                                              const T* __restrict__ in, float* __restrict__ out, float scale) {
    const int b = blockIdx.y;
    const size_t i = (size_t)blockIdx.x * NT + threadIdx.x;
    if (i >= count) return;
    const int c = (int)(i / plane), rem = (int)(i - (size_t)c * plane);
    const int w = rem / H, h = rem - w * H;
    out[(size_t)b * pbs + (size_t)c * pplane + (size_t)(w + 1) * php + h + 1] = (float)in[(size_t)b * count + i] * scale;
}

template <typename T>
__global__ __launch_bounds__(NT) void k_unpack(size_t count, int plane, int H, int php, int pplane, size_t out_bs, size_t in_bs,
                                                const float* __restrict__ out32, const float* __restrict__ in32,
                                                int residual_noise, T* __restrict__ out, float scale) {
    const int b = blockIdx.y;
    const size_t i = (size_t)blockIdx.x * NT + threadIdx.x;
    if (i >= count) return;
    const int c = (int)(i / plane), rem = (int)(i - (size_t)c * plane);
    const int w = rem / H, h = rem - w * H;
    const size_t pi = (size_t)c * pplane + (size_t)(w + 1) * php + h + 1;
    float I = out32[(size_t)b * out_bs + pi];
    if (residual_noise) I = in32[(size_t)b * in_bs + pi] - I;
    out[(size_t)b * count + i] = (T)(I * scale);
}

__global__ __launch_bounds__(NT) void k_real_to_complex(size_t count, const double* __restrict__ in, double2* __restrict__ out) {
    const size_t i = (size_t)blockIdx.x * NT + threadIdx.x;
    if (i < count) out[i] = make_double2(in[i], 0.0);
}

}

int ew_launch_minmax_normalise(qmri_ctx* ctx, int B, size_t n, int plane, int H, int s, int multi_level, double noise_std,
                               const double2* x, const double2* u, double* mm, double* norm, int nblk, const PTensor& in32, bool mm_ready,
                               bool complex_tsmi) {
    auto go = [&](auto cpx) {
        constexpr bool CPX = decltype(cpx)::value;
        if (!mm_ready) k_minmax<CPX><<<dim3(nblk, B), dim3(NT), 0, ctx->stream>>>(n, x, u, mm);
        k_normalise<CPX><<<dim3(nblk, B), dim3(NT), 0, ctx->stream>>>(n, plane, H, s, multi_level, noise_std, x, u, mm, nblk, norm, in32.base1(),
                                                                      in32.hp, (int)in32.plane(), in32.batch_stride());
    };
    if (complex_tsmi) go(std::true_type{});
    else go(std::false_type{});
    QMRI_HIP(ctx, hipGetLastError());
    return QMRI_OK;
}

int ew_launch_unnormalise_dual(qmri_ctx* ctx, int B, size_t n, int plane, int H, const PTensor& out32, const PTensor& in32,
                               int residual_noise, const double* norm, const double2* x, double2* u, double2* v, double2* z,
                               double* pz, int nblk_z, int s, bool complex_tsmi) {
    auto go = [&](auto cpx) {
        k_unnormalise_dual<decltype(cpx)::value><<<dim3(nblk_z, B), dim3(NT), 0, ctx->stream>>>(
            n, plane, H, s, out32.hp, (int)out32.plane(), out32.batch_stride(), in32.batch_stride(), out32.base1(), in32.base1(), residual_noise,
            norm, x, u, v, z, pz);
    };
    if (complex_tsmi) go(std::true_type{});
    else go(std::false_type{});
    QMRI_HIP(ctx, hipGetLastError());
    return QMRI_OK;
}

int ew_launch_diag(qmri_ctx* ctx, const OpDev& op, const LsqrDev& ls, int B, const double2* x, const double2* gt,
                   double* pd, double* diag_slot, int iters_total, int it) {
    const size_t n = (size_t)op.s * op.N * op.M;
    double* pg = pd + (size_t)B * op.N;
    if (gt) k_diffnorm<<<dim3(ls.nblk_z, B), dim3(NT), 0, ctx->stream>>>(n, gt, x, pg);
    k_diag_final<<<dim3(B), dim3(NT), 0, ctx->stream>>>(ls.st, pd, op.N, pg, ls.nblk_z, gt ? 1 : 0, diag_slot, iters_total, it);
    QMRI_HIP(ctx, hipGetLastError());
    return QMRI_OK;
}

int ew_launch_pack(qmri_ctx* ctx, int B, int C, int H, int W, const void* src, int src_is_double, const PTensor& dst, float scale) {
    const size_t count = (size_t)C * H * W;
    dim3 grid((unsigned)((count + NT - 1) / NT), B), blk(NT);
    if (src_is_double)
        k_pack<double><<<grid, blk, 0, ctx->stream>>>(count, C, H * W, H, dst.hp, (int)dst.plane(), dst.batch_stride(), (const double*)src, dst.base1(), scale);
    else
        k_pack<float><<<grid, blk, 0, ctx->stream>>>(count, C, H * W, H, dst.hp, (int)dst.plane(), dst.batch_stride(), (const float*)src, dst.base1(), scale);
    QMRI_HIP(ctx, hipGetLastError());
    return QMRI_OK;
}

int ew_launch_unpack(qmri_ctx* ctx, int B, int C, int H, int W, const PTensor& out32, const PTensor& in32, int residual_noise,
                     void* dst, int dst_is_double, float scale) {
    const size_t count = (size_t)C * H * W;
    dim3 grid((unsigned)((count + NT - 1) / NT), B), blk(NT);
    if (dst_is_double)
        k_unpack<double><<<grid, blk, 0, ctx->stream>>>(count, H * W, H, out32.hp, (int)out32.plane(), out32.batch_stride(),
                                                       in32.batch_stride(), out32.base1(), in32.base1(), residual_noise, (double*)dst, scale);
    else
        k_unpack<float><<<grid, blk, 0, ctx->stream>>>(count, H * W, H, out32.hp, (int)out32.plane(), out32.batch_stride(),
                                                      in32.batch_stride(), out32.base1(), in32.base1(), residual_noise, (float*)dst, scale);
    QMRI_HIP(ctx, hipGetLastError());
    return QMRI_OK;
}

__global__ __launch_bounds__(NT) void k_absmax(const float* __restrict__ x, const float* __restrict__ y, size_t n, unsigned* __restrict__ out) {
    unsigned m = 0;
    for (size_t i = (size_t)blockIdx.x * NT + threadIdx.x; i < n; i += (size_t)gridDim.x * NT)
        m = max(m, __float_as_uint(fabsf(y ? x[i] - y[i] : x[i])));
    for (int o = 32; o > 0; o >>= 1) m = max(m, (unsigned)__shfl_down((int)m, o, 64));
    if ((threadIdx.x & 63) == 0 && m) atomicMax(out, m);
}
int ew_launch_absmax(qmri_ctx* ctx, const float* x, const float* y, size_t n, unsigned* d_out) {
    k_absmax<<<dim3(256), dim3(NT), 0, ctx->stream>>>(x, y, n, d_out);
    QMRI_HIP(ctx, hipGetLastError());
    return QMRI_OK;
}

__global__ __launch_bounds__(NT) void k_coil_mul(size_t n, size_t plane, int cnt, const double2* __restrict__ x, const double2* __restrict__ maps, double2* __restrict__ out) {
    const size_t i = (size_t)blockIdx.x * NT + threadIdx.x;
    if (i >= n) return;
    const double2 v = x[i];
    const size_t px = i % plane;
    for (int j = 0; j < cnt; ++j) {
        const double2 c = maps[(size_t)j * plane + px];
        out[(size_t)j * n + i] = make_double2(c.x * v.x - c.y * v.y, c.x * v.y + c.y * v.x);
    }
}
__global__ __launch_bounds__(NT) void k_coil_sum(size_t n, size_t plane, int cnt, const double2* __restrict__ xj, const double2* __restrict__ maps, double2* __restrict__ x, int accumulate) {
    const size_t i = (size_t)blockIdx.x * NT + threadIdx.x;
    if (i >= n) return;
    const size_t px = i % plane;
    double2 a = accumulate ? x[i] : make_double2(0.0, 0.0);
    for (int j = 0; j < cnt; ++j) {
        const double2 c = maps[(size_t)j * plane + px], v = xj[(size_t)j * n + i];
// ... 22 lines not shown
```

### qmri_pnp_recon_poc_amd/csrc/qmri_internal.h

```cpp
#pragma once

#include <hip/hip_runtime.h>
#include <algorithm>
#include <cstdint>
#include <cstdio>
#include <string>
#include <vector>

#include "../../include/qmri.h"

struct qmri_ctx;
void qmri_set_error(qmri_ctx* ctx, const char* fmt, ...);

#define QMRI_HIP(ctx, expr)                                                                       \
    do {                                                                                          \
        hipError_t _e = (expr);                                                                   \
        if (_e != hipSuccess) {                                                                   \
            qmri_set_error((ctx), "%s failed: %s (%s:%d)", #expr, hipGetErrorString(_e), __FILE__, __LINE__); \
            return QMRI_ERR_HIP;                                                                  \
        }                                                                                         \
    } while (0)

#define QMRI_CHECK_ARG(ctx, cond, msg)                                                            \
    do {                                                                                          \
        if (!(cond)) {                                                                            \
            qmri_set_error((ctx), "invalid argument: %s", (msg));                                 \
            return QMRI_ERR_INVALID_ARG;                                                          \
        }                                                                                         \
    } while (0)

#define QMRI_TRY(expr)                                                                            \
    do {                                                                                          \
        int _s = (expr);                                                                          \
        if (_s != QMRI_OK) return _s;                                                             \
    } while (0)

namespace {
template <typename T> struct DevBuf {
    T* p = nullptr;
    DevBuf() = default; DevBuf(DevBuf&& o) noexcept : p(o.p) { o.p = nullptr; }
    ~DevBuf() { if (p) (void)hipFree(p); }
    operator T*() const { return p; }
};
template <typename T> struct PinnedBuf {
    T* p = nullptr;
    PinnedBuf() = default; PinnedBuf(PinnedBuf&& o) noexcept : p(o.p) { o.p = nullptr; }
    ~PinnedBuf() { if (p) (void)hipHostFree(p); }
    operator T*() const { return p; }
};
struct Event {
    hipEvent_t e = nullptr;
    Event() = default; Event(Event&& o) noexcept : e(o.e) { o.e = nullptr; }
    ~Event() { if (e) (void)hipEventDestroy(e); }
    operator hipEvent_t() const { return e; }
};
struct Stream {
    hipStream_t s = nullptr;
    Stream() = default; Stream(Stream&& o) noexcept : s(o.s) { o.s = nullptr; }
    ~Stream() { if (s) (void)hipStreamDestroy(s); }
    operator hipStream_t() const { return s; }
};
template <typename T> int dev_alloc(qmri_ctx* ctx, T** p, size_t count) {
    *p = nullptr;
    hipError_t e = hipMalloc((void**)p, std::max<size_t>(count, 1) * sizeof(T));
    if (e != hipSuccess) { qmri_set_error(ctx, "hipMalloc of %zu bytes failed: %s", count * sizeof(T), hipGetErrorString(e)); return QMRI_ERR_NOMEM; }
    return QMRI_OK;
}
}

enum QmriKnob {
    K_CONV_SCHEME,
    K_CONV_F32,
    K_CONV_WT,
    K_CONV_XCD,
    K_CONV_PERSIST,
    K_CONV_SPLITK,
    K_CONV_MIDCFG, K_CONV_DEEPCFG, K_CONV_DEEPKS,
    K_CONV_RESIDENT,
    K_RES_HEAD, K_RES_TAIL, K_RES_DOWN,
    K_RES_DELAY,
    K_RES_REARM,
    K_RES_STAMPS, K_CONV_STAMPS, K_CONV_STAMP_LAUNCH, K_LSQR_STAMPS,
    K_CONV_MT2, K_CONV_OCC,
    K_FUSE_EW,
    K_LSQR_PERSIST,
    K_LSQR_FOLD,
    K_DICTW_LSP,
    K_VERBOSE,
    K_PACK_GPU,
    K_NUFFT_SEG,
    K_FMAP_FUSE,
    K_FMAP_START,
    K_COUNT
};
int qmri_knob(QmriKnob k);

struct KEntry {
    uint16_t kw;
    uint16_t t;
};


struct OpDev {
    int N, M, s, T, m;
    const double* Vt;
    const KEntry* ent;
    const int32_t* perm;
    const int32_t* kptr;
    const double2* tw_h;
    const double2* tw_w;
    const int32_t* kslot;
    const double* ginv;
};

struct KSample { uint16_t ls, t; };
struct KsGroup { uint16_t ls, b, e, pad; };
struct KsCapsHost { int scap, ecap, gcap, sl, gcapb; };
constexpr KsCapsHost KS_CAPS[4] = {{64, 1024, 32, 8, 96}, {256, 768, 4, 1, 448}, {64, 2560, 32, 8, 144}, {64, 256, 4, 1, 128}};
constexpr int KS_NCAPS = 4;
struct KsUnit { int32_t s0, s1, e0, e1, g0, g1, pad0, pad1; };
struct LsqrState;
struct KsDev {
    int ns, G;
    int caps;
    const KsUnit* unit;
    const KSample* es;
    const KsGroup* grp;
    const int32_t* sgrp;
    LsqrState* st;
    LsqrState* hst;
    double* pu[2];
    double* pv[2];
    double* pinit;
    double* pR;
    const double* pz; int nblk_z;
    double2* cx; double2* cv; double2* cd; double2* cub;
    double2* ut; const double2* yk;
    double2* xhat; double2* zhat;
    double2* xhat_out;
    double* pdiag;
    double sr, tol;
    int maxit, ii, vcap;
    int b0;
    unsigned long long* stamps;
};

struct LsqrScalars {
    double c, s, phibar, normr, norma, factor;
    double thet, rho, phi, beta, alpha;
    double ua, ub, uc, ue;
};
struct LsqrState {
    LsqrScalars sc[2];
    double n2b, tolb;
    double ny2;
    double R;
    double ue_final;
    int32_t iter, done, flag, pad;
};

enum { DC_PLAIN = 0, DC_FWD_H_ONLY = 1, DC_DIAG = 3, DC_DIRECT = 4, DC_SPECTRUM = 5 };
constexpr int DC_SORT_BLOCKS = 64;

struct LsqrDev {
    LsqrState* st;
    double* pz;
    double2* yk;
    double* py;
    int nblk_z;
};

enum ConvKind { CONV_3X3 = 0, CONV_DOWN = 1, CONV_UP = 2, CONV_3X3N = 3 };
struct ConvLayer {
    ConvKind kind;
    int Cin, Cout;
    int cin_pad, n_ct;
    int MT;
    float* wp;
    size_t wp_floats;
    void* d_tab;
    int tab_B, tab_MT;
    void* wp6 = nullptr;
    int sp6 = 2;
    float w6_descale = 1.f;
    int nchunk6 = 0, n_ct6 = 0;
    int nsteps6s = 0;
    int index = -1;
    size_t w_off = 0;
};

struct PTensor {
    float* p = nullptr;
    int C = 0, Cal = 0, H = 0, W = 0;
    int hp = 0, h0 = 1;
    bool blk = false;
    float* base1() const { return p + (h0 - 1); }
    float* fbase() const { return p + (size_t)(h0 - 1) * (blk ? 8 : 1); }
    size_t plane() const { return (size_t)hp * (W + 2); }
    size_t batch_stride() const { return (size_t)Cal * plane(); }
};

struct ActCheckArgs { const float* slots; int* count; float* ref; int record; unsigned* range_flag; unsigned* host_words; int nlayers; };

struct NetPlan {
    qmri_net_desc desc{};
    int H = 0, W = 0, maxB = 0;
    std::vector<ConvLayer> layers;
    PTensor x[4], a[4], t[4];
    PTensor in32;
    PTensor out32;
    std::vector<float*> allocs;
    unsigned* d_counter = nullptr;
    unsigned counter_base = 0;
    bool counter_by_memset = false;
    bool force_f32 = false;
    unsigned* d_range_flag = nullptr;
    unsigned* h_range_flag = nullptr;
    int h_range_words = 0;
    int fallbacks = 0;
    float* d_act_slots = nullptr;
    int* d_act_count = nullptr;
    float* d_act_ref = nullptr;
    int act_cap = 0;
    bool act_on = false, act_record = false;
    bool act_defer = false, act_pending_valid = false;
    ActCheckArgs act_pending{};
    int sp6 = 2;
    bool blk_ok = false;
    int interior_fmt = -1;
    std::vector<float> w_host;
    float* d_wflat = nullptr;
    const float* w_begin = nullptr;
    std::vector<float> w_max;
    float* d_c6part = nullptr;
    size_t c6part_floats = 0;
    void* d_stamps = nullptr;
    unsigned char* d_res_xbuf = nullptr;
    int res_tiles = 0;
    unsigned res_epoch = 0;
    bool res_off = false;
    bool res_forced_off = false;
    double setup_ms[3] = {0, 0, 0};
    int res_timeouts = 0;
    int res_clean = 0;
    int res_drop = 0;
    double* d_io = nullptr; size_t io_cap = 0;
    void* d_res_stamps = nullptr;
    bool ready = false;
};

struct McWork {
    double2 *ut = nullptr;
    double2 *ub = nullptr, *v = nullptr, *d = nullptr, *t = nullptr;
    double2 *scr = nullptr;
    double* part = nullptr;
    LsqrState* st = nullptr;
    LsqrState* hst = nullptr;
    size_t cap_sl = 0, cap_img = 0;
    int pred = 8;
    int pred_cg = 8;
    double2 *sm = nullptr, *sy = nullptr, *sx = nullptr, *sz = nullptr;
    size_t stage_sl = 0, stage_img = 0;
};
void mc_free_work(McWork& w);
int mc_ensure_staging(qmri_ctx* ctx, int B, int ncoil);
int mc_adjoint_batch_dev(qmri_ctx* ctx, int B, int ncoil, const double2* d_maps, const double2* d_y, double2* d_x);
int mc_ensure_work(qmri_ctx* ctx, int B, int ncoil);
int mc_launch_coil_mul(qmri_ctx* ctx, int ncoil, int g0, int cnt, const double2* x, const double2* maps, const LsqrState* st, double2* out);
int mc_launch_coil_sum(qmri_ctx* ctx, int ncoil, int g0, int cnt, const double2* xj, const double2* maps, const LsqrState* st, double2* t);
int qmri_lsqr_mc_batch_dev(qmri_ctx* ctx, int B, int ncoil, const double2* d_maps, const double2* d_y, const double2* d_z, double r, double tol, int maxit,
                           double2* d_x, int32_t* iters_out, int32_t* flags_out);

struct CcWork {
    double2 *part = nullptr, *R = nullptr, *X = nullptr, *L = nullptr, *U = nullptr, *W = nullptr;
    size_t part_cap = 0, R_cap = 0, X_cap = 0, L_cap = 0, U_cap = 0, W_cap = 0;
    double2* hK = nullptr; size_t hK_cap = 0;
    int* hbad = nullptr;
    bool lds_attr = false;
    double2 *psi = nullptr, *sy = nullptr, *sm = nullptr, *oy = nullptr, *om = nullptr;
    size_t psi_cap = 0, sy_cap = 0, sm_cap = 0, oy_cap = 0, om_cap = 0;
};
void cc_free_work(CcWork& w);
int cc_ensure_staging(qmri_ctx* ctx, size_t ny, size_t nm, size_t nyo, size_t nmo);
int cc_compress_dev(qmri_ctx* ctx, int B, int ncoil, const double2* d_y, const double2* d_maps, const double2* d_psi, const qmri_cc_params& prm,
                    int* nv_out, double2* d_yout, double2* d_mout, double2* d_Wout, double* eig_out);
int cc_eig_host(qmri_ctx* ctx, int n, const double2* A, double* lam, double2* U);
int cc_choose_nv(int n, const double* lam, double energy);
int cc_batch_param_error(int ncoil, const qmri_cc_params* p, std::string* msg);
// ... 57 lines not shown
};
struct NufftHost {
    double* d_u = nullptr; double* d_ph = nullptr; int32_t* d_t = nullptr; int32_t* d_perm = nullptr; int32_t* d_list = nullptr;
    NuSeg* d_seg = nullptr; NuRed* d_red = nullptr; double* d_dp = nullptr; double2* d_r = nullptr;
    double2* d_g = nullptr; double2* d_grid = nullptr; double2* d_part = nullptr;
    double2* d_ones = nullptr;
    int w = 0, nseg = 0, nred = 0, nslot = 0;
    double beta = 0.0;
    double2* d_khat = nullptr;
    bool khat_ready = false;
    double* d_w = nullptr;
    bool w_set = false;
    double2* d_pm = nullptr;
    double2* d_bl = nullptr;
    size_t pm_cap = 0, bl_cap = 0;
    int fm_L = 0;
    bool fm_set = false;
    std::vector<double> fm_f, fm_ts, fm_p;
    double fm_f0 = 0.0, fm_fmin = 0.0, fm_fmax = 0.0, fm_tmin = 0.0, fm_tmax = 0.0;
    int fm_nbins = 0;
    double2* d_khat_fm = nullptr;
    double2* d_pm_n = nullptr;
    double2* d_xs = nullptr;
    int fmn_L = 0;
    bool fmn_plain = false;
    bool fmn_ready = false;
};
void spiral_points(int S, std::vector<double>& theta, std::vector<double>& rad);
constexpr double SPIRAL_DELTA = 3.14159265358979323846 / 180.0 * 7.5;
int nufft_launch_fwd(qmri_ctx* ctx, int B, const double2* x, double2* y);
int nufft_launch_adj(qmri_ctx* ctx, int B, const double2* y, double2* x);
int nufft_launch_adj_plain(qmri_ctx* ctx, int B, const double2* y, double2* x);
int nufft_launch_adj_w(qmri_ctx* ctx, int B, const double2* y, double2* x);
int dcf_weights_dev(qmri_ctx* ctx, int niter, double tol, double kappa, double* d_w_out, qmri_dcf_info* info);
struct OffresFit { double fit_max, fit_rms; };
int offres_phase_maps_dev(qmri_ctx* ctx, int L, size_t plane, const double* d_f, double f0, const double* d_tauhat, double2* d_pm);
int offres_coefficients_dev(qmri_ctx* ctx, int L, int nbins, bool exact, const double2* d_hist, const double2* d_G, const double2* d_chol,
                            const double* d_ts, double f0, double2* d_bl, OffresFit* fit);
int offres_refuse_toeplitz(qmri_ctx* ctx, const char* what);
int offres_ncoefficients_dev(qmri_ctx* ctx, int L, int nb, const double2* d_dh, const double2* d_G, const double2* d_Qw, const double* d_U,
                             const double* d_ts, double* d_c, OffresFit* fit);
void offres_drop_normal(NufftHost& h);
int nufft_check_gridded(qmri_ctx* ctx, const char* what, const char* instead);
void nufft_free(NufftHost& h);
bool nufft_kernel_ok(int w);
NufftDev nufft_dev_view(const qmri_ctx* ctx);
int nufft_launch_ramps(qmri_ctx* ctx, int B, const double2* x, double2* g);
int nufft_launch_unramps(qmri_ctx* ctx, int B, const double2* g, double2* x);
int nufft_launch_ramps_pm(qmri_ctx* ctx, int B, const double2* x, double2* g, const double2* pm);
int nufft_launch_unramps_pm(qmri_ctx* ctx, int B, const double2* g, double2* x, const double2* pm, bool acc);
int toep_prepare(qmri_ctx* ctx);
int toep_build_weighted(qmri_ctx* ctx, const double* d_c, double2* khat);
int toep_apply(qmri_ctx* ctx, int B, const double2* x, double2* out);
int qmri_cg_toep_batch_dev(qmri_ctx* ctx, int B, int ncoil, const double2* d_maps, const double2* d_y, const double2* d_z, double r, double tol, int maxit,
                           double2* d_x, int32_t* iters_out, int32_t* flags_out);
int mc_xupdate_dev(qmri_ctx* ctx, int solver, int B, int ncoil, const double2* d_maps, const double2* d_y, const double2* d_z, double r, double tol, int maxit,
                   double2* d_x, int32_t* iters_out, int32_t* flags_out);
int toep_check_solver(qmri_ctx* ctx, int solver);

enum { OP_GRIDDED = 0, OP_NUFFT = 1 };
struct OpHost {
    int kind = OP_GRIDDED;
    NufftHost nu;
    bool ready = false;
    int N = 0, M = 0, s = 0, T = 0, m = 0, maxB = 0, nsampled = 0;
    double* d_Vt = nullptr; KEntry* d_ent = nullptr; int32_t* d_perm = nullptr; int32_t* d_kptr = nullptr;
    double2* d_tw = nullptr; int32_t* d_kslot = nullptr; double* d_ginv = nullptr;
    double2* d_coils = nullptr; int ncoil = 0;
    McWork mc;
    KsDev ks{};
    bool xhat_valid = false;
    double ginv_r = -1.0;
    std::vector<double> V;
    std::vector<int32_t> frame_ptr, kidx, kptr_h, perm_h;
    std::vector<KEntry> ent_h;
    double2* d_tmp = nullptr;
    double2* d_xa = nullptr; double2* d_xb = nullptr;
    double2* d_ya = nullptr;
    LsqrDev ls{};
    double2* d_x = nullptr; double2* d_u = nullptr; double2* d_vv = nullptr; double2* d_z = nullptr;
    double2* d_chat = nullptr;
    double* d_mm = nullptr;
    double* d_norm = nullptr;
    double* d_diag = nullptr;
    double* d_pd = nullptr;
    int32_t* h_flags = nullptr;
    LsqrState* h_state = nullptr;
    LsqrState* h_ring = nullptr;
    size_t h_ring_cap = 0;
};

struct DictHost {
    bool ready = false;
    int K = 0, s = 0, Q = 0, ntiles = 0;
    int wide = 0, G8 = 0;
    float* d_pack = nullptr;
    float* d_xp = nullptr; size_t xp_cap = 0;
    float4* d_win = nullptr; size_t win_cap = 0;
    int slots_w = 0;
    float* d_normD = nullptr; float* d_lut = nullptr;
    float4* d_part = nullptr; size_t part_cap = 0;
    int slots = 0, slots_f = 0;
    uint4* d_pack16 = nullptr;
    int* d_gmax = nullptr; size_t gmax_cap = 0;
    float marg_coef = 0.f;
    int filter_on = 1; float margin_scale = 1.f;
    int G = 0, gtiles_max = 0;
    std::vector<int> gtile_h;
    float* d_gpack = nullptr; uint4* d_gpack16 = nullptr;
    int* d_gptr = nullptr; int* d_gtile = nullptr; double* d_gval = nullptr;
    int* d_gwork = nullptr; size_t gwork_cap = 0;
    int slots_g = 0, slots_gf = 0;
};

struct qmri_ctx {
    int device = 0;
    hipStream_t own_stream = nullptr;
    hipStream_t stream = nullptr;
    std::string err;
    OpHost op;
    NetPlan net;
    DictHost dict;
    CcWork cc;
    int prof_level = 0;
    qmri_profile prof{};
    hipEvent_t ev[4] = {nullptr, nullptr, nullptr, nullptr};
    hipEvent_t ev_state = nullptr;
    std::vector<hipEvent_t> chain;
    size_t chain_n = 0;
    std::vector<int> chain_kind;
    std::vector<double> chain_flop;
    bool conv6_attr[4][2] = {};
    bool conv6p_attr[2][3] = {{false, false, false}, {false, false, false}};
    bool conv6r_attr = false;
    bool ks_lds_attr[2] = {false, false};
    int lsqr_pred = 20;
    int ks_persist = -1;
    int ks_persist_cap = -1;
    void* d_ks_gran = nullptr;
    unsigned ks_tag = 16;
    int ks_timeouts = 0;
    int admm_repeats = 0;
    std::vector<hipEvent_t> marks;
    std::vector<int> mark_kind;
    size_t marks_n = 0;
    double last_call_ms[4] = {0, 0, 0, 0};
    double last_call_wall_ms = 0;
    LlrState llr;
    bool llr_lds_attr[3] = {false, false, false};
    int conv_ncu = 0;
    int conv_occ[4][2] = {{0, 0}, {0, 0}, {0, 0}, {0, 0}};
};

OpDev qmri_opdev(const qmri_ctx* ctx);

bool dc_size_supported(int N);
int dc_launch_fwd(qmri_ctx* ctx, const OpDev& op, const LsqrDev& ls, int mode, int B, const double2* src, double2* tmp,
                  double2* y_out, double* pdiag);
int dc_launch_adj(qmri_ctx* ctx, const OpDev& op, int B, const double2* y_in, double2* tmp, double2* dst);
int dc_launch_adj_h(qmri_ctx* ctx, const OpDev& op, int B, const double2* tmp, double2* dst, const double2* u = nullptr,
                    double* mm = nullptr, bool mm_cpx = false);
struct DualArgs {
    const float* out32; const float* in32; int php, pplane; size_t out_bs, in_bs; int residual_noise;
    const double* norm; const double2* x; double2* u; double* pz;
    int complex_tsmi;
};
int dc_hpass_blocks(const OpDev& op);
struct LsqrFuse { int z_hpass_nblk = 0; const double2* mm_u = nullptr; double* mm = nullptr; bool mm_cpx = false; };
int dc_launch_dual_fwd_h(qmri_ctx* ctx, const OpDev& op, int B, const DualArgs& d, const ActCheckArgs& ac, double2* tmp);
void qmri_free_operator(qmri_ctx* ctx);
void qmri_free_net(qmri_ctx* ctx);
void qmri_free_dict(qmri_ctx* ctx);
int qmri_prepare_direct(qmri_ctx* ctx, double r);
int qmri_lsqr_run(qmri_ctx* ctx, int B, const double2* d_z, double r, double tol, int maxit, double2* d_x,
                  int32_t* iters_out, int32_t* flag_out, double* pdiag, LsqrState* hslot, bool* deferred, const LsqrFuse* fuse);
__attribute__((visibility("hidden"))) int net_forward(qmri_ctx* ctx, int B);
__attribute__((visibility("hidden"))) int net_range_tripped(qmri_ctx* ctx, bool& tripped);
__attribute__((visibility("hidden"))) bool host_range_tripped(const NetPlan& p);
int ks_launch_init(qmri_ctx* ctx, const OpDev& op, const KsDev& ks, int B, const double2* hpass_tmp = nullptr, bool first_step = true);
int ks_launch_iter(qmri_ctx* ctx, const OpDev& op, const KsDev& ks, int B);
int ks_launch_final(qmri_ctx* ctx, const OpDev& op, const KsDev& ks, int B, double2* tmp);
int ks_persist_plan(qmri_ctx* ctx, const OpDev& op, const KsDev& ks, int B, int* per_launch);
int ks_launch_persist(qmri_ctx* ctx, const OpDev& op, const KsDev& ks, int B, void* gran, unsigned tag0, bool init_here, bool* ran);
size_t ks_gran_bytes(int G, int B);
int ks_lds_fits(qmri_ctx* ctx, int N, int s, int M, int vcap, int caps, bool* ok);
int dc_launch_direct(qmri_ctx* ctx, const OpDev& op, int B, const double2* z, const double2* chat, double r,
                     double2* tmp, double2* x_out);
int dc_launch_sort_y(qmri_ctx* ctx, const OpDev& op, const LsqrDev& ls, int B, const double2* y);
int dc_launch_prepare_z(qmri_ctx* ctx, const OpDev& op, const LsqrDev& ls, int B, const double2* v, const double2* u,
                        double2* z);
int ew_launch_minmax_normalise(qmri_ctx* ctx, int B, size_t n, int plane, int H, int s, int multi_level, double noise_std,
                               const double2* x, const double2* u, double* mm, double* norm, int nblk, const PTensor& in32, bool mm_ready = false,
                               bool complex_tsmi = false);
int ew_launch_unnormalise_dual(qmri_ctx* ctx, int B, size_t n, int plane, int H, const PTensor& out32, const PTensor& in32,
                               int residual_noise, const double* norm, const double2* x, double2* u, double2* v, double2* z,
                               double* pz, int nblk_z, int s = 0, bool complex_tsmi = false);
int ew_launch_diag(qmri_ctx* ctx, const OpDev& op, const LsqrDev& ls, int B, const double2* x, const double2* gt,
                   double* pd, double* diag_slot, int iters_total, int it);
int ew_launch_pack(qmri_ctx* ctx, int B, int C, int H, int W, const void* src, int src_is_double, const PTensor& dst, float scale = 1.f);
int ew_launch_absmax(qmri_ctx* ctx, const float* x, const float* y, size_t n, unsigned* d_out);
int ew_launch_unpack(qmri_ctx* ctx, int B, int C, int H, int W, const PTensor& out32, const PTensor& in32, int residual_noise,
                     void* dst, int dst_is_double, float scale = 1.f);
int ew_launch_real_to_complex(qmri_ctx* ctx, size_t count, const double* in, double2* out);
int ew_launch_coil_mul(qmri_ctx* ctx, size_t n, size_t plane, int cnt, const double2* x, const double2* maps, double2* out);
int ew_launch_coil_sum(qmri_ctx* ctx, size_t n, size_t plane, int cnt, const double2* xj, const double2* maps, double2* x, int accumulate);

int conv_launch(qmri_ctx* ctx, ConvLayer& L, int B, const PTensor& in, const PTensor& out, const PTensor* add1,
                const PTensor* add2, int relu_out);
int conv_cin_pad(ConvKind kind, int Cin);
enum { PROF_CONV3 = 0, PROF_CONV2 = 1, PROF_LSQR = 2, PROF_TV = 3 };
int qmri_prof_pair(qmri_ctx* ctx, hipEvent_t* start, hipEvent_t* stop, int kind = PROF_CONV3, double flop = 0.0);
int qmri_prof_chain_finish(qmri_ctx* ctx, long count = -1);
bool conv6_enabled();
int conv6_act_begin(qmri_ctx* ctx, int nlayers);
int conv6_act_end(qmri_ctx* ctx);
int conv6_default_sp();
bool conv6_weights_fit_f16(const float* w, size_t n);
void conv6_plan_pack(ConvLayer& L, const float* w, std::vector<uint16_t>& packed);
int conv6_pack_dev(qmri_ctx* ctx, ConvLayer& L, const float* d_w, float wmax);
int conv6s_pack_dev(qmri_ctx* ctx, ConvLayer& L, const float* d_w, float wmax);
int conv_pack_weights_dev(qmri_ctx* ctx, ConvLayer& L, const float* d_w);
int conv6_launch(qmri_ctx* ctx, const ConvLayer& L, int B, const PTensor& in, const PTensor& out, const PTensor* add1,
                 const PTensor* add2, int relu_out);
struct Conv6rRun {
    const ConvLayer* head = nullptr; const PTensor* head_in = nullptr;
    const ConvLayer* res = nullptr; int nres = 0;
    const PTensor* src = nullptr; const PTensor* cur = nullptr; const PTensor* skip = nullptr;
    const ConvLayer* tail = nullptr; const PTensor* tail_out = nullptr;
    const ConvLayer* down = nullptr; const PTensor* down_out = nullptr;
};
int conv6r_try(qmri_ctx* ctx, const Conv6rRun& run, int B, bool* done);
size_t conv6r_xbuf_bytes(int tiles);
void conv6s_plan_pack(ConvLayer& L, const float* w, std::vector<uint16_t>& packed);
bool conv6s_usable(const ConvLayer& L, const PTensor& in, const PTensor& out);
int conv6s_launch(qmri_ctx* ctx, const ConvLayer& L, int B, const PTensor& in, const PTensor& out);
size_t conv_pack_weights(const ConvLayer& L, const float* w_src, std::vector<float>& packed);
void conv_plan_layer(ConvLayer& L, ConvKind kind, int Cin, int Cout);

int dict_launch(qmri_ctx* ctx, const double2* d_X, int Npix, float* d_qmap, float* d_pd, float* d_mt, int32_t* d_dm, float2* d_xfit);
int dict_scratch(qmri_ctx* ctx, void** buf, size_t* cap, size_t need_bytes);
int dict_launch_xfit(qmri_ctx* ctx, const float4* win, int Npix, float2* d_xfit);
struct DictGroupView;
int dict_group_pixel_width(const qmri_ctx* ctx);
int dict_launch_grouped(qmri_ctx* ctx, const double2* d_X, int Npix, const DictGroupView& gv, int nslot_tiles, float* d_qmap, float* d_pd, float* d_mt,
                        int32_t* d_dm, float4* win);
int dictg_set_groups(qmri_ctx* ctx, int G, const int32_t* group_ptr, const double* group_val);
void dictg_free(qmri_ctx* ctx);
int dictg_launch(qmri_ctx* ctx, const double2* d_X, int Npix, const double* d_sel, float* d_qmap, float* d_pd, float* d_mt, int32_t* d_dm, int32_t* d_grp,
                 float2* d_xfit);
int dict_launch_merge(qmri_ctx* ctx, const float4* part, int P, int Npix, float* d_qmap, float* d_pd, float* d_mt, int32_t* d_dm, float4* win);
int dictw_pack_dictionary(qmri_ctx* ctx, const float* D_host, int K, int s);
int dictw_launch(qmri_ctx* ctx, const double2* d_X, int Npix, float* d_qmap, float* d_pd, float* d_mt, int32_t* d_dm, float4* win);
```

Baseline: 821.0 ADMM iters/s.

## Fuse min-max normalisation into LSQR adjoint pass and resident denoiser head

The LSQR final adjoint H-pass now writes the real part of v = x+u into a new buffer alongside the per-block min/max partials. The separate min-max normalise kernel is then skipped, and the resident conv6r head reads v directly, reduces the partials and normalises while staging its input tile. When the head path is not taken, a lighter normalise_v kernel runs instead. This removes a full elementwise launch and a pass over the TSMI per ADMM iteration, at the cost of an extra buffer write in the adjoint and more complex head staging code with hand-written waits.

```diff
diff --git a/include/qmri.h b/include/qmri.h
--- a/include/qmri.h
+++ b/include/qmri.h
@@ -298,6 +298,7 @@
     int64_t n_lsqr_launches;
     double ms_net_forward;
     int64_t n_net_forward;
+    int64_t n_ew_launches;
 } qmri_profile;
 int qmri_profile_enable(qmri_ctx* ctx, int level);
 int qmri_profile_get(qmri_ctx* ctx, qmri_profile* out, int reset);
diff --git a/qmri_pnp_recon_poc_amd/_lib.py b/qmri_pnp_recon_poc_amd/_lib.py
--- a/qmri_pnp_recon_poc_amd/_lib.py
+++ b/qmri_pnp_recon_poc_amd/_lib.py
@@ -125,7 +125,8 @@
                 ("n_conv3x3", C.c_int64), ("lsqr_iters", C.c_int64), ("admm_iters", C.c_int64),
                 ("ms_tv_iter", C.c_double), ("n_tv_iter", C.c_int64),
                 ("flop_conv3x3", C.c_double), ("ms_conv2x2", C.c_double), ("n_conv2x2", C.c_int64), ("flop_conv2x2", C.c_double),
-                ("ms_lsqr_kernels", C.c_double), ("n_lsqr_launches", C.c_int64), ("ms_net_forward", C.c_double), ("n_net_forward", C.c_int64)]
+                ("ms_lsqr_kernels", C.c_double), ("n_lsqr_launches", C.c_int64), ("ms_net_forward", C.c_double), ("n_net_forward", C.c_int64),
+                ("n_ew_launches", C.c_int64)]
 
 
 class Health(C.Structure):
diff --git a/qmri_pnp_recon_poc_amd/csrc/api_admm.cpp b/qmri_pnp_recon_poc_amd/csrc/api_admm.cpp
--- a/qmri_pnp_recon_poc_amd/csrc/api_admm.cpp
+++ b/qmri_pnp_recon_poc_amd/csrc/api_admm.cpp
@@ -103,15 +103,18 @@
 
 struct DenoiserStep { int B; const qmri_admm_params* prm; int multi; bool cpx; const double2* d_x; StageTimer* tm; };
 
-static int admm_to_net(qmri_ctx* ctx, const DenoiserStep& d, int mm_nblk, bool mm_ready, bool copy_range_flag) {
+static int admm_to_net(qmri_ctx* ctx, const DenoiserStep& d, int mm_nblk, bool mm_ready, bool copy_range_flag, bool vr_ready = false) {
     OpHost& o = ctx->op;
     NetPlan& net = ctx->net;
     const size_t plane = (size_t)o.N * o.M;
     if (d.tm) d.tm->start();
-    QMRI_TRY(ew_launch_minmax_normalise(ctx, d.B, plane * o.s, (int)plane, o.N, o.s, d.multi, d.prm->noise_std, d.d_x, o.d_u, o.d_mm, o.d_norm, mm_nblk, net.in32,
-                                        mm_ready, d.cpx));
+    if (vr_ready) net.norm_req = {true, o.d_vr, o.d_mm, o.d_norm, mm_nblk, o.s, d.multi, d.prm->noise_std};
+    else QMRI_TRY(ew_launch_minmax_normalise(ctx, d.B, plane * o.s, (int)plane, o.N, o.s, d.multi, d.prm->noise_std, d.d_x, o.d_u, o.d_mm, o.d_norm, mm_nblk, net.in32,
+                                             mm_ready, d.cpx));
     if (d.tm) { d.tm->stop(ctx->prof.ms_elementwise); d.tm->start(); }
-    QMRI_TRY(net_forward(ctx, d.B));
+    const int st_fwd = net_forward(ctx, d.B);
+    net.norm_req.pending = false;
+    QMRI_TRY(st_fwd);
     if (copy_range_flag && net.sp6 == 2 && (int)net.layers.size() + 1 > net.h_range_words)
         QMRI_HIP(ctx, hipMemcpyAsync(net.h_range_flag, net.d_range_flag, sizeof(unsigned), hipMemcpyDeviceToHost, ctx->stream));
     if (d.tm) d.tm->stop(ctx->prof.ms_denoiser);
@@ -290,6 +293,7 @@
     }
     const bool fused = qmri_knob(K_FUSE_EW) != 0 && prm->solver == QMRI_SOLVER_LSQR && !llr;
     const int hb = dc_hpass_blocks(op);
+    const bool fuse_norm = fused && !cpx && o.d_vr && qmri_knob(K_FUSE_NORM) != 0;
     bool z_in_tmp = false;
     struct DeferGuard { NetPlan& n; ~DeferGuard() { n.act_defer = false; n.act_pending_valid = false; } } defer_guard{net};
     net.act_defer = fused;
@@ -300,7 +304,7 @@
         if (prm->solver == QMRI_SOLVER_LSQR) {
             bool deferred = false;
             LsqrFuse lf;
-            if (fused) { lf.z_hpass_nblk = z_in_tmp ? hb : 0; lf.mm_u = o.d_u; lf.mm = o.d_mm; lf.mm_cpx = cpx; }
+            if (fused) { lf.z_hpass_nblk = z_in_tmp ? hb : 0; lf.mm_u = o.d_u; lf.mm = o.d_mm; lf.mm_cpx = cpx; lf.mm_vr = fuse_norm ? o.d_vr : nullptr; }
             QMRI_TRY(qmri_lsqr_run(ctx, B, o.d_z, prm->gamma, prm->cg_tol, prm->cg_maxit, o.d_x, it_b.data(), nullptr,
                                    diag ? o.d_pd : nullptr,
                                    o.h_ring + (size_t)it * B, &deferred, &lf));
@@ -320,7 +324,7 @@
         }
         if (!fused) QMRI_TRY(admm_denoiser_step(ctx, step, !llr, it));
         else {
-            QMRI_TRY(admm_to_net(ctx, step, hb, true, true));
+            QMRI_TRY(admm_to_net(ctx, step, hb, true, true, fuse_norm));
             tm.start();
             const DualArgs da = {net.out32.base1(), net.in32.base1(), net.out32.hp, (int)net.out32.plane(), net.out32.batch_stride(), net.in32.batch_stride(),
                                  net.desc.residual_noise, o.d_norm, o.d_x, o.d_u, o.ls.pz, cpx ? 1 : 0};
diff --git a/qmri_pnp_recon_poc_amd/csrc/api_core.cpp b/qmri_pnp_recon_poc_amd/csrc/api_core.cpp
--- a/qmri_pnp_recon_poc_amd/csrc/api_core.cpp
+++ b/qmri_pnp_recon_poc_amd/csrc/api_core.cpp
@@ -19,7 +19,7 @@
     {"conv_resident", 1}, {"res_head", 1}, {"res_tail", 1}, {"res_down", 1}, {"res_delay", 24}, {"res_rearm", 64},
     {"res_stamps", 0}, {"conv_stamps", 0}, {"conv_stamp_launch", -1}, {"lsqr_stamps", 0},
     {"conv_mt2", 1024}, {"conv_occ", 2},
-    {"fuse_ew", 1}, {"lsqr_persist", 1}, {"lsqr_fold", 1}, {"dictw_lsp", 2}, {"verbose", 0},
+    {"fuse_ew", 1}, {"fuse_norm", 1}, {"lsqr_persist", 1}, {"lsqr_fold", 1}, {"dictw_lsp", 2}, {"verbose", 0},
     {"pack_gpu", 1}, {"nufft_seg", NU_SEG},
     {"fmap_fuse", 0}, {"fmap_start", 0},
 };
@@ -130,7 +130,7 @@
                      (void*)o.ks.unit, (void*)o.ks.es, (void*)o.ks.grp, (void*)o.ks.sgrp,
                      o.ks.pu[0], o.ks.pu[1], o.ks.pv[0], o.ks.pv[1], o.ks.pinit, o.ks.pR, o.ks.cx, o.ks.cv, o.ks.cd, o.ks.cub,
                      o.ks.ut, o.ks.xhat, o.ks.zhat, o.ks.xhat_out, o.ks.stamps,
-                     o.d_x, o.d_u, o.d_vv, o.d_z, o.d_chat, o.d_mm, o.d_norm, o.d_diag, o.d_pd, o.d_coils };
+                     o.d_x, o.d_u, o.d_vv, o.d_z, o.d_chat, o.d_mm, o.d_norm, o.d_vr, o.d_diag, o.d_pd, o.d_coils };
     for (void* p : ptrs) free_dev(p);
     if (o.h_state) (void)hipHostFree(o.h_state);
     if (o.h_ring) (void)hipHostFree(o.h_ring);
@@ -450,6 +450,7 @@
     QMRI_TRY(dev_alloc(ctx, &o.d_chat, B * n));
     QMRI_TRY(dev_alloc(ctx, &o.d_mm, B * npart * 2));
     QMRI_TRY(dev_alloc(ctx, &o.d_norm, B * 2));
+    QMRI_TRY(dev_alloc(ctx, &o.d_vr, B * n));
     QMRI_TRY(dev_alloc(ctx, &o.d_pd, B * ((size_t)N + 2 * ls.nblk_z)));
     QMRI_HIP(ctx, hipMemset(ls.st, 0, B * sizeof(LsqrState)));
     QMRI_HIP(ctx, hipHostMalloc((void**)&o.h_state, B * sizeof(LsqrState), hipHostMallocDefault));
@@ -663,6 +664,7 @@
     const double2* const mm_u = fuse ? fuse->mm_u : nullptr;
     double* const mm = fuse ? fuse->mm : nullptr;
     const bool mm_cpx = fuse && fuse->mm_cpx;
+    double* const mm_vr = fuse ? fuse->mm_vr : nullptr;
     if (z_fused && !o.xhat_valid) { qmri_set_error(ctx, "qmri_lsqr_run: a transformed z needs the spectrum of x (internal)"); return QMRI_ERR_STATE; }
     if (!o.xhat_valid) QMRI_TRY(dc_launch_fwd(ctx, op, o.ls, DC_SPECTRUM, B, d_x, o.d_tmp, ks.xhat, nullptr));
     if (z_fused) ks.nblk_z = fuse->z_hpass_nblk;
@@ -685,7 +687,7 @@
         if (persisted) {
             ctx->ks_tag += 2u * (unsigned)(maxit + 2);
             QMRI_TRY(ks_launch_final(ctx, op, ks, B, o.d_tmp));
-            QMRI_TRY(dc_launch_adj_h(ctx, op, B, o.d_tmp, d_x, mm_u, mm, mm_cpx));
+            QMRI_TRY(dc_launch_adj_h(ctx, op, B, o.d_tmp, d_x, mm_u, mm, mm_cpx, mm_vr));
             if (deferred) {
                 *deferred = true;
                 std::swap(o.ks.xhat, o.ks.xhat_out);
@@ -722,7 +724,7 @@
         launched += std::max(nthis, 0);
         QMRI_HIP(ctx, hipEventRecord(ctx->ev_state, ctx->stream));
         QMRI_TRY(ks_launch_final(ctx, op, ks, B, o.d_tmp));
-        QMRI_TRY(dc_launch_adj_h(ctx, op, B, o.d_tmp, d_x, mm_u, mm, mm_cpx));
+        QMRI_TRY(dc_launch_adj_h(ctx, op, B, o.d_tmp, d_x, mm_u, mm, mm_cpx, mm_vr));
         QMRI_HIP(ctx, hipEventSynchronize(ctx->ev_state));
         all_done = true;
         for (int b = 0; b < B; ++b) all_done = all_done && hs[b].done;
diff --git a/qmri_pnp_recon_poc_amd/csrc/api_net.cpp b/qmri_pnp_recon_poc_amd/csrc/api_net.cpp
--- a/qmri_pnp_recon_poc_amd/csrc/api_net.cpp
+++ b/qmri_pnp_recon_poc_amd/csrc/api_net.cpp
@@ -395,6 +395,16 @@
     NetPlan& p = ctx->net;
     const int nb = p.desc.nb;
     size_t li = 0;
+    const bool norm_req = p.norm_req.pending;
+    p.norm_req.pending = false;
+    auto normalise_v = [&]() {
+        const NormReq& q = p.norm_req;
+        const size_t plane = (size_t)p.H * p.W;
+        return ew_launch_normalise_v(ctx, B, plane * q.s, (int)plane, p.H, q.s, q.multi, q.noise_std, q.v, q.mm, q.norm, q.nblk, p.in32);
+    };
+    const bool norm_in_head = norm_req && B == 1 && p.desc.arch == QMRI_ARCH_UNETRES && !p.desc.residual_noise && p.norm_req.nblk <= NORM_REQ_MAX_NBLK &&
+                              (size_t)p.norm_req.s * p.H * p.W * 8 < ((size_t)1 << 31);
+    if (norm_req && !norm_in_head) QMRI_TRY(normalise_v());
     if (p.desc.arch == QMRI_ARCH_SEQ_CONV) {
         const size_t nl = p.layers.size();
         const PTensor* in = &p.in32;
@@ -411,6 +421,7 @@
     if (res_head && p.d_res_xbuf && !p.force_f32 && p.layers.size() >= (size_t)(2 + 2 * nb)) {
         Conv6rRun r;
         r.head = &p.layers[0]; r.head_in = &p.in32; r.res = &p.layers[1]; r.nres = 2 * nb; r.src = &p.x[0]; r.cur = &p.a[0];
+        if (norm_in_head) r.head_norm = &p.norm_req;
         if (res_down) {
             r.down = &p.layers[1 + 2 * nb]; r.down_out = &p.x[1];
             QMRI_TRY(conv6r_try(ctx, r, B, &down_done));
@@ -422,6 +433,7 @@
             if (head_done) li = (size_t)(1 + 2 * nb);
         }
     }
+    if (norm_in_head && !head_done) QMRI_TRY(normalise_v());
     if (!head_done) QMRI_TRY(conv_launch(ctx, p.layers[li++], B, p.in32, p.x[0], nullptr, nullptr, 0));
     for (int l = 0; l < 3; ++l) {
         if (!(l == 0 && head_done)) QMRI_TRY(run_resblocks(ctx, li, nb, B, p.x[l], p.a[l], p.t[l], nullptr));
diff --git a/qmri_pnp_recon_poc_amd/csrc/conv6r_kernels.hip b/qmri_pnp_recon_poc_amd/csrc/conv6r_kernels.hip
--- a/qmri_pnp_recon_poc_amd/csrc/conv6r_kernels.hip
+++ b/qmri_pnp_recon_poc_amd/csrc/conv6r_kernels.hip
@@ -28,6 +28,7 @@
     float* dn_out; int dn_hp, dn_plane;
     float* out; int out_hp, out_plane, out_c;
     int in_planar, in_plane;
+    const double* nv; const double* nmm; double* nnorm; int n_nblk, n_s, n_H, n_W, n_multi; float n_noise;
     int nch[R_MAXL], kind[R_MAXL];
     unsigned char* xbuf; size_t xbuf_half;
     const uint4* wp[R_MAXL];
@@ -130,6 +131,93 @@
                     if (lo[k] != ~0u) {
                         *(uint2*)((unsigned char*)Bt + lo[k]) = s0;
                         *(uint2*)((unsigned char*)Bt + lo[k] + 2 * NPX * 16) = s1;
+                    }
+                }
+            } else if (A.in_planar == 2) {
+                constexpr int NIT = 2 * R_IH * R_IW, NQ = (NIT + NLD6 - 1) / NLD6, NMQ = NORM_REQ_MAX_NBLK / 256;
+                static_assert(NQ == 3 && NMQ == 3, "the waits below name 24 + 12 registers");
+                typedef double d2v_ __attribute__((ext_vector_type(2)));
+                const int nin = A.nch[0], ns = A.n_s, nH = A.n_H, nW = A.n_W, lane = lt & 63;
+                const unsigned cpl8 = (unsigned)(nH * nW) * 8u;
+                double nlo = 0.0, nrange = 0.0;
+#pragma unroll 1
+                for (int ck = 0; ck < nin; ++ck) {
+                    double v[NQ][8];
+                    d2v_ pm[4][NMQ];
+                    unsigned lo[NQ];
+                    bool inside[NQ];
+#pragma unroll
+                    for (int k = 0; k < NQ; ++k) {
+                        const int idx = lt + NLD6 * k;
+                        const bool valid = idx < NIT;
+                        const int idc = valid ? idx : 0, kh = idc / (R_IH * R_IW), px = idc - kh * (R_IH * R_IW), dw = px / R_IH, dh = px - dw * R_IH;
+                        const int gw = ow0 + dw - 1, gh = oh0 + dh - 1;
+                        inside[k] = valid && gw >= 0 && gw < nW && gh >= 0 && gh < nH;
+                        const unsigned poff = inside[k] ? (unsigned)((gw * nH + gh) * 8) : 0u;
+#pragma unroll
+                        for (int j = 0; j < 8; ++j) {
+                            const int c = 16 * ck + 8 * kh + j;
+                            v[k][j] = 0.0;
+                            if (inside[k] && c < ns) asm volatile("global_load_dwordx2 %0, %1, %2" : "=v"(v[k][j]) : "v"((unsigned)c * cpl8 + poff), "s"(A.nv) : "memory");
+                        }
+                        lo[k] = valid ? (unsigned)((ck * R_CHUNK + kh * NPX + dw * IHP + dh) * 16) : ~0u;
+                    }
+                    if (ck == 0) {
+#pragma unroll
+                        for (int w = 0; w < 4; ++w)
+#pragma unroll
+                            for (int q = 0; q < NMQ; ++q) {
+                                const int i = 64 * w + lane + 256 * q;
+                                pm[w][q] = d2v_{INFINITY, -INFINITY};
+                                if (i < A.n_nblk) asm volatile("global_load_dwordx4 %0, %1, %2" : "=v"(pm[w][q]) : "v"((unsigned)i * 16u), "s"(A.nmm) : "memory");
+                            }
+                        const uint4 z = make_uint4(0u, 0u, 0u, 0u);
+                        for (int i = lt; i < (4 - nin) * R_CHUNK; i += NLD6) Bt[nin * R_CHUNK + i] = z;
+                    }
+                    asm volatile("s_waitcnt vmcnt(0)"
+                                 : "+v"(v[0][0]), "+v"(v[0][1]), "+v"(v[0][2]), "+v"(v[0][3]), "+v"(v[0][4]), "+v"(v[0][5]), "+v"(v[0][6]), "+v"(v[0][7]), "+v"(v[1][0]),
+                                   "+v"(v[1][1]), "+v"(v[1][2]), "+v"(v[1][3]), "+v"(v[1][4]), "+v"(v[1][5]), "+v"(v[1][6]), "+v"(v[1][7]), "+v"(v[2][0]), "+v"(v[2][1]),
+                                   "+v"(v[2][2]), "+v"(v[2][3]), "+v"(v[2][4]), "+v"(v[2][5]), "+v"(v[2][6]), "+v"(v[2][7])::"memory");
+                    if (ck == 0) {
+                        asm volatile("" : "+v"(pm[0][0]), "+v"(pm[0][1]), "+v"(pm[0][2]), "+v"(pm[1][0]), "+v"(pm[1][1]), "+v"(pm[1][2]), "+v"(pm[2][0]), "+v"(pm[2][1]),
+                                          "+v"(pm[2][2]), "+v"(pm[3][0]), "+v"(pm[3][1]), "+v"(pm[3][2])::"memory");
+                        double hi = 0.0;
+#pragma unroll
+                        for (int w = 0; w < 4; ++w) {
+                            double a = INFINITY, b = -INFINITY;
+#pragma unroll
+                            for (int q = 0; q < NMQ; ++q)
+                                if (64 * w + lane + 256 * q < A.n_nblk) { a = fmin(a, pm[w][q][0]); b = fmax(b, pm[w][q][1]); }
+#pragma unroll
+                            for (int off = 32; off > 0; off >>= 1) { a = fmin(a, __shfl_down(a, off, 64)); b = fmax(b, __shfl_down(b, off, 64)); }
+                            a = __shfl(a, 0, 64); b = __shfl(b, 0, 64);
+                            if (w == 0) { nlo = a; hi = b; } else { nlo = fmin(nlo, a); hi = fmax(hi, b); }
+                        }
+                        nrange = hi - nlo;
+                        if (blockIdx.x == 0 && lt == 0) { A.nnorm[0] = nlo; A.nnorm[1] = nrange; }
+                    }
+#pragma unroll
+                    for (int k = 0; k < NQ; ++k) {
+                        const int idx = lt + NLD6 * k, kh = (idx < NIT ? idx : 0) / (R_IH * R_IW);
+                        float f[8];
+#pragma unroll
+                        for (int j = 0; j < 8; ++j) {
+                            const int c = 16 * ck + 8 * kh + j;
+                            f[j] = 0.f;
+                            if (inside[k]) {
+                                if (c < ns) f[j] = (float)((v[k][j] - nlo) / nrange);
+                                else if (A.n_multi && c == ns) f[j] = A.n_noise;
+                            }
+                        }
+                        uint4 s0, s1;
+                        split_pair_h(f[0], f[1], s0.x, s1.x);
+                        split_pair_h(f[2], f[3], s0.y, s1.y);
+                        split_pair_h(f[4], f[5], s0.z, s1.z);
+                        split_pair_h(f[6], f[7], s0.w, s1.w);
+                        if (lo[k] != ~0u) {
+                            *(uint4*)((unsigned char*)Bt + lo[k]) = s0;
+                            *(uint4*)((unsigned char*)Bt + lo[k] + 2 * NPX * 16) = s1;
+                        }
                     }
                 }
             } else {
@@ -596,6 +684,9 @@
             out.H * 2 != src.H || out.W * 2 != src.W || (size_t)out.Cal * out.plane() * 4 >= ((size_t)1 << 31)) return QMRI_OK;
     }
     if (src.H % 16 || src.W % 16) return QMRI_OK;
+    const NormReq* nr = run.head ? run.head_norm : nullptr;
+    if (nr && (!nr->v || !nr->mm || !nr->norm || nr->nblk < 1 || nr->nblk > NORM_REQ_MAX_NBLK || nr->s + nr->multi != run.head->Cin ||
+               (size_t)nr->s * src.H * src.W * 8 >= ((size_t)1 << 31))) return QMRI_OK;
     if ((size_t)src.Cal * src.plane() * 4 >= ((size_t)1 << 31)) return QMRI_OK;
     if (!ctx->conv_ncu) {
         hipDeviceProp_t prop;
@@ -606,7 +697,8 @@
     if (tiles > ctx->conv_ncu || tiles != net.res_tiles) return QMRI_OK;
     Conv6rArgs A{};
     A.src = run.head ? run.head_in->fbase() : src.fbase();
-    A.in_planar = run.head ? 1 : 0; A.in_plane = run.head ? (int)run.head_in->plane() : 0;
+    A.in_planar = run.head ? (nr ? 2 : 1) : 0; A.in_plane = run.head ? (int)run.head_in->plane() : 0;
+    if (nr) { A.nv = nr->v; A.nmm = nr->mm; A.nnorm = nr->norm; A.n_nblk = nr->nblk; A.n_s = nr->s; A.n_H = src.H; A.n_W = src.W; A.n_multi = nr->multi; A.n_noise = (float)nr->noise_std; }
     A.skip = run.skip ? run.skip->fbase() : nullptr;
     if (run.down) { A.dn_out = run.down_out->fbase(); A.dn_hp = run.down_out->hp; A.dn_plane = (int)run.down_out->plane(); }
     if (run.tail) { A.out = run.tail_out->fbase(); A.out_hp = run.tail_out->hp; A.out_plane = (int)run.tail_out->plane(); A.out_c = run.tail->Cout; }
diff --git a/qmri_pnp_recon_poc_amd/csrc/dc_kernels.hip b/qmri_pnp_recon_poc_amd/csrc/dc_kernels.hip
--- a/qmri_pnp_recon_poc_amd/csrc/dc_kernels.hip
+++ b/qmri_pnp_recon_poc_amd/csrc/dc_kernels.hip
@@ -270,7 +270,7 @@
 
 template <int R1, int R2, bool CPX>
 __global__ __launch_bounds__(NT) void k_adj_h(OpDev op, const double2* __restrict__ tmp, double2* __restrict__ dst,
-                                               const double2* __restrict__ u, double* __restrict__ mm) {
+                                               const double2* __restrict__ u, double* __restrict__ mm, double* __restrict__ vr) {
     typedef Plan<R1, R2> P;
     constexpr int N = P::N, L = Cfg<R1, R2>::L;
     __shared__ cd lds[L * P::LINE];
@@ -305,6 +305,7 @@
             st_wt(dst + g0 + k1 + R1 * k2, xv);
             if (u) {
                 const double v = xv.x + ur[k2]; lo = fmin(lo, v); hi = fmax(hi, v);
+                if (!CPX && vr) vr[g0 + k1 + R1 * k2] = v;
                 if (CPX) { const double vi = xv.y + ui[k2 % RI]; lo = fmin(lo, vi); hi = fmax(hi, vi); }
             }
         }
@@ -398,11 +399,11 @@
 }
 
 template <int R1, int R2>
-int launch_adj_h_t(qmri_ctx* ctx, const OpDev& op, int B, const double2* tmp, double2* dst, const double2* u, double* mm, bool mm_cpx) {
+int launch_adj_h_t(qmri_ctx* ctx, const OpDev& op, int B, const double2* tmp, double2* dst, const double2* u, double* mm, bool mm_cpx, double* vr) {
     int gx = 0;
     QMRI_TRY((hpass_grid<R1, R2>(ctx, op, &gx)));
-    if (u && mm_cpx) k_adj_h<R1, R2, true><<<dim3(gx, B), dim3(NT), 0, ctx->stream>>>(op, tmp, dst, u, mm);
-    else k_adj_h<R1, R2, false><<<dim3(gx, B), dim3(NT), 0, ctx->stream>>>(op, tmp, dst, u, mm);
+    if (u && mm_cpx) k_adj_h<R1, R2, true><<<dim3(gx, B), dim3(NT), 0, ctx->stream>>>(op, tmp, dst, u, mm, nullptr);
+    else k_adj_h<R1, R2, false><<<dim3(gx, B), dim3(NT), 0, ctx->stream>>>(op, tmp, dst, u, mm, u ? vr : nullptr);
     QMRI_HIP(ctx, hipGetLastError());
     return QMRI_OK;
 }
@@ -417,9 +418,9 @@
 }
 
 int launch_adj(qmri_ctx* ctx, const OpDev& op, int B, const double2* y_in, double2* tmp, double2* dst, bool skip_w,
-               const double2* u = nullptr, double* mm = nullptr, bool mm_cpx = false) {
+               const double2* u = nullptr, double* mm = nullptr, bool mm_cpx = false, double* vr = nullptr) {
     if (!skip_w) QMRI_TRY(with_plan(ctx, op.M, [&](auto p) { return launch_adj_w_t<decltype(p)::R1, decltype(p)::R2>(ctx, op, B, y_in, tmp); }));
-    return with_plan(ctx, op.N, [&](auto p) { return launch_adj_h_t<decltype(p)::R1, decltype(p)::R2>(ctx, op, B, tmp, dst, u, mm, mm_cpx); });
+    return with_plan(ctx, op.N, [&](auto p) { return launch_adj_h_t<decltype(p)::R1, decltype(p)::R2>(ctx, op, B, tmp, dst, u, mm, mm_cpx, vr); });
 }
 
 }
@@ -440,8 +441,8 @@
     return launch_adj(ctx, op, B, y_in, tmp, dst, false);
 }
 
-int dc_launch_adj_h(qmri_ctx* ctx, const OpDev& op, int B, const double2* tmp, double2* dst, const double2* u, double* mm, bool mm_cpx) {
-    return launch_adj(ctx, op, B, nullptr, const_cast<double2*>(tmp), dst, true, u, mm, mm_cpx);
+int dc_launch_adj_h(qmri_ctx* ctx, const OpDev& op, int B, const double2* tmp, double2* dst, const double2* u, double* mm, bool mm_cpx, double* vr) {
+    return launch_adj(ctx, op, B, nullptr, const_cast<double2*>(tmp), dst, true, u, mm, mm_cpx, vr);
 }
 
 int dc_hpass_blocks(const OpDev& op) {
diff --git a/qmri_pnp_recon_poc_amd/csrc/ew_kernels.hip b/qmri_pnp_recon_poc_amd/csrc/ew_kernels.hip
--- a/qmri_pnp_recon_poc_amd/csrc/ew_kernels.hip
+++ b/qmri_pnp_recon_poc_amd/csrc/ew_kernels.hip
@@ -112,6 +112,50 @@
         for (int i = c0 + threadIdx.x; i < c1; i += NT) {
             const int w = i / H, h = i - w * H;
             dst[(size_t)noise_c * pplane + (size_t)(w + 1) * php + h + 1] = (float)noise_std;
+        }
+    }
+}
+
+__global__ __launch_bounds__(NT) void k_normalise_v(size_t n, int plane, int H, int s, int multi_level, double noise_std,
+                                                     const double* __restrict__ vin, const double* __restrict__ mm, int nblk,
+                                                     double* __restrict__ norm, float* __restrict__ in32, int php, int pplane, size_t pbs) {
+    __shared__ double sh[2 * NT / 64];
+    const int b = blockIdx.y;
+    const size_t chunk = (n + gridDim.x - 1) / gridDim.x;
+    const size_t i0 = (size_t)blockIdx.x * chunk, i1 = (i0 + chunk < n) ? i0 + chunk : n;
+    double vr[NRQ];
+#pragma unroll
+    for (int q = 0; q < NRQ; ++q) {
+        const size_t i = i0 + threadIdx.x + (size_t)NT * q;
+        const size_t ic = (i < i1) ? i : i0;
+        vr[q] = vin[(size_t)b * n + ic];
+    }
+    double lo = INFINITY, hi = -INFINITY;
+    for (int i = threadIdx.x; i < nblk; i += NT) {
+        lo = fmin(lo, mm[((size_t)b * nblk + i) * 2]);
+        hi = fmax(hi, mm[((size_t)b * nblk + i) * 2 + 1]);
+    }
+    block_minmax(lo, hi, sh);
+    const double range = hi - lo;
+    if (blockIdx.x == 0 && threadIdx.x == 0) { norm[2 * b] = lo; norm[2 * b + 1] = range; }
+    float* dst = in32 + (size_t)b * pbs;
+    auto put = [&](size_t i, double v) __attribute__((always_inline)) {
+        const int c = (int)(i / plane), rem = (int)(i - (size_t)c * plane);
+        const int w = rem / H, h = rem - w * H;
+        dst[(size_t)c * pplane + (size_t)(w + 1) * php + h + 1] = (float)((v - lo) / range);
+    };
+#pragma unroll
+    for (int q = 0; q < NRQ; ++q) {
+        const size_t i = i0 + threadIdx.x + (size_t)NT * q;
+        if (i < i1) put(i, vr[q]);
+    }
+    for (size_t i = i0 + threadIdx.x + (size_t)NT * NRQ; i < i1; i += NT) put(i, vin[(size_t)b * n + i]);
+    if (multi_level) {
+        const int per = (plane + gridDim.x - 1) / gridDim.x;
+        const int c0 = blockIdx.x * per, c1 = (c0 + per < plane) ? c0 + per : plane;
+        for (int i = c0 + threadIdx.x; i < c1; i += NT) {
+            const int w = i / H, h = i - w * H;
+            dst[(size_t)s * pplane + (size_t)(w + 1) * php + h + 1] = (float)noise_std;
         }
     }
 }
@@ -249,6 +293,16 @@
     };
     if (complex_tsmi) go(std::true_type{});
     else go(std::false_type{});
+    if (ctx->prof_level > 0) ctx->prof.n_ew_launches += mm_ready ? 1 : 2;
+    QMRI_HIP(ctx, hipGetLastError());
+    return QMRI_OK;
+}
+
+int ew_launch_normalise_v(qmri_ctx* ctx, int B, size_t n, int plane, int H, int s, int multi_level, double noise_std, const double* v, const double* mm,
+                          double* norm, int nblk, const PTensor& in32) {
+    k_normalise_v<<<dim3(nblk, B), dim3(NT), 0, ctx->stream>>>(n, plane, H, s, multi_level, noise_std, v, mm, nblk, norm, in32.base1(), in32.hp,
+                                                              (int)in32.plane(), in32.batch_stride());
+    if (ctx->prof_level > 0) ctx->prof.n_ew_launches += 1;
     QMRI_HIP(ctx, hipGetLastError());
     return QMRI_OK;
 }
diff --git a/qmri_pnp_recon_poc_amd/csrc/qmri_internal.h b/qmri_pnp_recon_poc_amd/csrc/qmri_internal.h
--- a/qmri_pnp_recon_poc_amd/csrc/qmri_internal.h
+++ b/qmri_pnp_recon_poc_amd/csrc/qmri_internal.h
@@ -83,6 +83,7 @@
     K_RES_STAMPS, K_CONV_STAMPS, K_CONV_STAMP_LAUNCH, K_LSQR_STAMPS,
     K_CONV_MT2, K_CONV_OCC,
     K_FUSE_EW,
+    K_FUSE_NORM,
     K_LSQR_PERSIST,
     K_LSQR_FOLD,
     K_DICTW_LSP,
@@ -202,8 +203,12 @@
 
 struct ActCheckArgs { const float* slots; int* count; float* ref; int record; unsigned* range_flag; unsigned* host_words; int nlayers; };
 
+constexpr int NORM_REQ_MAX_NBLK = 768;
+struct NormReq { bool pending = false; const double* v = nullptr; const double* mm = nullptr; double* norm = nullptr; int nblk = 0, s = 0, multi = 0; double noise_std = 0.0; };
+
 struct NetPlan {
     qmri_net_desc desc{};
+    NormReq norm_req;
     int H = 0, W = 0, maxB = 0;
     std::vector<ConvLayer> layers;
     PTensor x[4], a[4], t[4];
@@ -427,6 +432,7 @@
     double2* d_chat = nullptr;
     double* d_mm = nullptr;
     double* d_norm = nullptr;
+    double* d_vr = nullptr;
     double* d_diag = nullptr;
     double* d_pd = nullptr;
     int32_t* h_flags = nullptr;
@@ -504,14 +510,15 @@
                   double2* y_out, double* pdiag);
 int dc_launch_adj(qmri_ctx* ctx, const OpDev& op, int B, const double2* y_in, double2* tmp, double2* dst);
 int dc_launch_adj_h(qmri_ctx* ctx, const OpDev& op, int B, const double2* tmp, double2* dst, const double2* u = nullptr,
-                    double* mm = nullptr, bool mm_cpx = false);
+                    double* mm = nullptr, bool mm_cpx = false,
+                    double* vr = nullptr);
 struct DualArgs {
     const float* out32; const float* in32; int php, pplane; size_t out_bs, in_bs; int residual_noise;
     const double* norm; const double2* x; double2* u; double* pz;
     int complex_tsmi;
 };
 int dc_hpass_blocks(const OpDev& op);
-struct LsqrFuse { int z_hpass_nblk = 0; const double2* mm_u = nullptr; double* mm = nullptr; bool mm_cpx = false; };
+struct LsqrFuse { int z_hpass_nblk = 0; const double2* mm_u = nullptr; double* mm = nullptr; bool mm_cpx = false; double* mm_vr = nullptr; };
 int dc_launch_dual_fwd_h(qmri_ctx* ctx, const OpDev& op, int B, const DualArgs& d, const ActCheckArgs& ac, double2* tmp);
 void qmri_free_operator(qmri_ctx* ctx);
 void qmri_free_net(qmri_ctx* ctx);
@@ -537,6 +544,8 @@
 int ew_launch_minmax_normalise(qmri_ctx* ctx, int B, size_t n, int plane, int H, int s, int multi_level, double noise_std,
                                const double2* x, const double2* u, double* mm, double* norm, int nblk, const PTensor& in32, bool mm_ready = false,
                                bool complex_tsmi = false);
+int ew_launch_normalise_v(qmri_ctx* ctx, int B, size_t n, int plane, int H, int s, int multi_level, double noise_std, const double* v, const double* mm,
+                          double* norm, int nblk, const PTensor& in32);
 int ew_launch_unnormalise_dual(qmri_ctx* ctx, int B, size_t n, int plane, int H, const PTensor& out32, const PTensor& in32,
                                int residual_noise, const double* norm, const double2* x, double2* u, double2* v, double2* z,
                                double* pz, int nblk_z, int s = 0, bool complex_tsmi = false);
@@ -569,6 +578,7 @@
                  const PTensor* add2, int relu_out);
 struct Conv6rRun {
     const ConvLayer* head = nullptr; const PTensor* head_in = nullptr;
+    const NormReq* head_norm = nullptr;
     const ConvLayer* res = nullptr; int nres = 0;
     const PTensor* src = nullptr; const PTensor* cur = nullptr; const PTensor* skip = nullptr;
     const ConvLayer* tail = nullptr; const PTensor* tail_out = nullptr;
```

New measurement: 826.8 ADMM iters/s, median of 6. No clear change (+0.7%).
